# mailund/stralg

Measured on AMD Instinct MI355X. Metric: Msuffixes/s (SA-IS + BWT C/O tables, 1 GiB DNA), higher is better.
Workload: dtype u8 text / u32 indices; 1 GPU; sa_is_construction + init_bwt_table (C, O) on 1073741824 symbols (dna), alphabet_size=5, one independent record per GPU; n=1073741824, alphabet_size=5, records_per_gpu=1, parallelism=batch x1, no collectives, seed=42, generator=dna, numa_node_rank0=1

## Files before the change

### include/stralg_amd.h

```cpp
#ifndef STRALG_AMD_H
#define STRALG_AMD_H

#include <stddef.h>
#include <stdint.h>

#ifdef __cplusplus
extern "C" {
#endif

typedef struct sx_ctx sx_ctx;

enum {
    SX_OK = 0,
    SX_E_ARG = -1,
    SX_E_NOMEM = -2,
    SX_E_INTERNAL = -3,
    SX_E_MALFORMED = -4,
    SX_E_CAPACITY = -5
};

enum {
    SX_KC_CLASSIFY = 0,
    SX_KC_SAMPLES,
    SX_KC_KEYS,
    SX_KC_RADIX_HIST,
    SX_KC_RADIX_SCATTER,
    SX_KC_SCAN,
    SX_KC_NAMES,
    SX_KC_DOUBLING,
    SX_KC_INDUCE_GATHER,
    SX_KC_INDUCE_SCAN,
    SX_KC_INDUCE_SCATTER,
    SX_KC_INDUCE_CHAIN,
    SX_KC_BWT_GATHER,
    SX_KC_OTABLE,
    SX_KC_MISC,
    SX_KC_FASTA,
    SX_KC_REMAP,
    SX_KC_LCP,
    SX_KC_SEARCH,
    SX_KC_LOCAL_SORT,
    SX_KC_SAM,
    SX_KC_COUNT
};

typedef struct sx_kernel_stat {
    uint64_t launches;
    double ms;
    uint64_t alg_bytes;
} sx_kernel_stat;

typedef struct sx_build_stats {
    uint64_t n;
    uint64_t n_lms;
    uint64_t n_samples;
    uint64_t n_names;
    uint32_t key_bits;
    uint32_t key_slots;
    uint32_t doubling_rounds;
    uint32_t induce_rounds;
    uint32_t sort_passes;
    uint32_t lms_path;
    uint32_t sort_local;
    uint32_t refine_tiers;
    double ms_total;
    uint32_t induce_redo;
    uint32_t long_runs;
    uint32_t recursion_levels;
    uint32_t sample_tied_permille;
    uint32_t long_subbuckets;
} sx_build_stats;

int sx_device_count(void);
int sx_device_numa_node(int device);
int sx_ctx_create(int device, sx_ctx **out);
void sx_ctx_destroy(sx_ctx *ctx);
int sx_ctx_live_count(void);
const char *sx_last_error(const sx_ctx *ctx);
void sx_ctx_trim(sx_ctx *ctx);
enum {
    SX_FLAG_FORCE_GENERAL_PATH = 1,
    SX_FLAG_CHAIN_MAX_ENTRIES = 2,
    SX_FLAG_NO_DIRECT_SORT = 3,
    SX_FLAG_PREFIX_SYMBOLS = 4,
    SX_FLAG_RADIX_DIGIT_BITS = 5,
    SX_FLAG_SORT_MODE = 6,
    SX_FLAG_INDUCE_BATCH_OFF = 7,
    SX_FLAG_INDUCE_BATCH_MIN = 8,
    SX_FLAG_INDUCE_ATTENDED = 9
    ,SX_FLAG_COPY_TEXT_FIRST = 10
    ,SX_FLAG_RECURSE_MIN = 11
    ,SX_FLAG_SAMPLE_MIN = 12
    ,SX_FLAG_INDUCE_NO_HOIST = 13
    ,SX_FLAG_TEXT_KEYS_OFF = 14
    ,SX_FLAG_LONG_SUBBUCKETS_OFF = 15
    ,SX_FLAG_SMALL_DIRECT_MAX = 16
    ,SX_FLAG_LOCAL_SORT_LEAN_OFF = 17
    ,SX_FLAG_SAM_BATCH_READS = 18
    ,SX_FLAG_SAM_WINDOW_BYTES = 19
};
int sx_ctx_set_flag(sx_ctx *ctx, int flag, int value);

int sx_sa_build(sx_ctx *ctx, const uint8_t *text, uint64_t n, uint32_t alphabet_size,
                uint32_t *sa_out);
int sx_sa_build_dev(sx_ctx *ctx, const uint8_t *d_text, uint64_t n, uint32_t alphabet_size,
                    uint32_t *d_sa_out);

int sx_sa_bwt_build_dev(sx_ctx *ctx, const uint8_t *d_text, uint64_t n, uint32_t alphabet_size,
                        uint32_t *d_sa_out, uint8_t *d_bwt_out);

int sx_bwt_tables(sx_ctx *ctx, const uint8_t *text, const uint32_t *sa, uint64_t N,
                  uint32_t sigma, uint32_t *c_out, uint32_t *o_out);
int sx_bwt_tables_dev(sx_ctx *ctx, const uint8_t *d_text, const uint32_t *d_sa, uint64_t N,
                      uint32_t sigma, uint32_t *d_c_out, uint32_t *d_o_out, uint8_t *d_bwt_out);

int sx_bwt_tables_from_bwt_dev(sx_ctx *ctx, const uint8_t *d_bwt, uint64_t N, uint32_t sigma,
                               uint32_t *d_c_out, uint32_t *d_o_out);
int sx_build_tables(sx_ctx *ctx, const uint8_t *text, uint64_t n, uint32_t sigma, uint32_t *sa_out,
                    uint32_t *c_out, uint32_t *o_out);

int sx_sa_inverse_dev(sx_ctx *ctx, const uint32_t *d_sa, uint64_t N, uint32_t *d_inv_out);
int sx_sa_lcp_dev(sx_ctx *ctx, const uint8_t *d_text, const uint32_t *d_sa, uint64_t N, uint32_t *d_inv_out,
                  uint32_t *d_lcp_out);
int sx_sa_inverse_lcp(sx_ctx *ctx, const uint8_t *text, const uint32_t *sa, uint64_t N, uint32_t *inv_out,
                      uint32_t *lcp_out);
int sx_bwt_exact_search_dev(sx_ctx *ctx, const uint32_t *d_c_table, const uint32_t *d_o_table, uint64_t N,
                            uint32_t sigma, const uint8_t *d_patterns, const uint32_t *d_offsets, uint32_t count,
                            uint32_t *d_l_out, uint32_t *d_r_out);

#define SX_APPROX_MAX_EDITS 8
#define SX_APPROX_GAP_D 0x8000u
typedef struct sx_approx_hit {
    uint32_t query;
    uint32_t L, R;
    uint16_t match_length;
    uint16_t n_gaps;
    uint16_t gap[SX_APPROX_MAX_EDITS];
} sx_approx_hit;
int sx_bwt_approx_search_dev(sx_ctx *ctx, const uint32_t *d_c_table, const uint32_t *d_o_table,
                             const uint32_t *d_ro_table, uint64_t N, uint32_t sigma, const uint8_t *d_patterns,
                             const uint32_t *d_offsets, uint32_t count, int max_edits, uint64_t *d_hit_offsets,
                             sx_approx_hit *d_hits, uint64_t hit_capacity, uint64_t *total_hits_out);
int sx_bwt_approx_search(sx_ctx *ctx, const uint32_t *c_table, const uint32_t *o_table, const uint32_t *ro_table,
                         uint64_t N, uint32_t sigma, const uint8_t *patterns, const uint32_t *offsets, uint32_t count,
                         int max_edits, uint64_t *hit_offsets, sx_approx_hit **hits_out, uint64_t *total_hits_out);

typedef int (*sx_sink_fn)(void *user, int section, const void *data, size_t bytes);
enum { SX_SECTION_SA = 0, SX_SECTION_C = 1, SX_SECTION_O = 2, SX_SECTION_SAM = 3 ,
       SX_SECTION_INDEX = 4  };
int sx_build_tables_stream(sx_ctx *ctx, const uint8_t *text, uint64_t n, uint32_t sigma, int want_sa, sx_sink_fn sink,
                           void *user);

typedef struct sx_sam_batch {
    const sx_approx_hit *d_hits;
    uint64_t n_hits;
    const uint32_t *d_sa;
    uint64_t sa_len;
    const uint32_t *const *d_sa_list;
    const uint64_t *d_sa_len_list;
    const uint8_t *d_names, *d_seqs, *d_quals;
    const uint32_t *d_name_off, *d_seq_off, *d_qual_off;
    uint32_t n_reads;
    const uint8_t *d_rnames;
    const uint32_t *d_rname_off;
    uint32_t n_records;
} sx_sam_batch;
int sx_sam_layout_dev(sx_ctx *ctx, const sx_sam_batch *batch, uint64_t *d_byte_offsets, uint64_t *total_bytes_out);
int sx_sam_emit_dev(sx_ctx *ctx, const sx_sam_batch *batch, const uint64_t *d_byte_offsets, uint64_t total_bytes, uint64_t byte_lo,
                    uint64_t byte_hi, uint8_t *d_out);

typedef struct sx_fastq {
    uint32_t count;
    uint8_t *names, *seqs, *quals;
    uint32_t *name_off, *seq_off, *qual_off;
} sx_fastq;
int sx_fastq_index(const uint8_t *file, size_t len, sx_fastq *out);
void sx_fastq_free(sx_fastq *fq);

typedef struct sx_map_record {
    const char *name;
    const uint32_t *sa;
    const uint32_t *c_table;
// ... 77 lines not shown
```

### stralg_amd/_lib.py

```python
import ctypes as C
import os

_HERE = os.path.dirname(os.path.abspath(__file__))
PRODUCT_LIB = os.path.join(_HERE, "libstralg_amd.so")

KC_NAMES = ["classify", "samples", "keys", "radix_hist", "radix_scatter", "scan", "names", "doubling",
            "induce_gather", "induce_scan", "induce_scatter", "induce_chain", "bwt_gather", "otable", "misc",
            "fasta", "remap", "lcp", "search", "local_sort", "sam"]


class KernelStat(C.Structure):
    _fields_ = [("launches", C.c_uint64), ("ms", C.c_double), ("alg_bytes", C.c_uint64)]


class BuildStats(C.Structure):
    _fields_ = [("n", C.c_uint64), ("n_lms", C.c_uint64), ("n_samples", C.c_uint64),
                ("n_names", C.c_uint64), ("key_bits", C.c_uint32), ("key_slots", C.c_uint32),
                ("doubling_rounds", C.c_uint32), ("induce_rounds", C.c_uint32),
                ("sort_passes", C.c_uint32), ("lms_path", C.c_uint32), ("sort_local", C.c_uint32), ("refine_tiers", C.c_uint32),
                ("ms_total", C.c_double), ("induce_redo", C.c_uint32), ("long_runs", C.c_uint32),
                ("recursion_levels", C.c_uint32), ("sample_tied_permille", C.c_uint32), ("long_subbuckets", C.c_uint32)]

    def as_dict(self):
        return {k: getattr(self, k) for k, _ in self._fields_}


APPROX_MAX_EDITS = 8
APPROX_GAP_D = 0x8000
APPROX_HIT_DTYPE = [("query", "<u4"), ("L", "<u4"), ("R", "<u4"), ("match_length", "<u2"), ("n_gaps", "<u2"),
                    ("gap", "<u2", (APPROX_MAX_EDITS,))]
SX_E_ARG, SX_E_MALFORMED, SX_E_CAPACITY = -1, -4, -5
SX_SECTION_SAM = 3
SX_FLAG_SAM_BATCH_READS, SX_FLAG_SAM_WINDOW_BYTES = 18, 19


class SamBatch(C.Structure):
    _fields_ = [("d_hits", C.c_void_p), ("n_hits", C.c_uint64), ("d_sa", C.c_void_p), ("sa_len", C.c_uint64),
                ("d_sa_list", C.c_void_p), ("d_sa_len_list", C.c_void_p),
                ("d_names", C.c_void_p), ("d_seqs", C.c_void_p), ("d_quals", C.c_void_p),
                ("d_name_off", C.c_void_p), ("d_seq_off", C.c_void_p), ("d_qual_off", C.c_void_p), ("n_reads", C.c_uint32),
                ("d_rnames", C.c_void_p), ("d_rname_off", C.c_void_p), ("n_records", C.c_uint32)]


class Fastq(C.Structure):
    _fields_ = [("count", C.c_uint32), ("names", C.c_void_p), ("seqs", C.c_void_p), ("quals", C.c_void_p),
                ("name_off", C.c_void_p), ("seq_off", C.c_void_p), ("qual_off", C.c_void_p)]


class MapRecord(C.Structure):
    _fields_ = [("name", C.c_char_p), ("sa", C.c_void_p), ("c_table", C.c_void_p), ("o_table", C.c_void_p),
                ("ro_table", C.c_void_p), ("N", C.c_uint64), ("sigma", C.c_uint32), ("remap", C.c_void_p)]


class FastqDev(C.Structure):
    _fields_ = [("count", C.c_uint32), ("d_names", C.c_void_p), ("d_seqs", C.c_void_p), ("d_quals", C.c_void_p),
                ("d_name_off", C.c_void_p), ("d_seq_off", C.c_void_p), ("d_qual_off", C.c_void_p),
                ("name_bytes", C.c_uint64), ("seq_bytes", C.c_uint64), ("qual_bytes", C.c_uint64)]


class IndexSource(C.Structure):
    _fields_ = [("record", MapRecord), ("string", C.c_void_p)]


class IndexRecord(C.Structure):
    _fields_ = [("name", C.c_char_p), ("N", C.c_uint64), ("sigma", C.c_uint32), ("has_ro", C.c_int), ("has_string", C.c_int),
                ("remap", C.c_void_p), ("d_string", C.c_void_p), ("d_sa", C.c_void_p), ("d_c", C.c_void_p), ("d_o", C.c_void_p),
                ("d_ro", C.c_void_p)]


SX_SECTION_INDEX = 4
SINK_FN = C.CFUNCTYPE(C.c_int, C.c_void_p, C.c_int, C.c_void_p, C.c_size_t)


def load(path=None):
    path = path or PRODUCT_LIB
    try:
        import torch
    except ImportError:
        pass
    if not os.path.exists(path):
        raise RuntimeError(
            f"{path} is missing: build it with `make -C stralg_amd/csrc` "
            "(or python -c 'import __graft_entry__ as g; g.build()'); there is no CPU fallback")
    lib = C.CDLL(path)
    vp, u8p, u32p, u64p = C.c_void_p, C.c_void_p, C.c_void_p, C.c_void_p
    sig = {
        "sx_device_count": (C.c_int, []),
        "sx_device_numa_node": (C.c_int, [C.c_int]),
        "sx_ctx_create": (C.c_int, [C.c_int, C.POINTER(vp)]),
        "sx_ctx_destroy": (None, [vp]),
        "sx_ctx_live_count": (C.c_int, []),
        "sx_last_error": (C.c_char_p, [vp]),
        "sx_ctx_trim": (None, [vp]),
        "sx_ctx_set_flag": (C.c_int, [vp, C.c_int, C.c_int]),
        "sx_sa_build": (C.c_int, [vp, u8p, C.c_uint64, C.c_uint32, u32p]),
        "sx_sa_build_dev": (C.c_int, [vp, u8p, C.c_uint64, C.c_uint32, u32p]),
        "sx_sa_bwt_build_dev": (C.c_int, [vp, u8p, C.c_uint64, C.c_uint32, u32p, u8p]),
        "sx_bwt_tables_from_bwt_dev": (C.c_int, [vp, u8p, C.c_uint64, C.c_uint32, u32p, u32p]),
        "sx_build_tables": (C.c_int, [vp, u8p, C.c_uint64, C.c_uint32, u32p, u32p, u32p]),
        "sx_bwt_tables": (C.c_int, [vp, u8p, u32p, C.c_uint64, C.c_uint32, u32p, u32p]),
        "sx_bwt_tables_dev": (C.c_int, [vp, u8p, u32p, C.c_uint64, C.c_uint32, u32p, u32p, u8p]),
        "sx_sa_inverse_dev": (C.c_int, [vp, u32p, C.c_uint64, u32p]),
        "sx_sa_lcp_dev": (C.c_int, [vp, u8p, u32p, C.c_uint64, u32p, u32p]),
        "sx_sa_inverse_lcp": (C.c_int, [vp, u8p, u32p, C.c_uint64, u32p, u32p]),
# ... 78 lines not shown
```

### stralg_amd/api.py

```python
import ctypes as C
import threading
import time

import numpy as np

from . import _lib


class StralgAmdError(RuntimeError):
    pass


def _ptr(x):
    if x is None:
        return None
    if isinstance(x, int):
        return x
    if isinstance(x, np.ndarray):
        return x.ctypes.data
    if hasattr(x, "data_ptr"):
        return x.data_ptr()
    raise TypeError(f"cannot take the address of {type(x)!r}")


# ... 217 lines not shown
        self._check(self.lib.sx_fasta_pack_dev(self.h, _ptr(d_file), file_len, _ptr(d_packed), C.byref(plen), _ptr(d_term),
                                               term_cap, C.byref(nrec)), "sx_fasta_pack_dev")
        return int(plen.value), int(nrec.value)

    def remap_dev(self, d_in, n, d_out):
        table = np.zeros(256, dtype=np.int16)
        sigma = C.c_uint32(0)
        self._check(self.lib.sx_remap_dev(self.h, _ptr(d_in), n, _ptr(d_out), table.ctypes.data_as(C.POINTER(C.c_int16)),
                                          C.byref(sigma)), "sx_remap_dev")
        return int(sigma.value), table

    def reverse_dev(self, d_in, n, d_out):
        self._check(self.lib.sx_reverse_dev(self.h, _ptr(d_in), n, _ptr(d_out)), "sx_reverse_dev")

    def fasta_records(self, data):
        buf = np.frombuffer(bytes(data), dtype=np.uint8)
        packed = np.zeros(buf.size + 1, dtype=np.uint8)
        term = np.zeros(buf.size + 2, dtype=np.uint32)
        plen, nrec = C.c_uint64(0), C.c_uint32(0)
        self._check(self.lib.sx_fasta_pack(self.h, _ptr(buf) if buf.size else None, buf.size, _ptr(packed), C.byref(plen),
                                           _ptr(term), term.size, C.byref(nrec)), "sx_fasta_pack")
        out = []
        for r in range(nrec.value):
            n0 = 0 if r == 0 else int(term[2 * r - 1]) + 1
            s0 = int(term[2 * r]) + 1
            out.append((packed[n0:int(term[2 * r])].tobytes(), packed[s0:int(term[2 * r + 1])].tobytes()))
        return out

    def prim_sort_pairs_dev(self, ka, va, kb, vb, n, begin_bit, end_bit):
        flag = C.c_int(0)
        self._check(self.lib.sx_prim_sort_pairs_dev(self.h, _ptr(ka), _ptr(va), _ptr(kb), _ptr(vb), n, begin_bit,
                                                    end_bit, C.byref(flag)), "sx_prim_sort_pairs_dev")
        return bool(flag.value)

    def prim_exclusive_sum_dev(self, d_in, d_out, n, d_total=None):
        self._check(self.lib.sx_prim_exclusive_sum_dev(self.h, _ptr(d_in), _ptr(d_out), n, _ptr(d_total)),
                    "sx_prim_exclusive_sum_dev")

    def prim_classify_dev(self, d_text, n, d_flags, d_hist_all, d_hist_l, d_hist_lms):
        self._check(self.lib.sx_prim_classify_dev(self.h, _ptr(d_text), n, _ptr(d_flags), _ptr(d_hist_all),
                                                  _ptr(d_hist_l), _ptr(d_hist_lms)), "sx_prim_classify_dev")

    def profile_only(self, kclass_name=None):
        k = -1 if kclass_name is None else _lib.KC_NAMES.index(kclass_name)
        self._check(self.lib.sx_profile_only(self.h, k), "sx_profile_only")

    def profile_enable(self, on=True):
        self._check(self.lib.sx_profile_enable(self.h, 1 if on else 0), "sx_profile_enable")

    def profile_reset(self):
        self._check(self.lib.sx_profile_reset(self.h), "sx_profile_reset")

    def profile_read(self):
        arr = (_lib.KernelStat * len(_lib.KC_NAMES))()
        self._check(self.lib.sx_profile_read(self.h, arr), "sx_profile_read")
        return {name: {"launches": int(arr[i].launches), "ms": float(arr[i].ms), "alg_bytes": int(arr[i].alg_bytes)}
                for i, name in enumerate(_lib.KC_NAMES)}

    def last_stats(self):
        st = _lib.BuildStats()
        self._check(self.lib.sx_last_stats(self.h, C.byref(st)), "sx_last_stats")
        return st.as_dict()

    def force_general_path(self, on=True):
        self._check(self.lib.sx_ctx_set_flag(self.h, 1, 1 if on else 0), "sx_ctx_set_flag")

    def set_chain_max_entries(self, entries):
        self._check(self.lib.sx_ctx_set_flag(self.h, 2, int(entries)), "sx_ctx_set_flag")

    def set_no_direct_sort(self, on=True):
        self._check(self.lib.sx_ctx_set_flag(self.h, 3, 1 if on else 0), "sx_ctx_set_flag")

    def set_prefix_symbols(self, symbols):
        self._check(self.lib.sx_ctx_set_flag(self.h, 4, int(symbols)), "sx_ctx_set_flag")

    def set_radix_digit_bits(self, bits):
        self._check(self.lib.sx_ctx_set_flag(self.h, 5, int(bits)), "sx_ctx_set_flag")

    def set_sort_mode(self, mode):
        self._check(self.lib.sx_ctx_set_flag(self.h, 6, int(mode)), "sx_ctx_set_flag")

    def set_induce_batch(self, on=True):
        self._check(self.lib.sx_ctx_set_flag(self.h, 7, 0 if on else 1), "sx_ctx_set_flag")

    def set_induce_batch_min(self, entries):
        self._check(self.lib.sx_ctx_set_flag(self.h, 8, int(entries)), "sx_ctx_set_flag")

    def set_induce_attended(self, mode=1):
        self._check(self.lib.sx_ctx_set_flag(self.h, 9, int(mode)), "sx_ctx_set_flag")

    def set_induce_hoist(self, on=True):
        self._check(self.lib.sx_ctx_set_flag(self.h, 13, 0 if on else 1), "sx_ctx_set_flag")

    def set_text_keys(self, on=True):
        self._check(self.lib.sx_ctx_set_flag(self.h, 14, 0 if on else 1), "sx_ctx_set_flag")

    def set_long_subbuckets(self, on=True):
        self._check(self.lib.sx_ctx_set_flag(self.h, 15, 0 if on else 1), "sx_ctx_set_flag")

    def set_local_sort_lean(self, on=True):
        self._check(self.lib.sx_ctx_set_flag(self.h, 17, 0 if on else 1), "sx_ctx_set_flag")

    def set_small_direct_max(self, suffixes):
        self._check(self.lib.sx_ctx_set_flag(self.h, 16, int(suffixes)), "sx_ctx_set_flag")

    def set_recurse_min(self, symbols):
        self._check(self.lib.sx_ctx_set_flag(self.h, 11, int(symbols)), "sx_ctx_set_flag")

    def set_sample_min(self, suffixes):
        self._check(self.lib.sx_ctx_set_flag(self.h, 12, int(suffixes)), "sx_ctx_set_flag")

    def set_copy_text_first(self, on=True):
        self._check(self.lib.sx_ctx_set_flag(self.h, 10, 1 if on else 0), "sx_ctx_set_flag")

    def trim(self):
        self.lib.sx_ctx_trim(self.h)

    def bind_to_numa_node(self):
        self.lib.stralg_amd_bind_thread_to_device.argtypes = [C.c_int]
        self.lib.stralg_amd_bind_thread_to_device.restype = C.c_int
        return int(self.lib.stralg_amd_bind_thread_to_device(self.device))


def _map_record(name, t, keep):
    sa = np.ascontiguousarray(t.sa.array, dtype=np.uint32)
    c = np.ascontiguousarray(t.c_table, dtype=np.uint32)
    o = np.ascontiguousarray(t.o_table, dtype=np.uint32)
    ro = None if t.ro_table is None else np.ascontiguousarray(t.ro_table, dtype=np.uint32)
    tab = np.ascontiguousarray(np.clip(t.remap_table.table, -1, 127), dtype=np.int8)
    keep.append((sa, c, o, ro, tab))
    return _lib.MapRecord(bytes(name), _ptr(sa), _ptr(c), _ptr(o), _ptr(ro), sa.size, t.remap_table.alphabet_size, _ptr(tab))


class Index:

    def __init__(self, ctx, handle):
        self.ctx = ctx
        self.h = handle

    @classmethod
    def from_fasta(cls, fasta_bytes, include_reverse=True, ctx=None):
        ctx = ctx or default_context()
        buf = np.frombuffer(bytes(fasta_bytes), dtype=np.uint8)
        h = C.c_void_p()
        ctx._check(ctx.lib.sx_index_build_fasta(ctx.h, _ptr(buf) if buf.size else None, buf.size, 1 if include_reverse else 0,
                                                C.byref(h)), "sx_index_build_fasta")
        return cls(ctx, h)

    @classmethod
    def from_tables(cls, records, ctx=None):
        ctx = ctx or default_context()
        src = (_lib.IndexSource * max(1, len(records)))()
        keep = []
        for r, (name, t) in enumerate(records):
            src[r].record = _map_record(name, t, keep)
            string = getattr(t.sa, "string", None)
            if string is not None:
                string = np.ascontiguousarray(string, dtype=np.uint8)
                keep.append(string)
                src[r].string = _ptr(string)
        h = C.c_void_p()
        ctx._check(ctx.lib.sx_index_from_sources(ctx.h, src, len(records), C.byref(h)), "sx_index_from_sources")
        return cls(ctx, h)

    @classmethod
    def load(cls, path_or_bytes, ctx=None):
# ... 329 lines not shown
```

### stralg_amd/csrc/sx_common.hpp

```cpp
#pragma once
#include <hip/hip_runtime.h>
#include <hip/hip_ext.h>

#include <stdint.h>
#include <stdio.h>
#include <string.h>

#include <vector>

#include "../../include/stralg_amd.h"

#define SX_CHECK(expr)                                                         \
    do {                                                                       \
        hipError_t e_ = (expr);                                                \
        if (e_ != hipSuccess) return sx_fail(ctx, (int)e_, #expr, __FILE__, __LINE__); \
    } while (0)

#define SX_TRY(expr)                                                           \
    do {                                                                       \
        int rc_ = (expr);                                                      \
        if (rc_ != 0) return rc_;                                              \
    } while (0)

struct sx_slab {
    void *p = nullptr;
    size_t cap = 0;
};

struct sx_arena {
    char *base = nullptr;
    size_t cap = 0, off = 0;
    template <class T> T *take(size_t count)
    {
        size_t bytes = (count * sizeof(T) + 255) & ~(size_t)255;
        if (off + bytes > cap) return nullptr;
        T *r = reinterpret_cast<T *>(base + off);
        off += bytes;
        return r;
    }
};

struct sx_event_pair {
    hipEvent_t a, b;
    int kclass;
};

enum {
    SX_SLAB_N = 0,
    SX_SLAB_M = 1,
    SX_SLAB_BWT = 2,
    SX_SLAB_SCAN = 3,
    SX_SLAB_SORT = 4,
    SX_SLAB_IO = 5,
    SX_SLAB_CHAIN = 6,
    SX_NSLABS = 7
};

struct sx_ctx {
    int device = 0;
    hipStream_t stream = nullptr;
    char err[512] = {0};
    sx_slab slab[SX_NSLABS];
    uint32_t *h_pin = nullptr;
    uint32_t readback_seq = 0;
    char *h_stage[2] = {nullptr, nullptr};
    uint32_t chain_epoch = 0;
    int64_t chain_max_override = -1;
    int prefix_symbols = 0;
    int force_general = 0;
    int no_direct = 0;
    int radix_digit_bits = 0;
    int sort_mode = 0;
    int induce_batch_off = 0;
    int induce_attended = 0;
    int induce_no_hoist = 0;
    int text_keys_off = 0;
    int long_subbuckets_off = 0;
    int local_sort_lean_off = 0;
    int64_t small_direct_max = -1;
    int copy_text_first = 0;
    int64_t sam_batch_reads = 0;
    int64_t sam_window_bytes = 0;
    int64_t sample_min = -1;
    int64_t recurse_min = -1;
    sx_ctx *child = nullptr;
    int depth = 0;
    int64_t induce_batch_min = -1;
    int prof_on = 0;
    int prof_only = -1;
    hipError_t launch_err = hipSuccess;
    int launch_err_class = 0;
    std::vector<sx_event_pair> ev_used;
    std::vector<sx_event_pair> ev_free;
    sx_kernel_stat kstat[SX_KC_COUNT];
    sx_build_stats stats;
};

int sx_fail(sx_ctx *ctx, int code, const char *what, const char *file, int line);
int sx_fail_msg(sx_ctx *ctx, int code, const char *msg);
int sx_slab_ensure(sx_ctx *ctx, int which, size_t bytes);
int sx_sync(sx_ctx *ctx);
int sx_readback(sx_ctx *ctx, const uint32_t *d_src, size_t count, uint32_t *h_dst);
int sx_readback_ranges(sx_ctx *ctx, const uint32_t *const *d_src, const uint32_t *counts, int ranges, uint32_t *h_dst);
int sx_chain_slab(sx_ctx *ctx, int which, size_t bytes);
uint32_t sx_chain_next_epoch(sx_ctx *ctx);

int sx_child_begin(sx_ctx *ctx, sx_ctx **child);
void sx_child_end(sx_ctx *ctx, sx_ctx *child);

sx_event_pair *sx_prof_pair(sx_ctx *ctx, int kclass);
void sx_prof_count(sx_ctx *ctx, int kclass, uint64_t alg_bytes);

template <class... P, class... A>
static inline void sx_launch(sx_ctx *ctx, int kclass, uint64_t alg_bytes, void (*kernel)(P...),
                             dim3 grid, dim3 block, A... args)
{
    const bool timed = ctx->prof_on && (ctx->prof_only < 0 || ctx->prof_only == kclass);
    sx_event_pair *ep = timed ? sx_prof_pair(ctx, kclass) : nullptr;
    if (ep) hipExtLaunchKernelGGL(kernel, grid, block, 0, ctx->stream, ep->a, ep->b, 0u, static_cast<P>(args)...);
    else hipLaunchKernelGGL(kernel, grid, block, 0, ctx->stream, args...);
    const hipError_t e = hipGetLastError();
    if (e != hipSuccess && ctx->launch_err == hipSuccess) ctx->launch_err = e, ctx->launch_err_class = kclass;
    if (ep) sx_prof_count(ctx, kclass, alg_bytes);
}

static inline uint32_t sx_div_up(uint64_t a, uint64_t b) { return (uint32_t)((a + b - 1) / b); }
static inline int sx_bitlen(uint64_t v)
{
    int b = 0;
    while (v) {
        ++b;
        v >>= 1;
    }
    return b;
}
```

### stralg_amd/csrc/sx_ctx.hip

```cpp
#include <atomic>
#include <chrono>
#include "sx_common.hpp"
#include "sx_scan.hpp"

#include <new>

static const char *kClassNames[SX_KC_COUNT] = {
    "classify", "samples", "keys", "radix_hist", "radix_scatter", "scan", "names",
    "doubling", "induce_gather", "induce_scan", "induce_scatter", "induce_chain", "bwt_gather", "otable", "misc",
    "fasta", "remap", "lcp", "search", "local_sort", "sam",
};

int sx_fail(sx_ctx *ctx, int code, const char *what, const char *file, int line)
{
    if (ctx) snprintf(ctx->err, sizeof ctx->err, "%s failed: %s (%d) at %s:%d", what,
                      hipGetErrorString((hipError_t)code), code, file, line);
    return code ? code : SX_E_INTERNAL;
}

int sx_fail_msg(sx_ctx *ctx, int code, const char *msg)
{
    if (ctx) snprintf(ctx->err, sizeof ctx->err, "%s", msg);
    return code;
}
// ... 93 lines not shown
int sx_readback(sx_ctx *ctx, const uint32_t *d_src, size_t count, uint32_t *h_dst)
{
    if (count > 1024) return sx_fail_msg(ctx, SX_E_INTERNAL, "readback too large");
    const uint32_t seq = ++ctx->readback_seq ? ctx->readback_seq : ++ctx->readback_seq;
    hipLaunchKernelGGL(sx::readback_kernel, dim3(1), dim3(256), 0, ctx->stream, d_src, (uint32_t)count, ctx->h_pin, seq);
    if (hipGetLastError() != hipSuccess) return sx_fail_msg(ctx, SX_E_INTERNAL, "readback launch refused");
    return readback_wait(ctx, seq, count, h_dst);
}

int sx_readback_ranges(sx_ctx *ctx, const uint32_t *const *d_src, const uint32_t *counts, int ranges, uint32_t *h_dst)
{
    sx::readback_ranges r = {{nullptr, nullptr, nullptr, nullptr}, {0, 0, 0, 0}};
    size_t total = 0;
    if (ranges < 1 || ranges > 4) return sx_fail_msg(ctx, SX_E_INTERNAL, "readback: one to four arrays");
    for (int k = 0; k < ranges; ++k) r.src[k] = d_src[k], r.count[k] = counts[k], total += counts[k];
    if (total > 1024) return sx_fail_msg(ctx, SX_E_INTERNAL, "readback too large");
    const uint32_t seq = ++ctx->readback_seq ? ctx->readback_seq : ++ctx->readback_seq;
    hipLaunchKernelGGL(sx::readback_ranges_kernel, dim3(1), dim3(256), 0, ctx->stream, r, ctx->h_pin, seq);
    if (hipGetLastError() != hipSuccess) return sx_fail_msg(ctx, SX_E_INTERNAL, "readback launch refused");
    return readback_wait(ctx, seq, total, h_dst);
}

static int readback_wait(sx_ctx *ctx, uint32_t seq, size_t count, uint32_t *h_dst)
{
    volatile uint32_t *flag = ctx->h_pin + 1024;
    const auto t0 = std::chrono::steady_clock::now();
    uint32_t spins = 0;
    while (*flag != seq) {
        __builtin_ia32_pause();
        if ((++spins & 0xFFu) == 0 && std::chrono::steady_clock::now() - t0 > std::chrono::microseconds(kReadbackSpinUs)) break;
    }
    if (*flag != seq) SX_CHECK(hipStreamSynchronize(ctx->stream));
    std::atomic_thread_fence(std::memory_order_acquire);
    if (*flag != seq) return sx_fail_msg(ctx, SX_E_INTERNAL, "readback: the sequence word did not arrive");
    if (ctx->launch_err != hipSuccess) return launch_error(ctx);
    memcpy(h_dst, ctx->h_pin, count * sizeof(uint32_t));
    return 0;
}

sx_event_pair *sx_prof_pair(sx_ctx *ctx, int kclass)
{
    sx_event_pair ep;
    if (!ctx->ev_free.empty()) {
        ep = ctx->ev_free.back();
        ctx->ev_free.pop_back();
    } else {
        if (hipEventCreate(&ep.a) != hipSuccess || hipEventCreate(&ep.b) != hipSuccess) return nullptr;
    }
    ep.kclass = kclass;
    ctx->ev_used.push_back(ep);
    return &ctx->ev_used.back();
}

void sx_prof_count(sx_ctx *ctx, int kclass, uint64_t alg_bytes)
{
    ctx->kstat[kclass].launches += 1;
    ctx->kstat[kclass].alg_bytes += alg_bytes;
}

static void prof_drain(sx_ctx *ctx)
{
    if (ctx->ev_used.empty()) return;
    (void)hipStreamSynchronize(ctx->stream);
    for (sx_event_pair &ep : ctx->ev_used) {
        float ms = 0.f;
        if (hipEventElapsedTime(&ms, ep.a, ep.b) == hipSuccess) ctx->kstat[ep.kclass].ms += ms;
        ctx->ev_free.push_back(ep);
    }
    ctx->ev_used.clear();
}

int sx_child_begin(sx_ctx *ctx, sx_ctx **out)
{
    if (!ctx->child) {
        int rc = sx_ctx_create(ctx->device, &ctx->child);
        if (rc != 0) return sx_fail_msg(ctx, rc, "cannot create the context of the reduced string");
        ctx->child->depth = ctx->depth + 1;
    }
    sx_ctx *c = ctx->child;
    c->chain_max_override = ctx->chain_max_override;
    c->radix_digit_bits = ctx->radix_digit_bits;
    c->sort_mode = ctx->sort_mode;
    c->induce_batch_off = ctx->induce_batch_off;
    c->induce_batch_min = ctx->induce_batch_min;
    c->induce_attended = ctx->induce_attended;
    c->induce_no_hoist = ctx->induce_no_hoist;
    c->text_keys_off = ctx->text_keys_off;
    c->long_subbuckets_off = ctx->long_subbuckets_off;
    c->local_sort_lean_off = ctx->local_sort_lean_off;
    c->small_direct_max = ctx->small_direct_max;
    c->copy_text_first = ctx->copy_text_first;
    c->recurse_min = ctx->recurse_min;
    c->sample_min = ctx->sample_min;
    c->no_direct = 1;
    c->force_general = 1;
    c->prefix_symbols = 0;
    c->prof_on = ctx->prof_on;
    c->prof_only = ctx->prof_only;
    *out = c;
    return 0;
}

void sx_child_end(sx_ctx *ctx, sx_ctx *c)
{
    prof_drain(c);
    for (int k = 0; k < SX_KC_COUNT; ++k) {
        ctx->kstat[k].launches += c->kstat[k].launches;
        ctx->kstat[k].ms += c->kstat[k].ms;
        ctx->kstat[k].alg_bytes += c->kstat[k].alg_bytes;
    }
    memset(c->kstat, 0, sizeof c->kstat);
    c->prof_on = 0;
}

extern "C" {

int sx_device_count(void)
{
    int n = 0;
    if (hipGetDeviceCount(&n) != hipSuccess) return 0;
    return n;
}

int sx_device_numa_node(int device)
{
    char bus[64] = {0};
    if (hipDeviceGetPCIBusId(bus, (int)sizeof bus, device) != hipSuccess) return -1;
    for (char *p = bus; *p; ++p)
        if (*p >= 'A' && *p <= 'F') *p = (char)(*p - 'A' + 'a');
    char path[160];
    snprintf(path, sizeof path, "/sys/bus/pci/devices/%s/numa_node", bus);
    FILE *f = fopen(path, "r");
    if (!f) return -1;
    int node = -1;
    if (fscanf(f, "%d", &node) != 1) node = -1;
    fclose(f);
    return node;
}

static std::atomic<int> g_live_contexts{0};
extern "C" int sx_ctx_live_count(void) { return g_live_contexts.load(); }

int sx_ctx_create(int device, sx_ctx **out)
{
    if (!out) return SX_E_ARG;
    *out = nullptr;
    int ndev = 0;
    hipError_t e = hipGetDeviceCount(&ndev);
    if (e != hipSuccess || ndev <= 0) {
        fprintf(stderr, "stralg_amd: no usable HIP device (%s); this library has no CPU fallback\n",
                e != hipSuccess ? hipGetErrorString(e) : "device count 0");
        return e != hipSuccess ? (int)e : SX_E_INTERNAL;
    }
    if (device < 0 || device >= ndev) return SX_E_ARG;
    sx_ctx *ctx = new (std::nothrow) sx_ctx();
    if (!ctx) return SX_E_NOMEM;
    ctx->device = device;
    memset(ctx->kstat, 0, sizeof ctx->kstat);
    memset(&ctx->stats, 0, sizeof ctx->stats);
    if (hipSetDevice(device) != hipSuccess || hipStreamCreateWithFlags(&ctx->stream, hipStreamNonBlocking) != hipSuccess ||
        hipHostMalloc((void **)&ctx->h_pin, 8192, hipHostMallocDefault) != hipSuccess) {
        fprintf(stderr, "stralg_amd: cannot initialise device %d\n", device);
        delete ctx;
        return SX_E_INTERNAL;
    }
    memset(ctx->h_pin, 0, 8192);
// ... 28 lines not shown
    }
    if (ctx->h_pin) (void)hipHostFree(ctx->h_pin);
    for (char *b : ctx->h_stage)
        if (b) (void)hipHostFree(b);
    if (ctx->stream) (void)hipStreamDestroy(ctx->stream);
    g_live_contexts.fetch_sub(1);
    delete ctx;
}

int sx_ctx_set_flag(sx_ctx *ctx, int flag, int value)
{
    if (!ctx) return SX_E_ARG;
    if (flag == SX_FLAG_FORCE_GENERAL_PATH) {
        ctx->force_general = value ? 1 : 0;
        return 0;
    }
    if (flag == SX_FLAG_NO_DIRECT_SORT) {
        ctx->no_direct = value ? 1 : 0;
        return 0;
    }
    if (flag == SX_FLAG_PREFIX_SYMBOLS) {
        ctx->prefix_symbols = value > 0 ? value : 0;
        return 0;
    }
    if (flag == SX_FLAG_SORT_MODE) {
        if (value < 0 || value > 3) return SX_E_ARG;
        ctx->sort_mode = value;
        return 0;
    }
    if (flag == SX_FLAG_RADIX_DIGIT_BITS) {
        if (value != 0 && (value < 8 || value > 10)) return SX_E_ARG;
        ctx->radix_digit_bits = value;
        return 0;
    }
    if (flag == SX_FLAG_INDUCE_BATCH_OFF) {
        ctx->induce_batch_off = value ? 1 : 0;
        return 0;
    }
    if (flag == SX_FLAG_SAMPLE_MIN) {
        ctx->sample_min = value < 0 ? -1 : (int64_t)value;
        return 0;
    }
    if (flag == SX_FLAG_RECURSE_MIN) {
        ctx->recurse_min = value < 0 ? -1 : (int64_t)value;
        return 0;
    }
    if (flag == SX_FLAG_COPY_TEXT_FIRST) {
        ctx->copy_text_first = value ? 1 : 0;
        return 0;
    }
    if (flag == SX_FLAG_INDUCE_ATTENDED) {
        if (value < 0 || value > 2) return SX_E_ARG;
        ctx->induce_attended = value == 1 ? 1 : 0;
        return 0;
    }
    if (flag == SX_FLAG_TEXT_KEYS_OFF) {
        ctx->text_keys_off = value ? 1 : 0;
        return 0;
    }
    if (flag == SX_FLAG_SMALL_DIRECT_MAX) {
        ctx->small_direct_max = value < 0 ? -1 : (int64_t)value;
        return 0;
    }
    if (flag == SX_FLAG_LONG_SUBBUCKETS_OFF) {
        ctx->long_subbuckets_off = value ? 1 : 0;
        return 0;
    }
    if (flag == SX_FLAG_LOCAL_SORT_LEAN_OFF) {
        ctx->local_sort_lean_off = value ? 1 : 0;
        return 0;
    }
    if (flag == SX_FLAG_SAM_BATCH_READS) {
        ctx->sam_batch_reads = value > 0 ? value : 0;
        return 0;
    }
    if (flag == SX_FLAG_SAM_WINDOW_BYTES) {
        ctx->sam_window_bytes = value > 0 ? value : 0;
        return 0;
    }
    if (flag == SX_FLAG_INDUCE_NO_HOIST) {
        ctx->induce_no_hoist = value ? 1 : 0;
        return 0;
    }
    if (flag == SX_FLAG_INDUCE_BATCH_MIN) {
        ctx->induce_batch_min = value < 0 ? -1 : (int64_t)value;
        return 0;
    }
    if (flag == SX_FLAG_CHAIN_MAX_ENTRIES) {
        ctx->chain_max_override = value < 0 ? -1 : (int64_t)value;
        return 0;
    }
    return SX_E_ARG;
}

const char *sx_last_error(const sx_ctx *ctx) { return ctx ? ctx->err : "no context"; }

int sx_profile_enable(sx_ctx *ctx, int on)
{
    if (!ctx) return SX_E_ARG;
    if (!on) prof_drain(ctx);
    ctx->prof_on = on ? 1 : 0;
    return 0;
}

int sx_profile_only(sx_ctx *ctx, int kclass)
{
    if (!ctx || kclass >= SX_KC_COUNT) return SX_E_ARG;
    ctx->prof_only = kclass < 0 ? -1 : kclass;
    return 0;
}

int sx_profile_reset(sx_ctx *ctx)
{
    if (!ctx) return SX_E_ARG;
    prof_drain(ctx);
    memset(ctx->kstat, 0, sizeof ctx->kstat);
    return 0;
}

int sx_profile_read(sx_ctx *ctx, sx_kernel_stat *out)
{
    if (!ctx || !out) return SX_E_ARG;
    prof_drain(ctx);
    memcpy(out, ctx->kstat, sizeof ctx->kstat);
    return 0;
}

const char *sx_kernel_class_name(int kclass)
{
    return kclass >= 0 && kclass < SX_KC_COUNT ? kClassNames[kclass] : "?";
}

int sx_last_stats(const sx_ctx *ctx, sx_build_stats *out)
{
    if (!ctx || !out) return SX_E_ARG;
    *out = ctx->stats;
    return 0;
}

}
```

### stralg_amd/csrc/sx_induce.hip

```cpp
#include "sx_induce_common.hpp"
#include "sx_induce_small.hpp"
#include "sx_induce_wide.hpp"
#include "sx_induce_chain.hpp"

using namespace sx;

size_t sx_induce_scratch_bytes(uint64_t N, uint32_t sigma)
{
    const uint64_t ntiles = (N + kIndTile - 1) / kIndTile + 1;
    const uint64_t wtiles = N / 4096 + 4;
    return (size_t)N * 8 + 256 + (size_t)(N / 2 + 2) * 8 + 256 + (size_t)N + 256 + (size_t)sigma * ntiles * 4 + 256 +
           (size_t)kBatchRows * (ntiles + 1) * 4 + 1024 +
           (sigma > 8 ? (size_t)(wtiles + wtiles / 256 + 4) * 1024 + 512 : 0) + 16384 +
           (sigma > 8 ? ((size_t)N / kWideTile + 520) * 1024 + 5 * 65536 * 4 + 16384 : 0);
}

namespace {
#ifndef SX_INDUCE_GRID_CAP
#define SX_INDUCE_GRID_CAP 16384
#endif
constexpr uint32_t kInduceGridCap = SX_INDUCE_GRID_CAP;
constexpr int kMaxSpec = 16;

template <class WT> struct induce_state {
    sx_ctx *ctx;
    const uint8_t *T;
    uint32_t *SA;
    WT *WN;
    uint64_t N, m;
    uint8_t *BW;
    uint32_t *cursor[2];
    uint32_t *ranges;
    uint32_t *tickets;
    uint32_t *run_len;
    uint64_t *status;
    uint32_t chain_max;
    uint32_t *hist;
    uint32_t *bhist;
    uint32_t *btotals;
    int batch_on;
    int unattended;
    uint32_t *poison;
    uint32_t *host_poison;
    uint32_t *whist;
    uint32_t *wsums;
    uint32_t stride;
    uint32_t nk;
    int small_alphabet;
    int par;
    wnd_cfg cfg;
    int hoist;
    uint32_t *d_begin;
    uint32_t *hoist_E;
    uint32_t *hoist_tot;
    uint32_t *hoist_err;
    uint32_t hoist_from;
    int next_c;
    int begun_c;
};

template <class WT>
void launch_round(induce_state<WT> &st, const uint32_t *srcP, const WT *srcW, int range_slot, int out_slot,
                  uint32_t tiles_bound, uint32_t tiles_likely, int rev, int mode, uint32_t c, int dir, int tail_follows,
                  int chained_only_up_to_chain_max = 0, int three_launch_only = 0)
{
    sx_ctx *ctx = st.ctx;
    uint32_t grid = tiles_bound < 1 ? 1 : tiles_bound;
    if (grid > kInduceGridCap) grid = kInduceGridCap;
    const uint32_t epoch = sx_chain_next_epoch(ctx);
    uint32_t *rin = st.ranges + 2 * range_slot;
    uint32_t *rout = out_slot >= 0 ? st.ranges + 2 * out_slot : nullptr;
    const uint32_t *cur = st.cursor[st.par];
    uint32_t *nxt = st.cursor[st.par ^ 1];
    const bool only3 = three_launch_only != 0;
    const bool both = only3 || (!chained_only_up_to_chain_max && (uint64_t)tiles_likely * kIndTile > st.chain_max);
    const uint32_t chain_max = only3 ? 0u : ((both || chained_only_up_to_chain_max) ? st.chain_max : ~0u);
    const int pass_large = chained_only_up_to_chain_max;
    if (both && st.small_alphabet) {
        const uint8_t *srcB = srcP == st.SA ? (const uint8_t *)st.BW : nullptr;
        const uint64_t src_len = srcP == st.SA ? st.N : st.m;
        if (srcB)
            sx_launch(ctx, SX_KC_INDUCE_GATHER, 0, induce_count_bytes_kernel, dim3(grid), dim3(kBlock), srcB, (const uint32_t *)rin, rev,
                      mode, c, st.hist, st.stride, st.nk, chain_max, src_len);
        else
            sx_launch(ctx, SX_KC_INDUCE_GATHER, 0, induce_count_kernel<WT, 3>, dim3(grid), dim3(kBlock), srcW, srcB,
                      (const uint32_t *)rin, rev, mode, c, st.cfg, st.hist, st.stride, st.nk, chain_max, src_len);
        sx_launch(ctx, SX_KC_INDUCE_SCAN, (uint64_t)tiles_bound * st.nk * 8, induce_offsets_kernel, dim3(st.nk),
                  dim3(kRowThreads), st.hist, st.stride, (const uint32_t *)rin, rout, cur, nxt, dir, c, chain_max, only3 ? 1 : 0);
        {
#define SX_SCATTER_SMALL(M)                                                                                            \
    sx_launch(ctx, SX_KC_INDUCE_SCATTER, 0, induce_scatter_small_kernel<WT, M>, dim3(grid), dim3(kBlock), srcP, srcW, \
              (const uint32_t *)rin, c, st.cfg, st.T, (const uint32_t *)st.hist, st.stride, cur, st.SA, st.WN, st.BW, st.nk, \
              chain_max)
            switch (mode) {
            case MODE_L_FROM_L: SX_SCATTER_SMALL(MODE_L_FROM_L); break;
            case MODE_L_FROM_LMS: SX_SCATTER_SMALL(MODE_L_FROM_LMS); break;
            case MODE_S_FROM_S: SX_SCATTER_SMALL(MODE_S_FROM_S); break;
            default: SX_SCATTER_SMALL(MODE_S_FROM_L); break;
            }
#undef SX_SCATTER_SMALL
        }
    }
    if (both && !st.small_alphabet) {
        const uint8_t *srcB = srcP == st.SA ? (const uint8_t *)st.BW : nullptr;
        const uint32_t wtiles = sx_div_up((uint64_t)(tiles_bound < 1 ? 1 : tiles_bound) * kIndTile, kWideTile);
        const uint32_t wgrid = wtiles > 2048 ? 2048 : wtiles;
        const int only = only3 ? 1 : 0;
        sx_launch(ctx, SX_KC_INDUCE_GATHER, 0, induce_wide_count_kernel<WT>, dim3(wgrid), dim3(kWideThreads), srcW, srcB,
                  (const uint32_t *)rin, rev, mode, c, st.cfg, st.whist, chain_max);
        if (wtiles <= kWideOffMaxTiles) {
            sx_launch(ctx, SX_KC_INDUCE_SCAN, (uint64_t)wtiles * 2048, induce_wide_offsets_kernel, dim3(256 / kWideOffCols), dim3(kWideOffThreads),
                      st.whist, (const uint32_t *)rin, rout, cur, nxt, dir, c, chain_max, only);
        } else {
            const uint32_t nchunks = sx_div_up(wtiles, kWideChunk);
            sx_launch(ctx, SX_KC_INDUCE_SCAN, (uint64_t)wtiles * 1024, induce_wide_colsum_kernel, dim3(nchunks), dim3(kBlock),
                      (const uint32_t *)st.whist, (const uint32_t *)rin, st.wsums, chain_max);
            sx_launch(ctx, SX_KC_INDUCE_SCAN, (uint64_t)nchunks * 2048, induce_wide_bases_kernel, dim3(1), dim3(kBlock), st.wsums,
                      (const uint32_t *)rin, rout, cur, nxt, dir, c, chain_max, only);
            sx_launch(ctx, SX_KC_INDUCE_SCAN, (uint64_t)wtiles * 2048, induce_wide_apply_kernel, dim3(nchunks), dim3(kBlock), st.whist,
                      (const uint32_t *)rin, (const uint32_t *)st.wsums, chain_max);
        }
        sx_launch(ctx, SX_KC_INDUCE_SCATTER, 0, induce_wide_scatter_kernel<WT, 8>, dim3(wgrid), dim3(kWideThreads),
                  srcP, srcW, (const uint32_t *)rin, rev, mode, c, st.cfg, st.T, (const uint32_t *)st.whist, cur, dir, st.SA, st.WN,
                  st.BW, chain_max);
    }
    uint32_t cgrid = grid > 1024 ? 1024 : grid;
    if (only3) {
    } else if (st.small_alphabet)
        sx_launch(ctx, SX_KC_INDUCE_CHAIN, 0, induce_round_kernel<WT, 3>, dim3(cgrid), dim3(kBlock), srcP, srcW,
                  (const uint32_t *)rin, rout, rev, mode, c, st.cfg, st.T, cur, nxt, dir, st.SA, st.WN, st.BW, st.nk, st.status,
                  epoch, st.tickets + range_slot, chain_max, tail_follows, pass_large);
    else if (st.nk <= 32)
        sx_launch(ctx, SX_KC_INDUCE_CHAIN, 0, induce_round_kernel<WT, 5>, dim3(cgrid), dim3(kBlock), srcP, srcW,
                  (const uint32_t *)rin, rout, rev, mode, c, st.cfg, st.T, cur, nxt, dir, st.SA, st.WN, st.BW, st.nk, st.status,
                  epoch, st.tickets + range_slot, chain_max, tail_follows, pass_large);
    else
        sx_launch(ctx, SX_KC_INDUCE_CHAIN, 0, induce_round_kernel<WT, 8>, dim3(cgrid), dim3(kBlock), srcP, srcW,
                  (const uint32_t *)rin, rout, rev, mode, c, st.cfg, st.T, cur, nxt, dir, st.SA, st.WN, st.BW, st.nk, st.status,
                  epoch, st.tickets + range_slot, chain_max, tail_follows, pass_large);
    st.par ^= 1;
    ctx->stats.induce_rounds++;
}

#ifndef SX_TAIL_ITERS_UNATTENDED
#define SX_TAIL_ITERS_UNATTENDED 1024u
#endif
constexpr uint32_t kTailIters = 64, kTailItersUnattended = SX_TAIL_ITERS_UNATTENDED;
template <class WT>
void launch_tail(induce_state<WT> &st, int range_slot, int out_slot, int rev, int mode, uint32_t c, int dir)
{
    sx_ctx *ctx = st.ctx;
    const uint32_t *cur = st.cursor[st.par];
    uint32_t *nxt = st.cursor[st.par ^ 1];
    if (st.small_alphabet)
        sx_launch(ctx, SX_KC_INDUCE_CHAIN, 0, induce_tail_small_kernel<WT>, dim3(1), dim3(kTailBlock), st.SA, st.WN, st.BW,
                  (const uint32_t *)(st.ranges + 2 * range_slot), st.ranges + 2 * out_slot, rev, mode, c, st.cfg, st.T,
                  cur, nxt, dir, st.unattended ? kTailItersUnattended : kTailIters, st.unattended ? st.poison : (uint32_t *)nullptr,
                  st.host_poison);
    else {
        tail_next nb = {-1, st.nk, nullptr, nullptr, nullptr, nullptr, nullptr, 0u, nullptr};
        if (st.hoist && st.unattended && st.next_c >= 0)
            nb = {st.next_c, st.nk, (const uint32_t *)st.d_begin, (const uint32_t *)st.hoist_E, (const uint32_t *)st.hoist_tot, st.ranges,
                  st.tickets, (uint32_t)(kMaxSpec + 2), st.hoist_err};
        sx_launch(ctx, SX_KC_INDUCE_CHAIN, 0, induce_tail_kernel<WT, 8>, dim3(1), dim3(kTailBlock), st.SA, st.WN, st.BW,
                  (const uint32_t *)(st.ranges + 2 * range_slot), st.ranges + 2 * out_slot, rev, mode, c, st.cfg, st.T,
                  cur, nxt, dir, st.unattended ? kTailItersUnattended : kTailIters, st.unattended ? st.poison : (uint32_t *)nullptr,
                  st.host_poison, nb);
        st.begun_c = nb.c;
    }
    st.par ^= 1;
}

template <class WT>
void launch_batch(induce_state<WT> &st, int range_slot, int out_slot, uint32_t tiles_bound, int mode, uint32_t c)
{
    sx_ctx *ctx = st.ctx;
    uint32_t grid = tiles_bound < 1 ? 1 : tiles_bound;
    if (grid > kInduceGridCap) grid = kInduceGridCap;
    const uint32_t *rin = st.ranges + 2 * range_slot;
    uint32_t *rout = st.ranges + 2 * out_slot;
    const uint32_t *cur = st.cursor[st.par];
    uint32_t *nxt = st.cursor[st.par ^ 1];
    const uint32_t min_len = ctx->induce_batch_min >= 0 ? (uint32_t)ctx->induce_batch_min : kTailEntries;
    if (mode == MODE_L_FROM_L) {
        sx_launch(ctx, SX_KC_INDUCE_GATHER, 0, induce_batch_count_kernel<WT, MODE_L_FROM_L>, dim3(grid), dim3(kBlock),
                  (const uint32_t *)st.SA, (const WT *)st.WN, rin, c, st.cfg, st.T, st.bhist, st.stride, min_len);
    } else {
        sx_launch(ctx, SX_KC_INDUCE_GATHER, 0, induce_batch_count_kernel<WT, MODE_S_FROM_S>, dim3(grid), dim3(kBlock),
                  (const uint32_t *)st.SA, (const WT *)st.WN, rin, c, st.cfg, st.T, st.bhist, st.stride, min_len);
    }
    sx_launch(ctx, SX_KC_INDUCE_SCAN, (uint64_t)tiles_bound * st.nk * kBatchRounds * 8, induce_batch_offsets_kernel,
              dim3(kBatchRounds * st.nk), dim3(kRowThreads), st.bhist, st.stride, rin, st.btotals, st.nk, min_len);
    if (mode == MODE_L_FROM_L) {
        sx_launch(ctx, SX_KC_INDUCE_SCATTER, 0, induce_batch_scatter_kernel<WT, MODE_L_FROM_L>, dim3(grid), dim3(kBlock),
                  (const uint32_t *)st.SA, (const WT *)st.WN, rin, rout, c, st.cfg, st.T, (const uint32_t *)st.bhist, st.stride,
                  (const uint32_t *)st.btotals, cur, nxt, st.SA, st.WN, st.BW, st.nk, min_len);
    } else {
        sx_launch(ctx, SX_KC_INDUCE_SCATTER, 0, induce_batch_scatter_kernel<WT, MODE_S_FROM_S>, dim3(grid), dim3(kBlock),
                  (const uint32_t *)st.SA, (const WT *)st.WN, rin, rout, c, st.cfg, st.T, (const uint32_t *)st.bhist, st.stride,
                  (const uint32_t *)st.btotals, cur, nxt, st.SA, st.WN, st.BW, st.nk, min_len);
    }
    st.par ^= 1;
    ctx->stats.induce_rounds++;
}

template <class WT>
int run_self_rounds(induce_state<WT> &st, uint32_t fixed_bound, uint32_t region_entries, int rev, int mode, uint32_t c,
                    int dir, int which, uint32_t *total_in_region, double share ,
                    const uint32_t *resume = nullptr )
{
    sx_ctx *ctx = st.ctx;
    bool first = true;
    uint32_t bound_tiles = sx_div_up(region_entries ? region_entries : 1, kIndTile);
    int spec = 1;
    {
        const int sh = st.small_alphabet ? 2 : 6;
        while (spec < kMaxSpec && (bound_tiles >> (sh * spec)) >= 1) ++spec;
    }
    if (!st.small_alphabet) {
        double expect = (double)region_entries * share;
        int by_share = 1;
        const double tail_takes = (double)(kTailMulti * kTailEntries) / ((st.unattended && !resume) ? 2.0 : 8.0);
        while (by_share < kMaxSpec && expect > tail_takes) ++by_share, expect *= share;
        if (st.unattended && !resume) spec = by_share;
        else if (by_share > spec) spec = by_share;
    }
    const uint64_t max_batches = 2 * (st.N / kTailIters) + 64;
    uint32_t r[2] = {0, 0};
    bool resuming = resume != nullptr;
    if (resuming) r[0] = resume[0], r[1] = resume[1];
    for (uint64_t batch = 0;; ++batch) {
        if (batch > max_batches) return sx_fail_msg(ctx, SX_E_INTERNAL, "induce: the rounds of a bucket did not come to an end");
        if (!resuming) {
        if (first && st.hoist) {
            if (st.begun_c != (int)c)
                sx_launch(ctx, SX_KC_INDUCE_SCAN, 0, bucket_begin_kernel, dim3(1), dim3(256), st.ranges, st.cursor[st.par],
                          (const uint32_t *)st.d_begin, (const uint32_t *)st.hoist_E, (const uint32_t *)st.hoist_tot, st.nk, c, st.hoist_from,
                          dir, st.tickets, (uint32_t)(kMaxSpec + 2), (const uint32_t *)(st.unattended ? st.poison : nullptr), st.hoist_err);
            st.begun_c = -1;
            st.hoist_from = c;
        } else if (first)
            sx_launch(ctx, SX_KC_INDUCE_SCAN, 0, set_range_kernel, dim3(1), dim3(1), st.ranges, fixed_bound, fixed_bound,
                      (const uint32_t *)st.cursor[st.par], (int)c, which, st.tickets, (uint32_t)(kMaxSpec + 2),
                      (const uint32_t *)(st.unattended ? st.poison : nullptr));
        else
            SX_CHECK(hipMemsetAsync(st.tickets, 0, (kMaxSpec + 2) * sizeof(uint32_t), ctx->stream));
        const bool batched = st.small_alphabet && st.batch_on && (mode == MODE_L_FROM_L || mode == MODE_S_FROM_S);
        if (batched) {
            int slot = 0;
            if (first) {
                double expect = (double)region_entries;
                const double batch_from = ctx->induce_batch_min >= 0 ? (double)ctx->induce_batch_min : (double)kBatchFrom;
                for (int k = 0; k < 6 && expect > batch_from; ++k, expect *= share) {
                    uint32_t tb = sx_div_up((uint64_t)(expect * 2.0 < (double)region_entries ? expect * 2.0 : (double)region_entries), kIndTile);
                    if (tb < 256) tb = bound_tiles < 256 ? bound_tiles : 256;
                    const bool sure = ctx->induce_batch_min >= 0 || expect > 4.0 * (double)st.chain_max;
                    launch_round<WT>(st, st.SA, st.WN, slot, slot + 1, tb, tb, rev, mode, c, dir, 1, 0, sure ? 1 : 0);
                    ++slot;
                }
            }
            launch_batch<WT>(st, slot, slot + 1, bound_tiles, mode, c);
            ++slot;
            if (!first) {
                for (int k = 0; k < 3; ++k, ++slot)
                    launch_round<WT>(st, st.SA, st.WN, slot, slot + 1, bound_tiles < 256 ? bound_tiles : 256, 0, rev, mode, c, dir, 1, 1);
            }
            spec = slot;
        }
        for (int k = 0; k < spec && !batched; ++k) {
            uint32_t tb = bound_tiles >> k;
            const uint32_t floor_tiles = bound_tiles < 256 ? bound_tiles : 256;
            if (tb < floor_tiles) tb = floor_tiles;
            double expect = 2.0 * (double)bound_tiles;
            for (int i = 0; i < k; ++i) expect *= share;
            const uint32_t likely = expect < (double)bound_tiles ? (uint32_t)expect : bound_tiles;
            const bool sure = first && k == 0 && (uint64_t)region_entries > 16ull * st.chain_max;
            launch_round<WT>(st, st.SA, st.WN, k, k + 1, tb, first && k == 0 ? bound_tiles : likely, rev, mode, c, dir, 1, 0, sure ? 1 : 0);
        }
        launch_tail<WT>(st, spec, spec + 1, rev, mode, c, dir);
        if (st.unattended) {
            if (total_in_region) *total_in_region = 0xFFFFFFFFu;
            return 0;
        }
        SX_TRY(sx_readback(ctx, st.ranges + 2 * (spec + 1), 2, r));
        if (r[1] == r[0]) {
            if (total_in_region) *total_in_region = dir > 0 ? r[1] : r[0];
            return 0;
        }
        }
        resuming = false;
        sx_launch(ctx, SX_KC_INDUCE_SCAN, 0, set_range_kernel, dim3(1), dim3(1), st.ranges, r[0], r[1],
                  (const uint32_t *)st.cursor[st.par], (int)c, 0, (uint32_t *)nullptr, 0u, (const uint32_t *)nullptr);
        if (r[1] - r[0] <= kRunEntries) {
            for (int rep = 0; rep < 2; ++rep) {
                SX_CHECK(hipMemsetAsync(st.run_len, 0xFF, sizeof(uint32_t), ctx->stream));
                const uint64_t look = st.N < (uint64_t)kRunProbe ? st.N : (uint64_t)kRunProbe;
                sx_launch(ctx, SX_KC_INDUCE_CHAIN, 0, run_probe_kernel, dim3(1, r[1] - r[0]), dim3(kBlock), st.T,
                          (const uint32_t *)st.SA, (const uint32_t *)st.ranges, c, 0u,
                          (uint32_t)(look < kRunProbeChunk ? look : kRunProbeChunk), st.run_len);
                if (look > kRunProbeChunk) {
                    const uint32_t far_chunks = sx_div_up(look - kRunProbeChunk, kRunProbeChunk);
                    sx_launch(ctx, SX_KC_INDUCE_CHAIN, 0, run_probe_kernel,
                              dim3(far_chunks < kRunProbeGrid ? far_chunks : kRunProbeGrid, r[1] - r[0]), dim3(kBlock), st.T,
                              (const uint32_t *)st.SA, (const uint32_t *)st.ranges, c, kRunProbeChunk, (uint32_t)look, st.run_len);
                }
                sx_launch(ctx, SX_KC_INDUCE_CHAIN, 0, run_fill_kernel<WT>, dim3(4096), dim3(kBlock), st.T, st.SA, st.WN, st.BW,
                          (const uint32_t *)st.ranges, (const uint32_t *)st.cursor[st.par], c, rev, dir, st.cfg,
                          (const uint32_t *)st.run_len);
                sx_launch(ctx, SX_KC_INDUCE_CHAIN, 0, run_commit_kernel, dim3(1), dim3(1), st.ranges, st.cursor[st.par], c, dir,
                          (const uint32_t *)st.run_len);
            }
        }
        first = false;
    }
}

template <class WT>
int induce_typed(sx_ctx *ctx, const sx_text_info &ti, uint32_t sigma, const uint32_t *sorted_lms,
                 const void *seed_windows, bool seed_windows_u32, uint32_t *SA, uint8_t *bwt_out, sx_arena &arena, wnd_cfg cfg)
{
    const uint64_t N = ti.N;
    const uint32_t nk = ti.maxc + 1 < sigma ? ti.maxc + 1 : sigma;
    induce_state<WT> st;
    st.ctx = ctx;
    st.T = ti.T;
    st.SA = SA;
    st.nk = nk;
    st.small_alphabet = nk <= 8;
    st.cfg = cfg;
    st.par = 0;
    st.WN = arena.take<WT>(N);
    st.BW = bwt_out ? bwt_out : arena.take<uint8_t>(N);
    st.N = N;
    st.m = ti.m;
    const bool widen = seed_windows && seed_windows_u32 && sizeof(WT) == 8;
    WT *seedW = seed_windows && !widen ? (WT *)seed_windows : arena.take<WT>(ti.m ? ti.m : 1);
    st.cursor[0] = arena.take<uint32_t>(256);
    st.cursor[1] = arena.take<uint32_t>(256);
    st.ranges = arena.take<uint32_t>(2 * (kMaxSpec + 3));
    st.tickets = arena.take<uint32_t>(kMaxSpec + 3);
    st.run_len = arena.take<uint32_t>(4);
    if (!st.WN || !st.BW || !seedW || !st.cursor[0] || !st.cursor[1] || !st.ranges || !st.tickets || !st.run_len)
        return sx_fail_msg(ctx, SX_E_INTERNAL, "induce: arena too small");

    uint32_t begin[257], lms_off[257];
    begin[0] = 0;
    lms_off[0] = 0;
    uint32_t largest = 1;
    for (uint32_t c = 0; c < 256; ++c) {
        begin[c + 1] = begin[c] + ti.h_all[c];
        lms_off[c + 1] = lms_off[c] + ti.h_lms[c];
        if (ti.h_all[c] > largest) largest = ti.h_all[c];
    }
    st.chain_max = ctx->chain_max_override >= 0 ? (uint32_t)ctx->chain_max_override
                                                : (st.small_alphabet ? 256u * (uint32_t)kIndTile : 4u * kTailEntries);
    const size_t status_words = ((size_t)sx_div_up(largest, kIndTile) + 2) * nk + kChainHeader;
    st.stride = sx_div_up(largest, kIndTile) + 1;
    st.hist = st.whist = st.wsums = st.bhist = st.btotals = nullptr;
    st.batch_on = ctx->induce_batch_off ? 0 : 1;
    if (st.small_alphabet) {
        st.hist = arena.take<uint32_t>((size_t)nk * st.stride);
        st.bhist = arena.take<uint32_t>((size_t)kBatchRows * st.stride);
        st.btotals = arena.take<uint32_t>(kBatchRows);
        if (!st.hist || !st.bhist || !st.btotals) return sx_fail_msg(ctx, SX_E_INTERNAL, "induce: arena too small (tile counts)");
    } else {
        const size_t wt = (size_t)sx_div_up(largest, kWideTile) + 2;
        st.whist = arena.take<uint32_t>(wt * 256);
        st.wsums = arena.take<uint32_t>((wt / kWideChunk + 2) * 256);
        if (!st.whist || !st.wsums) return sx_fail_msg(ctx, SX_E_INTERNAL, "induce: arena too small (tile counts)");
    }
    SX_TRY(sx_chain_slab(ctx, SX_SLAB_CHAIN, status_words * 8));
    st.status = (uint64_t *)ctx->slab[SX_SLAB_CHAIN].p;
    SX_CHECK(hipMemsetAsync(st.status, 0, sizeof(uint64_t), ctx->stream));

    if (widen)
        sx_launch(ctx, SX_KC_INDUCE_GATHER, ti.m * 12, widen_windows_kernel, dim3(sx_div_up(ti.m, kBlock * 4)), dim3(kBlock),
                  (const uint32_t *)seed_windows, (uint64_t)ti.m, (uint64_t *)seedW);
    else if (!seed_windows)
        sx_launch(ctx, SX_KC_INDUCE_GATHER, ti.m * (4 + sizeof(WT) + 16), fill_windows_kernel<WT>,
                  dim3(sx_div_up(ti.m, kBlock)), dim3(kBlock), ti.T, sorted_lms, ti.m, cfg, seedW);
    sx_launch(ctx, SX_KC_MISC, 0, set_entry_kernel<WT>, dim3(1), dim3(1), SA, st.WN, st.BW, (uint32_t)ti.n, ti.T, cfg);

    st.poison = arena.take<uint32_t>(4);
    if (!st.poison) return sx_fail_msg(ctx, SX_E_INTERNAL, "induce: arena too small");
    st.host_poison = ctx->h_pin + 1040;
    st.hoist = (!st.small_alphabet && !ctx->induce_no_hoist) ? 1 : 0;
    st.d_begin = st.hoist_E = st.hoist_tot = st.hoist_err = nullptr;
    st.hoist_from = 0;
    st.next_c = st.begun_c = -1;
    uint32_t *hz_BG = nullptr, *hz_EL = nullptr, *hz_ES = nullptr, *hz_tot = nullptr, *hz_dbase = nullptr, *hz_hist = nullptr,
             *hz_desc = nullptr;
    uint32_t h_desc[2][768];
    uint32_t hz_rows[2] = {0, 0}, hz_most[2] = {1, 1};
    if (st.hoist) {
        for (int pass = 0; pass < 2; ++pass) {
            uint32_t row = 0;
            for (uint32_t c = 0; c < 256; ++c) {
                const uint32_t len = c < nk ? (pass == 0 ? ti.h_lms[c] : ti.h_l[c]) : 0u;
                h_desc[pass][c] = pass == 0 ? lms_off[c] : begin[c];
                h_desc[pass][256 + c] = len;
                h_desc[pass][512 + c] = row;
                const uint32_t tiles = sx_div_up(len, kWideTile);
                row += tiles;
                if (tiles > hz_most[pass]) hz_most[pass] = tiles;
            }
            hz_rows[pass] = row;
        }
        st.d_begin = arena.take<uint32_t>(260);
        hz_BG = arena.take<uint32_t>(65536);
        hz_EL = arena.take<uint32_t>(65536);
        hz_ES = arena.take<uint32_t>(65536);
        hz_tot = arena.take<uint32_t>(65536);
        hz_dbase = arena.take<uint32_t>(65536);
        hz_desc = arena.take<uint32_t>(2 * 768);
        st.hoist_err = arena.take<uint32_t>(4);
        hz_hist = arena.take<uint32_t>(((size_t)(hz_rows[0] > hz_rows[1] ? hz_rows[0] : hz_rows[1]) + 2) * 256);
        if (!st.d_begin || !hz_BG || !hz_EL || !hz_ES || !hz_tot || !hz_dbase || !hz_desc || !st.hoist_err || !hz_hist)
            return sx_fail_msg(ctx, SX_E_INTERNAL, "induce: arena too small (up-front rounds)");
        SX_CHECK(hipMemcpyAsync(st.d_begin, begin, 257 * sizeof(uint32_t), hipMemcpyHostToDevice, ctx->stream));
        SX_CHECK(hipMemcpyAsync(hz_desc, h_desc, sizeof h_desc, hipMemcpyHostToDevice, ctx->stream));
        SX_CHECK(hipMemsetAsync(hz_BG, 0, 65536 * sizeof(uint32_t), ctx->stream));
        SX_CHECK(hipMemsetAsync(st.hoist_err, 0, 4 * sizeof(uint32_t), ctx->stream));
        uint32_t bg_grid = (uint32_t)sx_div_up(sx_div_up(ti.n ? ti.n : 1, 16), (uint64_t)kBigramThreads * 16);
        if (bg_grid > kBigramGrid) bg_grid = kBigramGrid;
        sx_launch(ctx, SX_KC_INDUCE_GATHER, ti.n * (uint64_t)sx_div_up(nk, kBigramWords / nk), bigram_kernel, dim3(bg_grid),
                  dim3(kBigramThreads), ti.T, (uint64_t)ti.n, nk, hz_BG);
        sx_launch(ctx, SX_KC_INDUCE_SCAN, 0, hoist_tables_kernel, dim3(1), dim3(256), (const uint32_t *)hz_BG, (const uint32_t *)st.d_begin, nk,
                  hz_EL, hz_ES);
    }
    auto hoisted_rounds = [&](int pass) -> int {
        const uint32_t *desc = hz_desc + pass * 768;
        const int rev = pass, mode = pass == 0 ? MODE_L_FROM_LMS : MODE_S_FROM_L, dir = pass == 0 ? +1 : -1;
        const uint32_t *srcP = pass == 0 ? sorted_lms : (const uint32_t *)SA;
        const WT *srcW = pass == 0 ? (const WT *)seedW : (const WT *)st.WN;
        const uint8_t *srcB = pass == 0 ? (const uint8_t *)nullptr : (const uint8_t *)st.BW;
        st.hoist_E = pass == 0 ? hz_EL : hz_ES;
        st.hoist_tot = hz_tot;
        st.hoist_from = pass == 0 ? 0u : nk - 1u;
        uint32_t gx = hz_most[pass];
        if (gx > kHoistGridX) gx = kHoistGridX;
        sx_launch(ctx, SX_KC_INDUCE_GATHER, 0, hoist_count_kernel<WT>, dim3(gx, nk), dim3(kWideThreads), srcW, srcB, desc, rev, mode, st.cfg,
                  hz_hist);
        sx_launch(ctx, SX_KC_INDUCE_SCAN, (uint64_t)hz_rows[pass] * 2048, hoist_offsets_kernel, dim3(nk), dim3(kBlock * kHoistOffGroups),
                  hz_hist, desc, (const uint32_t *)st.hoist_E, dir, hz_tot, hz_dbase);
        sx_launch(ctx, SX_KC_INDUCE_SCATTER, 0, hoist_scatter_kernel<WT, 8>, dim3(gx, nk), dim3(kWideThreads), srcP, srcW, desc, rev,
                  mode, st.cfg, st.T, (const uint32_t *)hz_hist, (const uint32_t *)hz_dbase, dir, st.SA, st.WN, st.BW,
                  (uint32_t)(pass == 0 ? 1 : 0));
        ctx->stats.induce_rounds++;
        return 0;
    };
    auto pass_end = [&](int pass, bool with_stop, uint32_t (&rec)[4], uint32_t (&cur)[256], uint32_t (&tail)[3]) -> int {
        const uint32_t *src[4];
        uint32_t cnt[4], page[4 + 256 + 3];
        int k = 0;
        if (with_stop) src[k] = (const uint32_t *)st.poison, cnt[k++] = 4;
        src[k] = (const uint32_t *)st.cursor[st.par], cnt[k++] = nk;
        if (pass == 1) {
            src[k] = (const uint32_t *)st.status, cnt[k++] = 2;
            if (st.hoist) src[k] = (const uint32_t *)st.hoist_err, cnt[k++] = 1;
        }
        SX_TRY(sx_readback_ranges(ctx, src, cnt, k, page));
        const uint32_t *q = page;
        if (with_stop) memcpy(rec, q, sizeof rec), q += 4;
        memcpy(cur, q, nk * sizeof(uint32_t)), q += nk;
        tail[0] = tail[1] = tail[2] = 0;
        if (pass == 1) {
            tail[0] = q[0], tail[1] = q[1];
            if (st.hoist) tail[2] = q[2];
        }
        return 0;
    };
    auto cursors_as_counted = [&](const uint32_t (&cur)[256]) -> bool {
        bool ok = true;
        for (uint32_t c = 1; c < nk; ++c)
            if (ti.h_all[c] && cur[c] != begin[c] + ti.h_l[c]) ok = false;
        return ok;
    };
    const bool unattended_ok = ctx->induce_attended != 1 && ti.open_tiles == 0;
    auto stopped = [&]() -> bool { return st.unattended && *(volatile uint32_t *)st.host_poison != 0; };
    auto pass_L = [&](uint32_t from, const uint32_t *resume) -> int {
        for (uint32_t c = from; c < nk; ++c) {
            if (ti.h_all[c] == 0) continue;
            if (stopped()) return 0;
            const bool carry_on = resume && c == from;
            if (carry_on) st.hoist_from = c;
            if (ti.h_l[c]) {
                uint32_t head_end = 0;
                st.unattended = (unattended_ok && !carry_on) ? 1 : 0;
                st.next_c = -1;
                for (uint32_t c2 = c + 1; c2 < nk && st.next_c < 0; ++c2)
                    if (ti.h_all[c2] && ti.h_l[c2]) st.next_c = (int)c2;
                SX_TRY(run_self_rounds<WT>(st, begin[c], ti.h_l[c], 0, MODE_L_FROM_L, c, +1, 1, &head_end, (double)ti.h_all[c] / (double)N,
                                           carry_on ? resume : nullptr));
                if (!st.unattended && head_end - begin[c] != ti.h_l[c])
                    return sx_fail_msg(ctx, SX_E_INTERNAL, "induce L: bucket did not receive its L-type count");
                st.unattended = unattended_ok ? 1 : 0;
            }
            if (ti.h_lms[c] && !st.hoist) {
                sx_launch(ctx, SX_KC_INDUCE_SCAN, 0, set_range_kernel, dim3(1), dim3(1), st.ranges, lms_off[c], lms_off[c + 1],
                          (const uint32_t *)st.cursor[st.par], (int)c, 0, st.tickets, 1u, (const uint32_t *)(st.unattended ? st.poison : nullptr));
                launch_round<WT>(st, sorted_lms, seedW, 0, -1, sx_div_up(ti.h_lms[c], kIndTile), sx_div_up(ti.h_lms[c], kIndTile), 0,
                                 MODE_L_FROM_LMS, c, +1, 0, 0, ti.h_lms[c] > st.chain_max ? 1 : 0);
            }
        }
        return 0;
    };
    auto pass_S = [&](uint32_t from, const uint32_t *resume) -> int {
        for (uint32_t cc = from + 1; cc-- > 0;) {
            const uint32_t c = cc;
            if (ti.h_all[c] == 0) continue;
            if (stopped()) return 0;
            const bool carry_on = resume && c == from;
            if (carry_on) st.hoist_from = c;
            const uint32_t n_s = ti.h_all[c] - ti.h_l[c];
            if (c > 0 && n_s) {
                uint32_t tail_end = 0;
                st.unattended = (unattended_ok && !carry_on) ? 1 : 0;
                st.next_c = -1;
                for (uint32_t c2 = c; c2-- > 1 && st.next_c < 0;)
                    if (ti.h_all[c2] && ti.h_all[c2] - ti.h_l[c2]) st.next_c = (int)c2;
                SX_TRY(run_self_rounds<WT>(st, begin[c + 1], n_s, 1, MODE_S_FROM_S, c, -1, 2, &tail_end, (double)ti.h_all[c] / (double)N,
                                           carry_on ? resume : nullptr));
                if (!st.unattended && begin[c + 1] - tail_end != n_s)
                    return sx_fail_msg(ctx, SX_E_INTERNAL, "induce S: bucket did not receive its S-type count");
                st.unattended = unattended_ok ? 1 : 0;
            }
            if (ti.h_l[c] && !st.hoist) {
                sx_launch(ctx, SX_KC_INDUCE_SCAN, 0, set_range_kernel, dim3(1), dim3(1), st.ranges, begin[c],
                          begin[c] + ti.h_l[c], (const uint32_t *)st.cursor[st.par], (int)c, 0, st.tickets, 1u,
                          (const uint32_t *)(st.unattended ? st.poison : nullptr));
                launch_round<WT>(st, SA, st.WN, 0, -1, sx_div_up(ti.h_l[c], kIndTile), sx_div_up(ti.h_l[c], kIndTile), 1,
                                 MODE_S_FROM_L, c, -1, 0, 0, ti.h_l[c] > st.chain_max ? 1 : 0);
            }
        }
        return 0;
    };
    ctx->stats.long_runs = ti.open_tiles ? 1u : 0u;
    for (int pass = 0; pass < 2; ++pass) {
        st.unattended = unattended_ok ? 1 : 0;
        if (pass == 1) SX_CHECK(hipStreamSynchronize(ctx->stream));
        SX_CHECK(hipMemcpyAsync(st.cursor[st.par], pass == 0 ? begin : begin + 1, 256 * sizeof(uint32_t), hipMemcpyHostToDevice, ctx->stream));
        if (st.hoist) SX_TRY(hoisted_rounds(pass));
        uint32_t from = pass == 0 ? 0u : nk - 1u, rec[4] = {0, 0, 0, 0}, cur[256], tail[3];
        const uint32_t *resume = nullptr;
        for (uint32_t attempt = 0;; ++attempt) {
            if (attempt > 2 * nk + 4) return sx_fail_msg(ctx, SX_E_INTERNAL, "induce: a pass did not come to its end");
            if (unattended_ok) {
                *(volatile uint32_t *)st.host_poison = 0;
                SX_CHECK(hipMemsetAsync(st.poison, 0, 4 * sizeof(uint32_t), ctx->stream));
            }
            st.next_c = st.begun_c = -1;
            SX_TRY(pass == 0 ? pass_L(from, resume) : pass_S(from, resume));
            SX_TRY(pass_end(pass, unattended_ok, rec, cur, tail));
            if (!unattended_ok || !rec[0]) break;
            ctx->stats.induce_redo++;
            from = rec[1];
            resume = rec + 2;
        }
        if (!cursors_as_counted(cur))
            return sx_fail_msg(ctx, SX_E_INTERNAL, pass == 0 ? "induce L: a bucket did not receive its L-type count"
                                                             : "induce S: a bucket did not receive its S-type count");
        if (pass == 1 && tail[0]) return sx_fail_msg(ctx, SX_E_INTERNAL, "induce: a look-back wait timed out");
        if (pass == 1 && tail[2]) return sx_fail_msg(ctx, SX_E_INTERNAL, "induce: a bucket's cursor is not where the text's bigram counts put it");
    }

    if (ctx->prof_on) {
        uint64_t n_l = 0;
        for (uint32_t c = 0; c < nk; ++c) n_l += ti.h_l[c];
        const uint64_t scanned = n_l + ti.m + (N - 1);
        if (ctx->prof_only < 0 || ctx->prof_only == SX_KC_INDUCE_GATHER)
            ctx->kstat[SX_KC_INDUCE_GATHER].alg_bytes += (scanned - ti.m) + ti.m * sizeof(WT);
        if (ctx->prof_only < 0 || ctx->prof_only == SX_KC_INDUCE_SCATTER)
            ctx->kstat[SX_KC_INDUCE_SCATTER].alg_bytes += (scanned + N) * (4 + sizeof(WT)) + N;
    }
    return 0;
}
}

int sx_bwt_from_seed_windows(sx_ctx *ctx, const uint32_t *seedw, uint64_t N, uint32_t maxc, uint8_t *bwt_out)
{
    wnd_cfg cfg;
    (void)sx_window_cfg(maxc, cfg);
    cfg.CW = 1;
    sx_launch(ctx, SX_KC_BWT_GATHER, N * 5, bwt_from_windows_kernel<uint32_t>, dim3(sx_div_up(N, kBlock * 16)), dim3(kBlock),
              seedw, N, cfg, bwt_out);
    return 0;
}

int sx_induce(sx_ctx *ctx, const sx_text_info &ti, uint32_t sigma, const uint32_t *sorted_lms,
              const void *seed_windows, bool seed_windows_u32, uint32_t *SA, uint8_t *bwt_out, sx_arena &arena)
{
    if (ti.N > 0xFFFFFFFFull) return sx_fail_msg(ctx, SX_E_ARG, "induce: n exceeds 32-bit positions");
    wnd_cfg cfg;
    const bool wide = sx_window_cfg(ti.maxc, cfg);
    if (!wide) return induce_typed<uint32_t>(ctx, ti, sigma, sorted_lms, seed_windows, false, SA, bwt_out, arena, cfg);
    return induce_typed<uint64_t>(ctx, ti, sigma, sorted_lms, seed_windows, seed_windows_u32, SA, bwt_out, arena, cfg);
}
```

### stralg_amd/csrc/sx_induce_chain.hpp

```cpp
#pragma once
#include "sx_induce_common.hpp"

namespace sx {

template <class WT, int BITS>
__global__ __launch_bounds__(kBlock) void induce_round_kernel(
    const uint32_t *__restrict__ srcP, const WT *__restrict__ srcW, const uint32_t *__restrict__ range_in,
    uint32_t *__restrict__ range_out, int rev, int mode, uint32_t c, wnd_cfg cfg, const uint8_t *__restrict__ T,
    const uint32_t *__restrict__ cursor_cur, uint32_t *__restrict__ cursor_nxt, int dir, uint32_t *__restrict__ SA,
    WT *__restrict__ WN, uint8_t *__restrict__ BW, uint32_t nkeys, uint64_t *__restrict__ status, uint32_t epoch,
    uint32_t *__restrict__ ticket,
    uint32_t chain_max ,
    int tail_follows ,
    int pass_large )
{
    __shared__ uint32_t wcount[kWavesPerBlock][256];
    __shared__ uint32_t gpos[256];
    __shared__ uint32_t gbase[256];
    __shared__ uint32_t tcount[256];
    __shared__ uint32_t s_tile;
    const int t = (int)threadIdx.x, lane = lane_id(), w = wave_id();
    const uint32_t lo = range_in[0], hi = range_in[1];
    const uint32_t len = hi - lo;
    if (len > chain_max && !pass_large) return;
    if (len == 0 || (range_out && tail_follows && len <= (BITS > 3 ? kTailMulti * kTailEntries : kTailEntries)) || len > chain_max) {
        if (blockIdx.x == 0) {
            cursor_nxt[t] = cursor_cur[t];
            if (t == 0 && range_out) {
                range_out[0] = len ? lo : hi;
                range_out[1] = hi;
            }
        }
        return;
    }
    const uint32_t ntiles = (len + kIndTile - 1) / kIndTile;
    gbase[t] = cursor_cur[t];
    for (;;) {
        if (t == 0) s_tile = atomicAdd(ticket, 1u);
        for (int i = t; i < kWavesPerBlock * 256; i += kBlock) (&wcount[0][0])[i] = 0;
        __syncthreads();
        const uint32_t tile = s_tile;
        if (tile >= ntiles) break;
        const uint32_t wave0 = tile * (uint32_t)kIndTile + (uint32_t)w * (kWave * kIndItems);
        uint32_t val[kIndItems], dig[kIndItems], rnk[kIndItems];
        WT wnd[kIndItems];
        bool ok[kIndItems];
#pragma unroll
        for (int k = 0; k < kIndItems; ++k) {
            const uint32_t i = wave0 + (uint32_t)k * kWave + lane;
            const uint32_t idx = lo + (i < len ? (rev ? len - 1u - i : i) : 0u);
            val[k] = srcP[idx];
            wnd[k] = srcW[idx];
        }
#pragma unroll
        for (int k = 0; k < kIndItems; ++k) {
            const uint32_t i = wave0 + (uint32_t)k * kWave + lane;
            const uint32_t p = i < len ? val[k] : 0u;
            const WT ww = wnd[k];
            ok[k] = false;
            dig[k] = 0;
            val[k] = 0;
            wnd[k] = 0;
            if (p != 0) {
                const uint32_t ch = wnd_first<WT>(ww, cfg);
                ok[k] = induce_accept(ch, c, mode);
                dig[k] = ch;
                val[k] = p - 1u;
                wnd[k] = wnd_pop<WT>(ww, cfg);
            }
        }
#pragma unroll
        for (int k = 0; k < kIndItems; ++k) rnk[k] = wave_rank_step<BITS>(dig[k], ok[k], wcount[w]);
        __syncthreads();
        {
            const uint32_t d = (uint32_t)t;
            uint32_t cnt = 0;
#pragma unroll
            for (int ww = 0; ww < kWavesPerBlock; ++ww) {
                const uint32_t x = wcount[ww][d];
                wcount[ww][d] = cnt;
                cnt += x;
            }
            uint32_t excl = 0;
            if (BITS > 3) {
                if (d < nkeys) excl = chain_exclusive_prefix(status, nkeys, tile, d, cnt, epoch);
                gpos[d] = excl;
                tcount[d] = cnt;
            } else {
                tcount[d] = cnt;
            }
        }
        if (BITS <= 3) {
            __syncthreads();
            for (uint32_t d = (uint32_t)w; d < nkeys; d += kWavesPerBlock) {
                const uint32_t excl = chain_exclusive_prefix_wave(status, nkeys, tile, d, tcount[d], epoch);
                if (lane == 0) gpos[d] = excl;
            }
        }
        __syncthreads();
        if (tile == ntiles - 1) {
            const uint32_t d = (uint32_t)t;
            const uint32_t total = (d < nkeys ? gpos[d] : 0u) + tcount[d], cur = gbase[d];
            cursor_nxt[d] = dir > 0 ? cur + total : cur - total;
            if (d == c && range_out) {
                range_out[0] = dir > 0 ? cur : cur - total;
                range_out[1] = dir > 0 ? cur + total : cur;
            }
        }
        __syncthreads();
        {
            bool need[kIndItems];
#pragma unroll
            for (int k = 0; k < kIndItems; ++k) need[k] = ok[k] && val[k] != 0 && wnd_count<WT>(wnd[k]) == 0;
            refill_windows<WT, kIndItems>(T, val, need, cfg, wnd);
        }
#pragma unroll
        for (int k = 0; k < kIndItems; ++k) {
            if (ok[k]) {
                const uint32_t d = dig[k];
                const uint32_t r = gpos[d] + wcount[w][d] + rnk[k];
                const uint32_t dst = dir > 0 ? gbase[d] + r : gbase[d] - 1u - r;
                const WT nw = wnd[k];
                SA[dst] = val[k];
                WN[dst] = nw;
                BW[dst] = wnd_symbol<WT>(nw, cfg);
            }
        }
        __syncthreads();
    }
}

struct tail_next {
    int c;
    uint32_t nk;
    const uint32_t *begin;
    const uint32_t *E;
    const uint32_t *tot;
    uint32_t *range;
    uint32_t *tickets;
    uint32_t ntickets;
    uint32_t *err;
};
template <class WT, int BITS>
__global__ __launch_bounds__(kTailBlock) void induce_tail_kernel(uint32_t *SA, WT *WN, uint8_t *BW, const uint32_t *__restrict__ range_in,
                                                             uint32_t *__restrict__ range_out, int rev, int mode,
                                                             uint32_t c, wnd_cfg cfg, const uint8_t *__restrict__ T,
                                                             const uint32_t *__restrict__ cursor_cur,
                                                             uint32_t *__restrict__ cursor_nxt, int dir,
                                                             uint32_t max_iters, uint32_t *poison, uint32_t *host_poison,
                                                             tail_next nb)
{
    constexpr int kDigits = BITS == 3 ? 8 : 256;
    __shared__ uint32_t wcount[kTailWaves][kDigits];
    __shared__ uint32_t gbase[256];
    __shared__ uint32_t s_range[2];
    __shared__ uint32_t s_flag;
    constexpr int kStageCap = BITS > 3 ? kTailTile : 1;
#ifndef SX_TAIL_STAGE_FROM
#define SX_TAIL_STAGE_FROM 512u
#endif
    constexpr uint32_t kStageFrom = SX_TAIL_STAGE_FROM;
    __shared__ WT st_w[kStageCap];
    __shared__ uint32_t st_v[kStageCap];
    __shared__ uint8_t st_d[kStageCap];
    __shared__ uint32_t st_off[BITS > 3 ? 256 : 1], st_ex[BITS > 3 ? 256 : 1], st_scan[kTailWaves];
    const int t = (int)threadIdx.x, lane = lane_id(), w = wave_id();
    if (t < 256) gbase[t] = cursor_cur[t];
    if (t == 0) {
        s_range[0] = range_in[0];
        s_range[1] = range_in[1];
    }
    for (int i = t; i < kTailWaves * kDigits; i += kTailBlock) (&wcount[0][0])[i] = 0;
    __syncthreads();
    uint32_t val[kIndItems];
    WT wnd[kIndItems];
    bool live[kIndItems];
    bool held = false;
    uint32_t prev_len = 0;
    const uint32_t wave0 = (uint32_t)w * (kWave * kIndItems);
    for (uint32_t it = 0; it < max_iters; ++it) {
        const uint32_t lo = s_range[0], len = s_range[1] - lo;
        if (len == 0 || len > (BITS == 3 ? kTailEntries : kTailMulti * kTailEntries)) break;
        const bool multi = len > kTailEntries;
        if ((mode == MODE_L_FROM_L || mode == MODE_S_FROM_S) && len == prev_len && !multi) {
            const uint32_t G = len <= (uint32_t)kTailBlock ? (uint32_t)kTailBlock / len : 1u;
            const uint64_t cpat = 0x0101010101010101ull * (uint64_t)c;
            uint32_t first_other = G;
            for (uint32_t e = (uint32_t)t; e < len * G; e += kTailBlock) {
                const uint32_t i = e / G, q = e % G;
                const uint32_t p = SA[lo + (rev ? len - 1u - i : i)];
                bool all_c = false;
                if (p >= 16u * (q + 1u)) {
                    uint64_t o0, o1;
                    load_bytes16(T, (uint64_t)(p - 16u * (q + 1u)), o0, o1);
                    all_c = o0 == cpat && o1 == cpat;
                }
                if (!all_c && q < first_other) first_other = q;
            }
            if (t == 0) s_flag = G;
            __syncthreads();
            if (first_other < G) atomicMin(&s_flag, first_other);
            __syncthreads();
            const uint32_t L = 16u * s_flag;
            __syncthreads();
            if (L) {
                const uint32_t cur = gbase[c], total = L * len;
                for (uint32_t o = (uint32_t)t; o < total; o += kTailBlock) {
// ... 132 lines not shown
        __syncthreads();
        }
        if ((uint32_t)t == c) {
            const uint32_t now = gbase[c];
            s_range[0] = dir > 0 ? c_first : now;
            s_range[1] = dir > 0 ? now : c_first;
        }
        __syncthreads();
    }
    uint32_t mine = t < 256 ? gbase[t] : 0u;
    if (nb.c >= 0) {
        if (t == 0) {
            s_flag = (s_range[0] != s_range[1] || (poison && poison[0])) ? 1u : 0u;
            for (uint32_t i = 0; i < nb.ntickets; ++i) nb.tickets[i] = 0;
        }
        __syncthreads();
        const uint32_t d = (uint32_t)t, cn = (uint32_t)nb.c;
        if (s_flag) {
            if (t == 0) nb.range[0] = nb.range[1] = 0;
        } else if (d < nb.nk && (dir > 0 ? d >= cn : d <= cn)) {
            uint32_t want, have = mine;
            if (dir > 0) {
                want = cn == 0 ? nb.begin[d] : nb.E[(uint64_t)(cn - 1) * 256 + d];
                for (uint32_t k = c; k < cn; ++k) have += nb.tot[(uint64_t)k * 256 + d];
            } else {
                want = cn + 1 >= nb.nk ? nb.begin[d + 1] : nb.E[(uint64_t)(cn + 1) * 256 + d];
                for (uint32_t k = c; k > cn; --k) have -= nb.tot[(uint64_t)k * 256 + d];
            }
            if (have != want) atomicOr(nb.err, dir > 0 ? 1u : 2u);
            mine = want;
            if (d == cn) {
                nb.range[0] = dir > 0 ? nb.begin[cn] : want;
                nb.range[1] = dir > 0 ? want : nb.begin[cn + 1];
            }
        }
    }
    if (t < 256) cursor_nxt[t] = mine;
    if (t == 0) {
        range_out[0] = s_range[0];
        range_out[1] = s_range[1];
        tail_report(s_range[0], s_range[1], c, poison, host_poison);
    }
}

constexpr uint32_t kRunProbe = 1u << 26;
constexpr uint32_t kRunEntries = 64;
constexpr uint32_t kRunProbeChunk = (uint32_t)kBlock * 16u;
constexpr uint32_t kRunProbeGrid = 256;
__global__ __launch_bounds__(kBlock) void run_probe_kernel(const uint8_t *__restrict__ T, const uint32_t *__restrict__ SA,
                                                          const uint32_t *__restrict__ range, uint32_t c, uint32_t from,
                                                          uint32_t look, uint32_t *__restrict__ run_len )
{
    const uint32_t lo = range[0], len = range[1] - lo;
    if (len == 0 || len > kRunEntries || blockIdx.y >= len) {
        if (blockIdx.x == 0 && blockIdx.y == 0 && threadIdx.x == 0 && (len == 0 || len > kRunEntries)) atomicMin(run_len, 0u);
        return;
    }
    const uint32_t p = SA[lo + blockIdx.y];
    for (uint32_t chunk0 = from + blockIdx.x * kRunProbeChunk; chunk0 < look; chunk0 += gridDim.x * kRunProbeChunk) {
        if (__hip_atomic_load(run_len, __ATOMIC_RELAXED, __HIP_MEMORY_SCOPE_AGENT) <= chunk0) return;
        const uint32_t d0 = chunk0 + threadIdx.x * 16u;
        if (d0 >= p) {
            if (d0 < p + 16u) atomicMin(run_len, p);
            continue;
        }
        const uint32_t cnt = p - d0 < 16u ? p - d0 : 16u;
        uint32_t first_other = cnt;
        for (uint32_t e = 0; e < cnt; ++e)
            if (T[p - d0 - 1u - e] != (uint8_t)c) {
                first_other = e;
                break;
            }
        if (first_other < 16u) atomicMin(run_len, d0 + first_other);
    }
}

__device__ __forceinline__ uint32_t run_length(const uint32_t *run_len, uint32_t len)
{
    if (len == 0 || len > kRunEntries) return 0;
    const uint32_t L = *run_len, most = kRunProbe / len;
    return L > most ? most : L;
}

template <class WT>
__global__ __launch_bounds__(kBlock) void run_fill_kernel(const uint8_t *__restrict__ T, uint32_t *SA, WT *__restrict__ WN,
                                                         uint8_t *__restrict__ BW, const uint32_t *__restrict__ range,
                                                         const uint32_t *__restrict__ cursor, uint32_t c, int rev, int dir,
                                                         wnd_cfg cfg, const uint32_t *__restrict__ run_len)
{
    const uint32_t lo = range[0], len = range[1] - lo;
    const uint64_t total = (uint64_t)run_length(run_len, len) * len;
    const uint32_t cur = cursor[c];
    for (uint64_t o = (uint64_t)blockIdx.x * kBlock + threadIdx.x; o < total; o += (uint64_t)gridDim.x * kBlock) {
        const uint32_t j = (uint32_t)(o / len) + 1u, i = (uint32_t)(o % len);
        const uint32_t v = SA[lo + (rev ? len - 1u - i : i)] - j;
        const uint32_t dst = dir > 0 ? cur + (uint32_t)o : cur - 1u - (uint32_t)o;
        const WT nw = v ? wnd_fill<WT>(T, v, cfg) : (WT)0;
        SA[dst] = v;
        WN[dst] = nw;
        BW[dst] = wnd_symbol<WT>(nw, cfg);
    }
}

__global__ void run_commit_kernel(uint32_t *__restrict__ range, uint32_t *__restrict__ cursor, uint32_t c, int dir,
                                  const uint32_t *__restrict__ run_len)
{
    if (threadIdx.x != 0 || blockIdx.x != 0) return;
    const uint32_t lo = range[0], len = range[1] - lo;
    const uint32_t total = run_length(run_len, len) * len;
    if (total == 0) return;
    const uint32_t cur = cursor[c];
    cursor[c] = dir > 0 ? cur + total : cur - total;
    range[0] = dir > 0 ? cur + total - len : cur - total;
    range[1] = range[0] + len;
}

__global__ void set_range_kernel(uint32_t *range, uint32_t lo, uint32_t hi, const uint32_t *cursor, int c, int which,
                                 uint32_t *tickets, uint32_t ntickets, const uint32_t *poison)
{
    if (threadIdx.x == 0 && blockIdx.x == 0) {
        for (uint32_t i = 0; i < ntickets; ++i) tickets[i] = 0;
        if (which == 1) hi = cursor[c];
        else if (which == 2) lo = cursor[c];
        if (poison && poison[0]) lo = hi = 0;
        range[0] = lo;
        range[1] = hi;
    }
}

__device__ __forceinline__ void tail_report(uint32_t lo, uint32_t hi, uint32_t c, uint32_t *poison, uint32_t *host_poison)
{
    if (!poison || lo == hi || poison[0]) return;
    poison[1] = c, poison[2] = lo, poison[3] = hi;
    poison[0] = 1;
    __hip_atomic_store(host_poison, 1u, __ATOMIC_RELAXED, __HIP_MEMORY_SCOPE_SYSTEM);
}

template <class WT>
__global__ __launch_bounds__(kBlock) void bwt_from_windows_kernel(const WT *__restrict__ WN, uint64_t N, wnd_cfg cfg,
                                                                  uint8_t *__restrict__ bwt)
{
    const uint64_t i0 = ((uint64_t)blockIdx.x * kBlock + threadIdx.x) * 16u;
    if (i0 >= N) return;
    if (i0 + 16u <= N && (((uintptr_t)WN | (uintptr_t)bwt) & 15u) == 0) {
        uint32_t out[4] = {0, 0, 0, 0};
#pragma unroll
        for (int q = 0; q < 4; ++q) {
            WT w[4];
            load_quad(WN + i0 + 4 * q, w);
#pragma unroll
            for (int e = 0; e < 4; ++e) {
                const uint32_t b = wnd_count<WT>(w[e]) == 0 ? 0u : wnd_first<WT>(w[e], cfg);
                out[q] |= (b & 0xFFu) << (8 * e);
            }
        }
        uint4 v;
        v.x = out[0], v.y = out[1], v.z = out[2], v.w = out[3];
        *reinterpret_cast<uint4 *>(bwt + i0) = v;
    } else {
        for (uint64_t i = i0; i < N && i < i0 + 16u; ++i) {
            const WT w = WN[i];
            bwt[i] = wnd_count<WT>(w) == 0 ? (uint8_t)0 : (uint8_t)wnd_first<WT>(w, cfg);
        }
    }
}

__global__ __launch_bounds__(kBlock) void widen_windows_kernel(const uint32_t *__restrict__ in, uint64_t count, uint64_t *__restrict__ out)
{
    const uint64_t i0 = ((uint64_t)blockIdx.x * kBlock + threadIdx.x) * 4u;
    if (i0 >= count) return;
    if (i0 + 4u <= count && (((uintptr_t)in | (uintptr_t)out) & 15u) == 0) {
        const uint4 v = *reinterpret_cast<const uint4 *>(in + i0);
        uint4 a, b;
        a.x = v.x, a.y = 0, a.z = v.y, a.w = 0;
        b.x = v.z, b.y = 0, b.z = v.w, b.w = 0;
        *reinterpret_cast<uint4 *>(out + i0) = a;
        *reinterpret_cast<uint4 *>(out + i0 + 2) = b;
    } else {
        for (uint64_t i = i0; i < count && i < i0 + 4u; ++i) out[i] = in[i];
    }
}

template <class WT>
__global__ void set_entry_kernel(uint32_t *SA, WT *WN, uint8_t *BW, uint32_t p, const uint8_t *T, wnd_cfg cfg)
{
    const WT w = p ? wnd_fill<WT>(T, p, cfg) : (WT)0;
    SA[0] = p;
    WN[0] = w;
    BW[0] = wnd_symbol<WT>(w, cfg);
}

}
```

### stralg_amd/csrc/sx_induce_common.hpp

```cpp
#pragma once
#include "sx_common.hpp"
#include "sx_device.hpp"
#include "sx_scan.hpp"
#include "sx_internal.hpp"
#include "sx_window.hpp"

namespace sx {

constexpr int kIndItems = 8;
constexpr int kIndTile = kBlock * kIndItems;
constexpr int kTailBlock = 1024, kTailWaves = kTailBlock / kWave;
constexpr int kTailTile = kTailBlock * kIndItems;
constexpr uint32_t kTailEntries = (uint32_t)kTailTile;
constexpr uint32_t kTailMulti = 4;

enum { MODE_L_FROM_L = 0, MODE_L_FROM_LMS = 1, MODE_S_FROM_S = 2, MODE_S_FROM_L = 3 };
__device__ __forceinline__ void tail_report(uint32_t lo, uint32_t hi, uint32_t c, uint32_t *poison, uint32_t *host_poison);

__device__ __forceinline__ bool induce_accept(uint32_t ch, uint32_t c, int mode)
{
    switch (mode) {
    case MODE_L_FROM_L: return ch >= c;
    case MODE_L_FROM_LMS: return true;
    case MODE_S_FROM_S: return ch <= c;
    default: return ch < c;
    }
}

template <class WT>
__global__ __launch_bounds__(kBlock) void fill_windows_kernel(const uint8_t *__restrict__ T,
                                                              const uint32_t *__restrict__ pos, uint64_t count,
                                                              wnd_cfg cfg, WT *__restrict__ out)
{
    const uint64_t k = (uint64_t)blockIdx.x * kBlock + threadIdx.x;
    if (k >= count) return;
    const uint32_t p = pos[k];
    out[k] = p ? wnd_fill<WT>(T, p, cfg) : (WT)0;
}

__device__ __forceinline__ void load_quad(const uint32_t *__restrict__ p, uint32_t (&o)[4])
{
    const uint4 v = *reinterpret_cast<const uint4 *>(p);
    o[0] = v.x, o[1] = v.y, o[2] = v.z, o[3] = v.w;
}
__device__ __forceinline__ void load_quad(const uint64_t *__restrict__ p, uint64_t (&o)[4])
{
    const uint4 v0 = *reinterpret_cast<const uint4 *>(p), v1 = *reinterpret_cast<const uint4 *>(p + 2);
    o[0] = pack64(v0.x, v0.y), o[1] = pack64(v0.z, v0.w), o[2] = pack64(v1.x, v1.y), o[3] = pack64(v1.z, v1.w);
}

}
```

### stralg_amd/csrc/sx_induce_small.hpp

```cpp
#pragma once
#include "sx_induce_common.hpp"

namespace sx {


__global__ __launch_bounds__(kBlock) void induce_count_bytes_kernel(const uint8_t *__restrict__ srcB,
                                                                    const uint32_t *__restrict__ range_in, int rev, int mode,
                                                                    uint32_t c, uint32_t *__restrict__ hist, uint32_t stride,
                                                                    uint32_t nkeys, uint32_t chain_max, uint64_t src_len)
{
    const uint32_t lo = range_in[0], len = range_in[1] - lo;
    if (len <= chain_max) return;
    const uint32_t ntiles = (len + kIndTile - 1) / kIndTile;
    const bool aligned = ((uintptr_t)srcB & 15u) == 0;
    {
        constexpr int kPieces = kIndTile / 16 / kWave + 1;
        const int lane = lane_id();
        for (uint32_t tile = blockIdx.x * kWavesPerBlock + wave_id(); tile < ntiles; tile += gridDim.x * kWavesPerBlock) {
            const uint32_t tile0 = tile * (uint32_t)kIndTile;
            const uint32_t cnt = len - tile0 < (uint32_t)kIndTile ? len - tile0 : (uint32_t)kIndTile;
            const uint32_t a = rev ? lo + len - tile0 - cnt : lo + tile0, b = a + cnt;
            uint32_t S[kPieces][4], inside[kPieces];
#pragma unroll
            for (int k = 0; k < kPieces; ++k) {
// ... 46 lines not shown
    if (len <= chain_max) return;
    const uint32_t ntiles = (len + kIndTile - 1) / kIndTile;
    const bool aligned = ((uintptr_t)srcW & 15u) == 0;
    (void)srcB;
    {
        constexpr int kQuads = kIndTile / 4 / kWave + 1;
        const int lane = lane_id();
        for (uint32_t tile = blockIdx.x * kWavesPerBlock + wave_id(); tile < ntiles; tile += gridDim.x * kWavesPerBlock) {
            const uint32_t tile0 = tile * (uint32_t)kIndTile;
            const uint32_t cnt = len - tile0 < (uint32_t)kIndTile ? len - tile0 : (uint32_t)kIndTile;
            const uint32_t a = rev ? lo + len - tile0 - cnt : lo + tile0, b = a + cnt;
            const bool whole = aligned && ((uint64_t)(a >> 2) + (uint64_t)kQuads * kWave) * 4u <= src_len;
            uint64_t packed = 0;
            constexpr int kHalf = (kQuads + 1) / 2;
#pragma unroll 1
            for (int h = 0; h < 2; ++h) {
                WT W[kHalf][4];
                uint32_t inside[kHalf];
#pragma unroll
                for (int kk = 0; kk < kHalf; ++kk) {
                    const int k = h * kHalf + kk;
                    const uint64_t e0 = ((uint64_t)(a >> 2) + (uint64_t)lane + (uint64_t)k * kWave) * 4u;
                    const uint32_t from = e0 < a ? (uint32_t)(a - e0) : 0u, to = e0 >= b ? 0u : (b - e0 < 4u ? (uint32_t)(b - e0) : 4u);
                    inside[kk] = (k < kQuads && from < to) ? ((1u << to) - 1u) & ~((1u << from) - 1u) : 0u;
                    W[kk][0] = W[kk][1] = W[kk][2] = W[kk][3] = 0;
                    if (whole) {
                        if (k < kQuads) load_quad(srcW + e0, W[kk]);
                    } else {
#pragma unroll
                        for (int e = 0; e < 4; ++e)
                            if ((inside[kk] >> e) & 1u) W[kk][e] = srcW[e0 + e];
                    }
                }
#pragma unroll
                for (int kk = 0; kk < kHalf; ++kk) {
#pragma unroll
                    for (int e = 0; e < 4; ++e) {
                        const uint32_t ch = wnd_first<WT>(W[kk][e], cfg) & 7u;
                        const bool ok = ((inside[kk] >> e) & 1u) && wnd_count<WT>(W[kk][e]) != 0 && induce_accept(ch, c, mode);
                        packed += (uint64_t)(ok ? 1u : 0u) << (8u * ch);
                    }
                }
            }
            uint64_t even = packed & 0x00FF00FF00FF00FFull, odd = (packed >> 8) & 0x00FF00FF00FF00FFull;
            even = wave_total_packed(even);
            odd = wave_total_packed(odd);
            if ((uint32_t)lane < nkeys && lane < 8)
                hist[(uint64_t)lane * stride + tile] = (uint32_t)(((lane & 1) ? odd : even) >> (16 * (lane >> 1))) & 0xFFFFu;
        }
        return;
    }
}

__global__ __launch_bounds__(kRowThreads) void induce_offsets_kernel(uint32_t *__restrict__ hist, uint32_t stride,
                                                                const uint32_t *__restrict__ range_in,
                                                                uint32_t *__restrict__ range_out,
                                                                const uint32_t *__restrict__ cursor_cur,
                                                                uint32_t *__restrict__ cursor_nxt, int dir, uint32_t c,
                                                                uint32_t chain_max,
                                                                int only_form )
{
    __shared__ uint32_t lds[kRowPieces * kRowWaves];
    const uint32_t len = range_in[1] - range_in[0];
    if (len <= chain_max) {
        if (only_form && threadIdx.x == 0) {
            cursor_nxt[blockIdx.x] = cursor_cur[blockIdx.x];
            if (blockIdx.x == c && range_out) range_out[0] = range_out[1] = range_in[1];
        }
        return;
    }
    const uint32_t ntiles = (len + kIndTile - 1) / kIndTile;
    const uint32_t key = blockIdx.x;
    const uint32_t total = wide_scan_row_inplace(hist + (uint64_t)key * stride, ntiles, lds);
    if (threadIdx.x == 0) {
        const uint32_t cur = cursor_cur[key];
        cursor_nxt[key] = dir > 0 ? cur + total : cur - total;
        if (key == c && range_out) {
            range_out[0] = dir > 0 ? cur : cur - total;
            range_out[1] = dir > 0 ? cur + total : cur;
        }
    }
}

template <class WT, int MODE>
__global__ __launch_bounds__(kBlock) void induce_scatter_small_kernel(
    const uint32_t *__restrict__ srcP, const WT *__restrict__ srcW, const uint32_t *__restrict__ range_in, uint32_t c,
    wnd_cfg cfg, const uint8_t *__restrict__ T, const uint32_t *__restrict__ offs, uint32_t stride,
    const uint32_t *__restrict__ cursor_cur, uint32_t *__restrict__ SA, WT *__restrict__ WN, uint8_t *__restrict__ BW,
    uint32_t nkeys, uint32_t chain_max)
{
    constexpr bool kRev = MODE == MODE_S_FROM_S || MODE == MODE_S_FROM_L;
    constexpr uint64_t kField16 = 0x00FF00FF00FF00FFull;
    __shared__ uint64_t wsum[2][kWavesPerBlock];
    __shared__ uint64_t sbase[2];
    __shared__ uint32_t gadj[8];
    __shared__ uint32_t sP[kIndTile];
    __shared__ WT sW[kIndTile];
    __shared__ uint8_t sD[kIndTile];
    __shared__ uint16_t refill[kIndTile];
    __shared__ uint32_t nrefill;
    const int t = (int)threadIdx.x, lane = lane_id(), w = wave_id();
    const uint32_t lo = range_in[0], len = range_in[1] - lo;
    if (len <= chain_max) return;
    const uint32_t ntiles = (len + kIndTile - 1) / kIndTile;
    const uint32_t base_d = t < (int)nkeys ? cursor_cur[t] : 0u;
    for (uint32_t tile = blockIdx.x; tile < ntiles; tile += gridDim.x) {
        const uint32_t pre = t < (int)nkeys ? offs[(uint64_t)t * stride + tile] : 0u;
        if (t == 0) nrefill = 0;
        const uint32_t i0 = tile * (uint32_t)kIndTile + (uint32_t)t * kIndItems;
        uint32_t P[kIndItems];
        WT W[kIndItems];
        if (i0 + kIndItems <= len) {
            const uint32_t first = kRev ? lo + len - i0 - kIndItems : lo + i0;
            uint32_t Pm[kIndItems];
            WT Wm[kIndItems];
            __builtin_memcpy(Pm, srcP + first, sizeof(Pm));
            __builtin_memcpy(Wm, srcW + first, sizeof(Wm));
#pragma unroll
            for (int k = 0; k < kIndItems; ++k) {
                P[k] = Pm[kRev ? kIndItems - 1 - k : k];
                W[k] = Wm[kRev ? kIndItems - 1 - k : k];
            }
        } else {
#pragma unroll
            for (int k = 0; k < kIndItems; ++k) {
                const uint32_t i = i0 + (uint32_t)k;
                const uint32_t idx = i < len ? (kRev ? lo + len - 1u - i : lo + i) : lo;
                P[k] = i < len ? srcP[idx] : 0u;
                W[k] = i < len ? srcW[idx] : (WT)0;
            }
        }
        uint32_t rnk[kIndItems], dig[kIndItems];
        bool ok[kIndItems];
        uint64_t cnt = 0;
#pragma unroll
        for (int k = 0; k < kIndItems; ++k) {
            const uint32_t ch = wnd_first<WT>(W[k], cfg) & 7u;
            ok[k] = P[k] != 0 && induce_accept(ch, c, MODE);
            dig[k] = ch;
            rnk[k] = (uint32_t)(cnt >> (8u * ch)) & 0xFFu;
            cnt += (uint64_t)(ok[k] ? 1u : 0u) << (8u * ch);
        }
        const uint64_t own0 = cnt & kField16, own1 = (cnt >> 8) & kField16;
        const uint64_t inc0 = wave_inclusive_sum_packed(own0), inc1 = wave_inclusive_sum_packed(own1);
        if (lane == kWave - 1) wsum[0][w] = inc0, wsum[1][w] = inc1;
        __syncthreads();
        uint64_t ex0 = inc0 - own0, ex1 = inc1 - own1, tot0 = 0, tot1 = 0;
#pragma unroll
        for (int i = 0; i < kWavesPerBlock; ++i) {
            const uint64_t x0 = wsum[0][i], x1 = wsum[1][i];
            if (i < w) ex0 += x0, ex1 += x1;
            tot0 += x0, tot1 += x1;
        }
        if (t < 8) {
            uint32_t first_slot = 0;
            for (int d = 0; d < t; ++d) first_slot += (uint32_t)(((d & 1) ? tot1 : tot0) >> (16 * (d >> 1))) & 0xFFFFu;
            const uint32_t g = kRev ? base_d - 1u - pre : base_d + pre;
            gadj[t] = kRev ? g + first_slot : g - first_slot;
        }
        if (t == 0) {
            uint64_t even = 0, odd = 0;
            uint32_t run = 0;
#pragma unroll
            for (int d = 0; d < 8; ++d) {
                if (d & 1) odd |= (uint64_t)run << (16 * (d >> 1));
                else even |= (uint64_t)run << (16 * (d >> 1));
                run += (uint32_t)(((d & 1) ? tot1 : tot0) >> (16 * (d >> 1))) & 0xFFFFu;
            }
            sbase[0] = even, sbase[1] = odd;
        }
        __syncthreads();
        ex0 += sbase[0];
        ex1 += sbase[1];
        const uint32_t produced = (uint32_t)((tot0 & 0xFFFFu) + ((tot0 >> 16) & 0xFFFFu) + ((tot0 >> 32) & 0xFFFFu) + (tot0 >> 48) +
                                             (tot1 & 0xFFFFu) + ((tot1 >> 16) & 0xFFFFu) + ((tot1 >> 32) & 0xFFFFu) + (tot1 >> 48));
#pragma unroll
        for (int k = 0; k < kIndItems; ++k) {
            if (ok[k]) {
                const uint32_t d = dig[k];
                const uint32_t slot = ((uint32_t)(((d & 1u) ? ex1 : ex0) >> (16u * (d >> 1))) & 0xFFFFu) + rnk[k];
                const uint32_t j = P[k] - 1u;
                const WT nw = wnd_pop<WT>(W[k], cfg);
                sP[slot] = j;
                sW[slot] = nw;
                sD[slot] = (uint8_t)d;
                if (j != 0 && wnd_count<WT>(nw) == 0) refill[atomicAdd(&nrefill, 1u)] = (uint16_t)slot;
            }
        }
        __syncthreads();
        const uint32_t nre = nrefill;
        if (nre) {
            for (uint32_t r = (uint32_t)t; r < nre; r += kBlock) {
                const uint32_t slot = refill[r];
                sW[slot] = wnd_fill<WT>(T, sP[slot], cfg);
            }
            __syncthreads();
        }
#pragma unroll
        for (int k = 0; k < kIndItems; ++k) {
            const uint32_t i = (uint32_t)t + (uint32_t)k * kBlock;
            if (i < produced) {
                const uint32_t g = gadj[sD[i]];
                const uint32_t dst = kRev ? g - i : g + i;
                const WT nw = sW[i];
                SA[dst] = sP[i];
                WN[dst] = nw;
                BW[dst] = wnd_symbol<WT>(nw, cfg);
            }
        }
        __syncthreads();
    }
}

constexpr int kTailBatch = 8;
constexpr uint32_t kRunCap = 255;
#ifndef SX_TAIL_CLOSED_FROM
#define SX_TAIL_CLOSED_FROM 256u
#endif
constexpr uint32_t kClosedFrom = SX_TAIL_CLOSED_FROM;
constexpr uint32_t kClosedEntries = 5120;
template <class WT>
__global__ __launch_bounds__(kTailBlock) void induce_tail_small_kernel(uint32_t *SA, WT *WN, uint8_t *BW,
                                                                       const uint32_t *__restrict__ range_in,
                                                                       uint32_t *__restrict__ range_out, int rev, int mode,
                                                                       uint32_t c, wnd_cfg cfg, const uint8_t *__restrict__ T,
                                                                       const uint32_t *__restrict__ cursor_cur,
                                                                       uint32_t *__restrict__ cursor_nxt, int dir,
                                                                       uint32_t max_iters, uint32_t *poison, uint32_t *host_poison)
{
    constexpr uint64_t kField16 = 0x00FF00FF00FF00FFull;
    __shared__ uint64_t wsum[kTailBatch][2][kTailWaves];
    __shared__ uint32_t s_tot[kTailBatch][8], s_base[kTailBatch][8];
    __shared__ uint32_t gbase[8];
    __shared__ uint32_t s_range[2];
    __shared__ uint32_t s_flag;
    constexpr uint32_t kCfEntries = sizeof(WT) == 4 ? kClosedEntries : 64u;
    __shared__ uint32_t cf_p[kCfEntries];
    __shared__ WT cf_w[kCfEntries];
    __shared__ uint8_t cf_r[kCfEntries];
    __shared__ uint32_t cf_hr[kRunCap + 1], cf_he[8][kRunCap + 1], cf_scan[kTailWaves], cf_rmax;
    const int t = (int)threadIdx.x, lane = lane_id(), w = wave_id();
    if (t < 8) gbase[t] = cursor_cur[t];
    if (t == 0) {
        s_range[0] = range_in[0];
        s_range[1] = range_in[1];
    }
    __syncthreads();
    const uint32_t B = cfg.B, cmask = cfg.mask;
    bool last_batch = false;
    uint32_t val[kIndItems];
    WT wnd[kIndItems];
    uint32_t live = 0;
    uint32_t per = kIndItems;
    bool held = false;
    uint32_t prev_len = 0, last_in = ~0u;
    for (uint32_t it = 0; it < max_iters;) {
        const uint32_t lo = s_range[0], len = s_range[1] - lo;
        if (len == 0 || len > kTailEntries) break;
        if (len == prev_len) {
            const uint32_t G = len <= (uint32_t)kTailBlock ? (uint32_t)kTailBlock / len : 1u;
            const uint64_t cpat = 0x0101010101010101ull * (uint64_t)c;
            uint32_t first_other = G;
            for (uint32_t e = (uint32_t)t; e < len * G; e += kTailBlock) {
                const uint32_t i = e / G, q = e % G;
                const uint32_t p = SA[lo + (rev ? len - 1u - i : i)];
                bool all_c = false;
                if (p >= 16u * (q + 1u)) {
                    uint64_t o0, o1;
                    load_bytes16(T, (uint64_t)(p - 16u * (q + 1u)), o0, o1);
                    all_c = o0 == cpat && o1 == cpat;
                }
                if (!all_c && q < first_other) first_other = q;
            }
            if (t == 0) s_flag = G;
            __syncthreads();
            if (first_other < G) atomicMin(&s_flag, first_other);
            __syncthreads();
            const uint32_t L = 16u * s_flag;
            __syncthreads();
            if (L) {
                const uint32_t cur = gbase[c], total = L * len;
                for (uint32_t o = (uint32_t)t; o < total; o += kTailBlock) {
                    const uint32_t j = o / len + 1u, i = o % len;
                    const uint32_t v = SA[lo + (rev ? len - 1u - i : i)] - j;
                    const uint32_t dst = dir > 0 ? cur + o : cur - 1u - o;
                    const WT nw = v ? wnd_fill<WT>(T, v, cfg) : (WT)0;
                    SA[dst] = v;
                    WN[dst] = nw;
                    BW[dst] = wnd_symbol<WT>(nw, cfg);
                }
                __syncthreads();
                if ((uint32_t)t == c) {
                    gbase[c] = dir > 0 ? cur + total : cur - total;
                    s_range[0] = dir > 0 ? cur + total - len : cur - total;
                    s_range[1] = dir > 0 ? cur + total : cur - total + len;
                }
                held = false;
                last_batch = false;
                ++it;
                __syncthreads();
                continue;
            }
        }
        prev_len = len;
        if ((mode == MODE_L_FROM_L || mode == MODE_S_FROM_S) && c >= 1u && last_batch && (uint64_t)len * 2 >= last_in &&
            len >= kClosedFrom && len <= kCfEntries) {
            if (t <= (int)kRunCap) cf_hr[t] = 0;
            for (uint32_t i = (uint32_t)t; i < (kRunCap + 1) * 8; i += kTailBlock) (&cf_he[0][0])[i] = 0;
            __syncthreads();
            const uint64_t cpat = 0x0101010101010101ull * (uint64_t)c;
            const uint32_t per2 = (len + (uint32_t)kTailBlock - 1u) / (uint32_t)kTailBlock;
#pragma unroll 1
            for (uint32_t k = 0; k < per2; ++k) {
                const uint32_t i = (uint32_t)t * per2 + k;
                if (i < len) {
                    const uint32_t p = SA[lo + (rev ? len - 1u - i : i)];
                    uint32_t r = 0;
                    bool open = p != 0;
                    for (uint32_t g = 0; g < (kRunCap + 1) / 64 && open; ++g) {
                        uint64_t o[4][2];
#pragma unroll
                        for (uint32_t u = 0; u < 4; ++u) {
                            const uint32_t done = 64u * g + 16u * u;
                            o[u][0] = o[u][1] = ~cpat;
                            if (p >= done + 16u) load_bytes16(T, (uint64_t)(p - done - 16u), o[u][0], o[u][1]);
                        }
#pragma unroll
                        for (uint32_t u = 0; u < 4; ++u) {
                            const uint32_t done = 64u * g + 16u * u;
                            if (!open) {
                            } else if (p >= done + 16u) {
                                const uint64_t x1 = o[u][1] ^ cpat, x0 = o[u][0] ^ cpat;
                                if (x1) r += (uint32_t)__clzll((unsigned long long)x1) >> 3, open = false;
                                else if (x0) r += 8u + ((uint32_t)__clzll((unsigned long long)x0) >> 3), open = false;
                                else r += 16u;
                            } else {
                                uint32_t a = p - done;
                                while (a > 0 && T[a - 1u] == (uint8_t)c) --a, ++r;
                                open = false;
                            }
                        }
                    }
                    if (r > kRunCap) r = kRunCap;
                    const WT wend = p > r ? wnd_fill<WT>(T, p - r, cfg) : (WT)0;
                    cf_p[i] = p;
                    cf_r[i] = (uint8_t)r;
                    cf_w[i] = wend;
                    atomicAdd(&cf_hr[r], 1u);
                    if (r < kRunCap && p > r) {
                        const uint32_t d = wnd_first<WT>(wend, cfg);
                        if (induce_accept(d, c, mode)) atomicAdd(&cf_he[d & 7u][r], 1u);
                    }
                }
            }
            __syncthreads();
            if (w <= 8) {
                uint32_t *row = w == 0 ? cf_hr : cf_he[w - 1];
                uint32_t v[4], sum = 0, top = 0;
#pragma unroll
                for (int q = 0; q < 4; ++q) {
                    v[q] = row[4 * lane + q];
                    if (v[q]) top = (uint32_t)(4 * lane + q);
                    sum += v[q];
                }
                uint32_t inc = wave_inclusive_scan<OpAdd>(sum);
                if (w == 0) {
                    const uint32_t rmax = wave_reduce_max(top);
                    if (lane == 0) cf_rmax = rmax;
                    uint32_t run = inc - sum, s4[4], ssum = 0;
#pragma unroll
                    for (int q = 0; q < 4; ++q) {
// ... 7 lines not shown
                    for (int q = 0; q < 4; ++q) {
                        row[4 * lane + q] = run2;
                        run2 += s4[q];
                    }
                } else {
                    uint32_t run = inc - sum;
#pragma unroll
                    for (int q = 0; q < 4; ++q) {
                        row[4 * lane + q] = run;
                        run += v[q];
                    }
                }
            }
            __syncthreads();
            const uint32_t rmax = cf_rmax;
            const uint32_t J = rmax < kRunCap ? rmax + 1u : kRunCap;
            const uint32_t curC = gbase[c];
            uint32_t curD[8];
#pragma unroll
            for (int d = 0; d < 8; ++d) curD[d] = gbase[d];
            WT crun = 0;
            for (uint32_t i = 0; i < cfg.CW; ++i) crun = (crun << B) | (WT)(c - 1u);
            const WT field_mask = cfg.CW * B >= 8 * sizeof(WT) ? ~(WT)0 : (((WT)1 << (cfg.CW * B)) - 1u);
            uint32_t cur_len = len;
            for (uint32_t e0 = 0; e0 < J; e0 += (uint32_t)kTailWaves) {
            if (e0 > 0) {
                const uint32_t alive = cf_hr[e0] - cf_hr[e0 - 1u];
                if ((uint64_t)alive * 8 <= (uint64_t)cur_len * 7) {
                    constexpr uint32_t kPerC = (kCfEntries + (uint32_t)kTailBlock - 1u) / (uint32_t)kTailBlock;
                    const uint32_t perc = (cur_len + (uint32_t)kTailBlock - 1u) / (uint32_t)kTailBlock;
                    uint32_t kp[kPerC], kr[kPerC], keep = 0, cnt = 0;
                    WT kw[kPerC];
#pragma unroll
                    for (uint32_t k = 0; k < kPerC; ++k) {
                        const uint32_t i = (uint32_t)t * perc + k;
                        kp[k] = 0, kr[k] = 0, kw[k] = 0;
                        if (k < perc && i < cur_len) {
                            kp[k] = cf_p[i], kr[k] = cf_r[i], kw[k] = cf_w[i];
                            if (kr[k] >= e0) keep |= 1u << k, ++cnt;
                        }
                    }
                    const uint32_t inc = wave_inclusive_scan<OpAdd>(cnt);
                    if (lane == kWave - 1) cf_scan[w] = inc;
                    __syncthreads();
                    uint32_t at = inc - cnt;
                    for (int ww = 0; ww < w; ++ww) at += cf_scan[ww];
#pragma unroll
                    for (uint32_t k = 0; k < kPerC; ++k) {
                        if ((keep >> k) & 1u) {
                            cf_p[at] = kp[k], cf_r[at] = (uint8_t)kr[k], cf_w[at] = kw[k];
                            ++at;
                        }
                    }
                    cur_len = alive;
                    __syncthreads();
                }
            }
            const uint32_t nchunks = (cur_len + (uint32_t)kWave - 1u) / (uint32_t)kWave;
            const uint32_t j = e0 + 1u + (uint32_t)w;
            if (j <= J) {
                uint32_t cc = cf_hr[j - 1u], cd[8];
#pragma unroll
                for (int d = 0; d < 8; ++d) cd[d] = cf_he[d][j - 1u];
                for (uint32_t ch = 0; ch < nchunks; ++ch) {
                    const uint32_t i = ch * (uint32_t)kWave + (uint32_t)lane;
                    const bool valid = i < cur_len;
                    const uint32_t r = valid ? cf_r[i] : 0u, p = valid ? cf_p[i] : 0u;
                    const WT wend = valid ? cf_w[i] : (WT)0;
                    const uint32_t dd = wnd_first<WT>(wend, cfg);
                    const bool cont = valid && r >= j;
                    const bool endf = valid && r + 1u == j && r < kRunCap && p > r && induce_accept(dd, c, mode);
                    const uint64_t bc = __ballot(cont ? 1 : 0);
                    if (bc) {
                        if (cont) {
                            const uint32_t o = cc + (uint32_t)__popcll(bc & lanemask_lt());
                            const uint32_t dst = dir > 0 ? curC + o : curC - 1u - o, pos = p - j;
                            const uint32_t k = r - j, have = k + wnd_count<WT>(wend);
                            WT nw = 0;
                            if (pos != 0) {
                                const WT codes = k >= cfg.CW ? crun : ((crun & (((WT)1 << (k * B)) - 1u)) | ((wend >> kCntBits) << (k * B))) & field_mask;
                                nw = (codes << kCntBits) | (WT)(have < cfg.CW ? have : cfg.CW);
                            }
                            SA[dst] = pos;
                            WN[dst] = nw;
                            BW[dst] = wnd_symbol<WT>(nw, cfg);
                        }
                        cc += (uint32_t)__popcll(bc);
                    }
                    const uint64_t be = __ballot(endf ? 1 : 0);
                    if (be) {
#pragma unroll
                        for (int d = 1; d < 8; ++d) {
                            const bool mine = endf && dd == (uint32_t)d;
                            const uint64_t bd = __ballot(mine ? 1 : 0);
                            if (bd) {
                                if (mine) {
                                    const uint32_t o = cd[d] + (uint32_t)__popcll(bd & lanemask_lt());
                                    const uint32_t dst = dir > 0 ? curD[d] + o : curD[d] - 1u - o, pos = p - j;
                                    const WT nw = pos == 0 ? (WT)0 : wnd_pop<WT>(wend, cfg);
                                    SA[dst] = pos;
                                    WN[dst] = nw;
                                    BW[dst] = wnd_symbol<WT>(nw, cfg);
                                }
                                cd[d] += (uint32_t)__popcll(bd);
                            }
                        }
                    }
                }
            }
            __syncthreads();
            }
            if (t < 8) {
                const uint32_t tot = (uint32_t)t == c ? cf_hr[kRunCap] : cf_he[t][kRunCap];
                const uint32_t before = gbase[t];
                gbase[t] = dir > 0 ? before + tot : before - tot;
                if ((uint32_t)t == c) {
                    const uint32_t from = rmax < kRunCap ? tot : cf_hr[kRunCap - 1u];
                    s_range[0] = dir > 0 ? before + from : before - tot;
                    s_range[1] = dir > 0 ? before + tot : before - from;
                }
            }
            held = false;
            last_batch = true;
            last_in = len;
            it += J;
            __syncthreads();
            continue;
        }
        if (!held) {
            live = 0;
            per = (len + (uint32_t)kTailBlock - 1u) / (uint32_t)kTailBlock;
#pragma unroll
            for (int k = 0; k < kIndItems; ++k) {
                const uint32_t i = (uint32_t)t * per + (uint32_t)k;
                val[k] = 0;
                wnd[k] = 0;
                if ((uint32_t)k < per && i < len) {
                    const uint32_t idx = lo + (rev ? len - 1u - i : i);
                    val[k] = SA[idx];
                    wnd[k] = WN[idx];
                    live |= 1u << k;
                }
            }
            held = true;
        }
        const uint32_t nr = (uint64_t)len * 8 >= last_in ? (uint32_t)kTailBatch : 1u;
        last_in = len;
        last_batch = nr > 1;
        if (nr > 1) {
            WT fresh[kIndItems];
            uint32_t dry = 0;
#pragma unroll
            for (int k = 0; k < kIndItems; ++k) {
                fresh[k] = 0;
                if ((uint32_t)k < per && ((live >> k) & 1u) && val[k] != 0) {
                    const uint32_t need = val[k] < (uint32_t)(kTailBatch + 1) ? val[k] : (uint32_t)(kTailBatch + 1);
                    if (wnd_count<WT>(wnd[k]) < need) {
                        dry |= 1u << k;
                        fresh[k] = wnd_fill<WT>(T, val[k], cfg);
                    }
                }
            }
#pragma unroll
            for (int k = 0; k < kIndItems; ++k)
                if ((dry >> k) & 1u) wnd[k] = fresh[k];
        }
        const bool wave_live = __any(live != 0u ? 1 : 0);
        uint64_t cnt[kTailBatch];
        uint32_t emask[kIndItems];
        uint32_t alive_after = 0;
        uint64_t ex0[kTailBatch], ex1[kTailBatch];
#pragma unroll
        for (int j = 0; j < kTailBatch; ++j) cnt[j] = 0, ex0[j] = 0, ex1[j] = 0;
#pragma unroll
        for (int k = 0; k < kIndItems; ++k) emask[k] = 0;
        if (wave_live) {
#pragma unroll
            for (int k = 0; k < kIndItems; ++k) {
                if ((uint32_t)k >= per) break;
                bool alive = (live >> k) & 1u;
                const WT codes = wnd[k] >> kCntBits;
#pragma unroll
                for (int j = 0; j < kTailBatch; ++j) {
                    if ((uint32_t)j < nr) {
                        const uint32_t sym = ((uint32_t)(codes >> (j * B)) & cmask) + 1u;
                        const bool ok = alive && val[k] > (uint32_t)j && induce_accept(sym, c, mode);
                        if (ok) {
                            const uint32_t sh = 8u * (sym & 7u);
                            emask[k] |= (1u << j) | (((uint32_t)(cnt[j] >> sh) & 7u) << (8 + 3 * j));
                            cnt[j] += 1ull << sh;
                        }
                        alive = ok && sym == c;
                    }
                }
                if (alive) alive_after |= 1u << k;
            }
#pragma unroll
            for (int j = 0; j < kTailBatch; ++j) {
                if ((uint32_t)j < nr) {
                    const uint64_t own0 = cnt[j] & kField16, own1 = (cnt[j] >> 8) & kField16;
                    const uint64_t inc0 = wave_inclusive_sum_packed(own0), inc1 = wave_inclusive_sum_packed(own1);
                    if (lane == kWave - 1) wsum[j][0][w] = inc0, wsum[j][1][w] = inc1;
                    ex0[j] = inc0 - own0, ex1[j] = inc1 - own1;
                }
            }
        } else if (lane < kTailBatch * 2) {
            wsum[lane >> 1][lane & 1][w] = 0;
        }
        __syncthreads();
        if (t < kTailBatch * 2 * kTailWaves) {
            const int j = t / (2 * kTailWaves), h = (t / kTailWaves) & 1, ww = t % kTailWaves;
            static_assert(kTailWaves == 16, "a (round, half) is scanned by a 16-lane segment");
            const uint64_t own = (uint32_t)j < nr ? wsum[j][h][ww] : 0ull;
            const uint64_t inc = row_inclusive_sum_packed(own);
            if ((uint32_t)j < nr) {
                wsum[j][h][ww] = inc - own;
                if (ww == kTailWaves - 1) {
#pragma unroll
                    for (int f = 0; f < 4; ++f) s_tot[j][2 * f + h] = (uint32_t)(inc >> (16 * f)) & 0xFFFFu;
                }
            }
        }
        __syncthreads();
        if (t < 8) {
            uint32_t b = gbase[t];
#pragma unroll
            for (int j = 0; j < kTailBatch; ++j) {
                if ((uint32_t)j < nr) {
                    s_base[j][t] = b;
                    b = dir > 0 ? b + s_tot[j][t] : b - s_tot[j][t];
                }
            }
            gbase[t] = b;
            if ((uint32_t)t == c) {
                const uint32_t sb = s_base[nr - 1u][t], n_last = s_tot[nr - 1u][t];
                s_range[0] = dir > 0 ? sb : sb - n_last;
                s_range[1] = dir > 0 ? sb + n_last : sb;
            }
        }
        __syncthreads();
        uint32_t live_next = 0;
        if (wave_live) {
#pragma unroll
        for (int j = 0; j < kTailBatch; ++j)
            if ((uint32_t)j < nr) ex0[j] += wsum[j][0][w], ex1[j] += wsum[j][1][w];
#pragma unroll
        for (int k = 0; k < kIndItems; ++k) {
            if ((uint32_t)k >= per) break;
            const WT codes = wnd[k] >> kCntBits;
            const uint32_t wcnt = wnd_count<WT>(wnd[k]);
#pragma unroll
            for (int j = 0; j < kTailBatch; ++j) {
                if ((uint32_t)j < nr && ((emask[k] >> j) & 1u)) {
                    const uint32_t d = (((uint32_t)(codes >> (j * B)) & cmask) + 1u) & 7u;
                    const uint64_t exw = (d & 1u) ? ex1[j] : ex0[j];
                    const uint32_t r = ((uint32_t)(exw >> (16u * (d >> 1))) & 0xFFFFu) + ((emask[k] >> (8 + 3 * j)) & 7u);
                    const uint32_t sb = s_base[j][d];
                    const uint32_t dst = dir > 0 ? sb + r : sb - 1u - r;
                    const uint32_t pos = val[k] - (uint32_t)(j + 1);
                    WT nw = (((codes >> (j * B)) >> B) << kCntBits) | (WT)(wcnt - (uint32_t)(j + 1));
                    if (pos != 0 && wcnt == (uint32_t)(j + 1)) nw = wnd_fill<WT>(T, pos, cfg);
                    SA[dst] = pos;
                    WN[dst] = nw;
                    BW[dst] = wnd_symbol<WT>(nw, cfg);
                    if ((uint32_t)j == nr - 1u && ((alive_after >> k) & 1u)) {
                        live_next |= 1u << k;
                        val[k] = pos;
                        wnd[k] = nw;
                    }
                }
            }
        }
        }
        live = live_next;
        it += nr;
        __syncthreads();
    }
    if (t < 8) cursor_nxt[t] = gbase[t];
    if (t == 0) {
        range_out[0] = s_range[0];
        range_out[1] = s_range[1];
        tail_report(s_range[0], s_range[1], c, poison, host_poison);
    }
}

constexpr int kBatchRounds = 8;
constexpr int kBatchRows = kBatchRounds * 8;
#ifndef SX_BATCH_FROM
#define SX_BATCH_FROM (1u << 21)
#endif
constexpr uint32_t kBatchFrom = SX_BATCH_FROM;

template <class WT> struct batch_plan {
    uint32_t a;
    uint32_t tsym;
    bool term;
};

__device__ __forceinline__ uint32_t batch_field_of(uint32_t bit, uint32_t B)
{
    return B == 2 ? bit >> 1 : (B == 1 ? bit : (B == 3 ? (bit * 171u) >> 9 : bit >> 2));
}

template <class WT, int MODE>
__device__ __forceinline__ batch_plan<WT> batch_chain(WT &w, uint32_t p, uint32_t c, const wnd_cfg &cfg, WT cpat,
                                                        const uint8_t *__restrict__ T)
{
    batch_plan<WT> pl;
    uint32_t cntw = wnd_count<WT>(w);
    WT x = (w >> kCntBits) ^ cpat;
    uint32_t r = x ? batch_field_of((uint32_t)(sizeof(WT) == 8 ? __builtin_ctzll((unsigned long long)x) : __builtin_ctz((uint32_t)x)), cfg.B)
                   : cfg.CW;
    if (r >= cntw && cntw <= (uint32_t)kBatchRounds && p > cntw) {
        w = wnd_fill<WT>(T, p, cfg);
        cntw = wnd_count<WT>(w);
        x = (w >> kCntBits) ^ cpat;
        r = x ? batch_field_of((uint32_t)(sizeof(WT) == 8 ? __builtin_ctzll((unsigned long long)x) : __builtin_ctz((uint32_t)x)), cfg.B)
              : cfg.CW;
    }
    uint32_t a = r < cntw ? r : cntw;
    pl.term = a < (uint32_t)kBatchRounds && a < cntw;
    if (a > (uint32_t)kBatchRounds) a = (uint32_t)kBatchRounds;
    pl.a = a;
    pl.tsym = ((uint32_t)((w >> kCntBits) >> (a * cfg.B)) & cfg.mask) + 1u;
    pl.term = pl.term && induce_accept(pl.tsym, c, MODE) && pl.tsym < 8u;
    return pl;
}

template <class WT>
__device__ __forceinline__ WT batch_window(WT w, uint32_t depth, uint32_t pos, const wnd_cfg &cfg, const uint8_t *__restrict__ T)
{
    const uint32_t cntw = wnd_count<WT>(w);
    WT nw = ((((w >> kCntBits) >> (depth * cfg.B)) >> cfg.B) << kCntBits) | (WT)(cntw - (depth + 1u));
    if (pos != 0 && cntw == depth + 1u) nw = wnd_fill<WT>(T, pos, cfg);
    return nw;
}

template <class WT> __device__ __forceinline__ WT batch_cpat(uint32_t c, const wnd_cfg &cfg)
{
    WT pat = 0;
    for (uint32_t i = 0; i < cfg.CW; ++i) pat |= (WT)(c - 1u) << (i * cfg.B);
    return pat;
}

template <class WT, bool kRev, bool kWantP>
__device__ __forceinline__ void batch_load(const uint32_t *__restrict__ srcP, const WT *__restrict__ srcW, uint32_t lo, uint32_t len,
                                           uint32_t i0, uint32_t (&P)[kIndItems], WT (&W)[kIndItems])
{
    if (i0 + kIndItems <= len) {
        const uint32_t first = kRev ? lo + len - i0 - kIndItems : lo + i0;
        uint32_t Pm[kIndItems];
        WT Wm[kIndItems];
        if (kWantP) __builtin_memcpy(Pm, srcP + first, sizeof(Pm));
        __builtin_memcpy(Wm, srcW + first, sizeof(Wm));
#pragma unroll
        for (int k = 0; k < kIndItems; ++k) {
            P[k] = kWantP ? Pm[kRev ? kIndItems - 1 - k : k] : 0u;
            W[k] = Wm[kRev ? kIndItems - 1 - k : k];
        }
    } else {
#pragma unroll
        for (int k = 0; k < kIndItems; ++k) {
            const uint32_t i = i0 + (uint32_t)k;
            const uint32_t idx = i < len ? (kRev ? lo + len - 1u - i : lo + i) : lo;
            P[k] = (kWantP && i < len) ? srcP[idx] : 0u;
            W[k] = i < len ? srcW[idx] : (WT)0;
        }
    }
}

template <class WT, int MODE>
__device__ __forceinline__ void batch_tally(const batch_plan<WT> &pl, uint32_t c, uint64_t (&cnt)[kBatchRounds])
{
#pragma unroll
    for (int j = 0; j < kBatchRounds; ++j) {
        const uint64_t self = (uint32_t)j < pl.a ? 1ull << (8u * c) : 0ull;
        const uint64_t term = (pl.term && pl.a == (uint32_t)j) ? 1ull << (8u * pl.tsym) : 0ull;
        cnt[j] += self + term;
    }
}

template <class WT, int MODE>
__global__ __launch_bounds__(kBlock) void induce_batch_count_kernel(const uint32_t *__restrict__ srcP, const WT *__restrict__ srcW,
                                                                    const uint32_t *__restrict__ range_in, uint32_t c, wnd_cfg cfg,
                                                                    const uint8_t *__restrict__ T, uint32_t *__restrict__ hist ,
                                                                    uint32_t stride, uint32_t min_len)
{
    constexpr bool kRev = MODE == MODE_S_FROM_S;
    constexpr uint64_t kField16 = 0x00FF00FF00FF00FFull;
    __shared__ uint64_t wtot[kBatchRounds][2][kWavesPerBlock];
    const int t = (int)threadIdx.x, lane = lane_id(), w = wave_id();
    const uint32_t lo = range_in[0], len = range_in[1] - lo;
    if (len <= min_len) return;
    const uint32_t ntiles = (len + kIndTile - 1) / kIndTile;
    const WT cpat = batch_cpat<WT>(c, cfg);
    for (uint32_t tile = blockIdx.x; tile < ntiles; tile += gridDim.x) {
        const uint32_t i0 = tile * (uint32_t)kIndTile + (uint32_t)t * kIndItems;
        uint32_t P[kIndItems];
        WT W[kIndItems];
        batch_load<WT, kRev, false>(srcP, srcW, lo, len, i0, P, W);
        uint64_t cnt[kBatchRounds];
#pragma unroll
        for (int j = 0; j < kBatchRounds; ++j) cnt[j] = 0;
#pragma unroll
        for (int k = 0; k < kIndItems; ++k) {
            const uint32_t cntw = wnd_count<WT>(W[k]);
            uint32_t p = cntw;
            if (cntw != 0 && cntw <= (uint32_t)kBatchRounds) {
                const WT x = (W[k] >> kCntBits) ^ cpat;
                const WT low = cntw * cfg.B >= sizeof(WT) * 8 ? ~(WT)0 : (((WT)1 << (cntw * cfg.B)) - 1);
                if ((x & low) == 0) {
                    const uint32_t i = i0 + (uint32_t)k;
                    p = srcP[kRev ? lo + len - 1u - i : lo + i];
                }
            }
            const batch_plan<WT> pl = batch_chain<WT, MODE>(W[k], p, c, cfg, cpat, T);
            batch_tally<WT, MODE>(pl, c, cnt);
        }
#pragma unroll
        for (int j = 0; j < kBatchRounds; ++j) {
            const uint64_t e = wave_total_packed(cnt[j] & kField16), o = wave_total_packed((cnt[j] >> 8) & kField16);
            if (lane == 0) wtot[j][0][w] = e, wtot[j][1][w] = o;
        }
        __syncthreads();
        if (t < kBatchRows) {
            const int j = t >> 3, d = t & 7;
            uint64_t sum = 0;
#pragma unroll
            for (int ww = 0; ww < kWavesPerBlock; ++ww) sum += wtot[j][d & 1][ww];
            hist[(uint64_t)t * stride + tile] = (uint32_t)(sum >> (16 * (d >> 1))) & 0xFFFFu;
        }
        __syncthreads();
    }
}

__global__ __launch_bounds__(kRowThreads) void induce_batch_offsets_kernel(uint32_t *__restrict__ hist, uint32_t stride,
                                                                      const uint32_t *__restrict__ range_in,
                                                                      uint32_t *__restrict__ totals, uint32_t nk, uint32_t min_len)
{
    __shared__ uint32_t lds[kRowPieces * kRowWaves];
    const uint32_t len = range_in[1] - range_in[0];
    if (len <= min_len) return;
    const uint32_t ntiles = (len + kIndTile - 1) / kIndTile;
    const uint32_t row = (blockIdx.x / nk) * 8u + blockIdx.x % nk;
    const uint32_t total = wide_scan_row_inplace(hist + (uint64_t)row * stride, ntiles, lds);
    if (threadIdx.x == 0) totals[row] = total;
}

template <class WT, int MODE>
__global__ __launch_bounds__(kBlock, 2) void induce_batch_scatter_kernel(
    const uint32_t *__restrict__ srcP, const WT *__restrict__ srcW, const uint32_t *__restrict__ range_in,
    uint32_t *__restrict__ range_out, uint32_t c, wnd_cfg cfg, const uint8_t *__restrict__ T, const uint32_t *__restrict__ offs,
    uint32_t stride, const uint32_t *__restrict__ totals, const uint32_t *__restrict__ cursor_cur, uint32_t *__restrict__ cursor_nxt,
    uint32_t *__restrict__ SA, WT *__restrict__ WN, uint8_t *__restrict__ BW, uint32_t nk, uint32_t min_len)
{
    constexpr bool kRev = MODE == MODE_S_FROM_S;
    constexpr uint64_t kField16 = 0x00FF00FF00FF00FFull;
    __shared__ uint64_t wsum[kBatchRounds][2][kWavesPerBlock];
    __shared__ uint32_t s_round0[kBatchRows];
    __shared__ uint32_t s_base[kBatchRows];
    const int t = (int)threadIdx.x, lane = lane_id(), w = wave_id();
    const uint32_t lo = range_in[0], hi = range_in[1], len = hi - lo;
    if (len <= min_len) {
        if (blockIdx.x == 0) {
            if (t < 256) cursor_nxt[t] = cursor_cur[t];
            if (t == 0 && range_out) range_out[0] = lo, range_out[1] = hi;
        }
        return;
    }
    const uint32_t ntiles = (len + kIndTile - 1) / kIndTile;
    __shared__ uint32_t s_tot[kBatchRows];
    if (t < kBatchRows) s_tot[t] = (uint32_t)(t & 7) < nk ? totals[t] : 0u;
    __syncthreads();
    if (t < kBatchRows) {
        const int j = t >> 3, d = t & 7;
        uint32_t before = 0;
        for (int jj = 0; jj < j; ++jj) before += s_tot[jj * 8 + d];
        s_round0[t] = before;
    }
    __syncthreads();
    if (blockIdx.x == 0 && t < 256) {
        uint32_t all = 0;
        if ((uint32_t)t < nk) all = s_round0[(kBatchRounds - 1) * 8 + t] + s_tot[(kBatchRounds - 1) * 8 + t];
        const uint32_t cur = cursor_cur[t];
        cursor_nxt[t] = kRev ? cur - all : cur + all;
        if ((uint32_t)t == c && range_out) {
            const uint32_t last = s_tot[(kBatchRounds - 1) * 8 + t];
            range_out[0] = kRev ? cur - all : cur + all - last;
            range_out[1] = kRev ? cur - all + last : cur + all;
        }
    }
    const uint32_t base_d = (uint32_t)(t & 7) < nk && t < kBatchRows ? cursor_cur[t & 7] : 0u;
    const WT cpat = batch_cpat<WT>(c, cfg);
    for (uint32_t tile = blockIdx.x; tile < ntiles; tile += gridDim.x) {
        if (t < kBatchRows) {
            const uint32_t rel = s_round0[t] + (((uint32_t)(t & 7) < nk) ? offs[(uint64_t)t * stride + tile] : 0u);
            s_base[t] = kRev ? base_d - 1u - rel : base_d + rel;
        }
        const uint32_t i0 = tile * (uint32_t)kIndTile + (uint32_t)t * kIndItems;
        uint32_t P[kIndItems];
        WT W[kIndItems];
        batch_load<WT, kRev, true>(srcP, srcW, lo, len, i0, P, W);
        batch_plan<WT> pl[kIndItems];
        uint64_t cnt[kBatchRounds];
#pragma unroll
        for (int j = 0; j < kBatchRounds; ++j) cnt[j] = 0;
#pragma unroll
        for (int k = 0; k < kIndItems; ++k) {
            pl[k] = batch_chain<WT, MODE>(W[k], P[k], c, cfg, cpat, T);
            batch_tally<WT, MODE>(pl[k], c, cnt);
        }
        uint64_t ex0[kBatchRounds], ex1[kBatchRounds];
#pragma unroll
        for (int j = 0; j < kBatchRounds; ++j) {
            const uint64_t own0 = cnt[j] & kField16, own1 = (cnt[j] >> 8) & kField16;
            const uint64_t inc0 = wave_inclusive_sum_packed(own0), inc1 = wave_inclusive_sum_packed(own1);
            if (lane == kWave - 1) wsum[j][0][w] = inc0, wsum[j][1][w] = inc1;
            ex0[j] = inc0 - own0, ex1[j] = inc1 - own1;
        }
        __syncthreads();
#pragma unroll
        for (int j = 0; j < kBatchRounds; ++j) {
#pragma unroll
            for (int ww = 0; ww < kWavesPerBlock; ++ww)
                if (ww < w) ex0[j] += wsum[j][0][ww], ex1[j] += wsum[j][1][ww];
        }
        uint64_t run[kBatchRounds];
#pragma unroll
        for (int j = 0; j < kBatchRounds; ++j) run[j] = 0;
#pragma unroll
        for (int k = 0; k < kIndItems; ++k) {
#pragma unroll
            for (int j = 0; j < kBatchRounds; ++j) {
                const bool self = (uint32_t)j < pl[k].a, term = pl[k].term && pl[k].a == (uint32_t)j;
                if (self || term) {
                    const uint32_t d = self ? c : pl[k].tsym;
                    const uint64_t exw = (d & 1u) ? ex1[j] : ex0[j];
                    const uint32_t r = ((uint32_t)(exw >> (16u * (d >> 1))) & 0xFFFFu) + ((uint32_t)(run[j] >> (8u * d)) & 0xFFu);
                    const uint32_t sb = s_base[j * 8 + (int)d];
                    const uint32_t dst = kRev ? sb - r : sb + r;
                    const uint32_t pos = P[k] - (uint32_t)(j + 1);
                    const WT nw = batch_window<WT>(W[k], (uint32_t)j, pos, cfg, T);
                    SA[dst] = pos;
                    WN[dst] = nw;
                    BW[dst] = wnd_symbol<WT>(nw, cfg);
                    run[j] += 1ull << (8u * d);
                }
            }
        }
        __syncthreads();
    }
}

}
```

### stralg_amd/csrc/sx_window.hpp

```cpp
#pragma once
#include "sx_common.hpp"
#include "sx_device.hpp"

namespace sx {

constexpr int kCntBits = 4;
struct wnd_cfg {
    uint32_t B;
    uint32_t CW;
    uint32_t mask;
};

template <class WT> __device__ __forceinline__ uint32_t wnd_count(WT w) { return (uint32_t)(w & (WT)15); }
template <class WT> __device__ __forceinline__ uint32_t wnd_first(WT w, const wnd_cfg &c)
{
    return (uint32_t)((w >> kCntBits) & (WT)c.mask) + 1u;
}
template <class WT> __device__ __forceinline__ uint8_t wnd_symbol(WT w, const wnd_cfg &c)
{
    return (uint8_t)(wnd_count<WT>(w) ? wnd_first<WT>(w, c) : 0u);
}
template <class WT> __device__ __forceinline__ WT wnd_pop(WT w, const wnd_cfg &c)
{
    const WT cnt = w & (WT)15;
    return (((w >> kCntBits) >> c.B) << kCntBits) | (cnt - 1);
}
template <class WT>
__device__ __forceinline__ WT wnd_from_bytes(uint64_t lo, uint64_t hi, uint32_t cnt, const wnd_cfg &c)
{
    WT acc = 0;
    if (cnt == c.CW && c.B <= 2) {
        const uint32_t w[4] = {(uint32_t)lo, (uint32_t)(lo >> 32), (uint32_t)hi, (uint32_t)(hi >> 32)};
        const uint32_t nw = c.CW >> 2, r = c.CW & 3u;
        const uint32_t coef4 = (1u << 24) | (1u << (16 + c.B)) | (1u << (8 + 2 * c.B)) | (1u << (3 * c.B));
        uint32_t a = 0, bias = 0;
#pragma unroll
        for (uint32_t j = 0; j < 4; ++j) {
            if (j < nw) a = __builtin_amdgcn_udot4(w[j], coef4, a << (4 * c.B), false);
            else if (j == nw && r) a = __builtin_amdgcn_udot4(w[j], coef4 >> (8 * (4 - r)), a << (r * c.B), false);
        }
        for (uint32_t i = 0; i < c.CW; ++i) bias |= 1u << (c.B * i);
        return (WT)(((a - bias) << kCntBits) | cnt);
    }
    if (cnt == c.CW) {
#pragma unroll
        for (uint32_t i = 0; i < 15; ++i) {
            if (i < c.CW) {
                const uint64_t byte = ((i < 8 ? lo : hi) >> (8u * (i & 7u))) & 0xFFull;
                acc = (acc << c.B) | (WT)(byte - 1u);
            }
        }
    } else {
#pragma unroll
        for (uint32_t i = 0; i < 15; ++i) {
            if (i < cnt) {
                const uint64_t byte = ((i < 8 ? lo : hi) >> (8u * (i & 7u))) & 0xFFull;
                acc = (acc << c.B) | (WT)(byte - 1u);
            }
        }
    }
    return (acc << kCntBits) | (WT)cnt;
}

template <class WT>
__device__ __forceinline__ WT wnd_fill(const uint8_t *__restrict__ T, uint32_t p, const wnd_cfg &c)
{
    const uint32_t cnt = p < c.CW ? p : c.CW;
    uint64_t lo, hi;
    load_bytes16(T, (uint64_t)(p - cnt), lo, hi);
    return wnd_from_bytes<WT>(lo, hi, cnt, c);
}

template <class WT>
__device__ __forceinline__ WT wnd_fill_lds(const uint8_t *img, uint64_t origin, uint32_t p, const wnd_cfg &c)
{
    const uint32_t cnt = p < c.CW ? p : c.CW;
    uint64_t lo, hi;
    lds_bytes16(img, (uint32_t)((uint64_t)(p - cnt) - origin), lo, hi);
    return wnd_from_bytes<WT>(lo, hi, cnt, c);
}

}

static inline bool sx_window_cfg(uint32_t maxc, sx::wnd_cfg &cfg)
{
    cfg.B = (uint32_t)sx_bitlen(maxc > 0 ? maxc - 1 : 0);
    if (cfg.B < 1) cfg.B = 1;
    cfg.mask = (1u << cfg.B) - 1u;
    const bool wide = cfg.B > 4;
    cfg.CW = ((wide ? 64u : 32u) - (uint32_t)sx::kCntBits) / cfg.B;
    if (cfg.CW > 15) cfg.CW = 15;
    return wide;
}
```

Baseline: 53310 Msuffixes/s.

## Add optional 16-bit stored induce windows to halve window-array traffic

Introduces a template storage type for the per-entry window array in induced sorting, so 32-bit working windows can be stored in 16 bits when the symbol width is small. Stores truncate the window to 12 code bits with a clamped count, and loads widen back to the working type. The small-alphabet kernels are templated on the storage type, and the paths for large alphabets are disabled in narrow mode. The mode is selected through a new flag that defaults to 0, which appears to keep 32-bit storage.

```diff
diff --git a/include/stralg_amd.h b/include/stralg_amd.h
--- a/include/stralg_amd.h
+++ b/include/stralg_amd.h
@@ -69,6 +69,7 @@
     uint32_t recursion_levels;
     uint32_t sample_tied_permille;
     uint32_t long_subbuckets;
+    uint32_t window_bits;
 } sx_build_stats;
 
 int sx_device_count(void);
@@ -98,6 +99,7 @@
     ,SX_FLAG_LOCAL_SORT_LEAN_OFF = 17
     ,SX_FLAG_SAM_BATCH_READS = 18
     ,SX_FLAG_SAM_WINDOW_BYTES = 19
+    ,SX_FLAG_INDUCE_WINDOW_BITS = 20
 };
 int sx_ctx_set_flag(sx_ctx *ctx, int flag, int value);
 
diff --git a/stralg_amd/_lib.py b/stralg_amd/_lib.py
--- a/stralg_amd/_lib.py
+++ b/stralg_amd/_lib.py
@@ -19,7 +19,8 @@
                 ("doubling_rounds", C.c_uint32), ("induce_rounds", C.c_uint32),
                 ("sort_passes", C.c_uint32), ("lms_path", C.c_uint32), ("sort_local", C.c_uint32), ("refine_tiers", C.c_uint32),
                 ("ms_total", C.c_double), ("induce_redo", C.c_uint32), ("long_runs", C.c_uint32),
-                ("recursion_levels", C.c_uint32), ("sample_tied_permille", C.c_uint32), ("long_subbuckets", C.c_uint32)]
+                ("recursion_levels", C.c_uint32), ("sample_tied_permille", C.c_uint32), ("long_subbuckets", C.c_uint32),
+                ("window_bits", C.c_uint32)]
 
     def as_dict(self):
         return {k: getattr(self, k) for k, _ in self._fields_}
diff --git a/stralg_amd/api.py b/stralg_amd/api.py
--- a/stralg_amd/api.py
+++ b/stralg_amd/api.py
@@ -323,6 +323,9 @@
 
     def set_induce_batch(self, on=True):
         self._check(self.lib.sx_ctx_set_flag(self.h, 7, 0 if on else 1), "sx_ctx_set_flag")
+
+    def set_induce_window_bits(self, bits=0):
+        self._check(self.lib.sx_ctx_set_flag(self.h, 20, int(bits)), "sx_ctx_set_flag")
 
     def set_induce_batch_min(self, entries):
         self._check(self.lib.sx_ctx_set_flag(self.h, 8, int(entries)), "sx_ctx_set_flag")
diff --git a/stralg_amd/csrc/sx_common.hpp b/stralg_amd/csrc/sx_common.hpp
--- a/stralg_amd/csrc/sx_common.hpp
+++ b/stralg_amd/csrc/sx_common.hpp
@@ -72,6 +72,7 @@
     int radix_digit_bits = 0;
     int sort_mode = 0;
     int induce_batch_off = 0;
+    int induce_window_bits = 0;
     int induce_attended = 0;
     int induce_no_hoist = 0;
     int text_keys_off = 0;
diff --git a/stralg_amd/csrc/sx_ctx.hip b/stralg_amd/csrc/sx_ctx.hip
--- a/stralg_amd/csrc/sx_ctx.hip
+++ b/stralg_amd/csrc/sx_ctx.hip
@@ -199,6 +199,7 @@
     c->radix_digit_bits = ctx->radix_digit_bits;
     c->sort_mode = ctx->sort_mode;
     c->induce_batch_off = ctx->induce_batch_off;
+    c->induce_window_bits = ctx->induce_window_bits;
     c->induce_batch_min = ctx->induce_batch_min;
     c->induce_attended = ctx->induce_attended;
     c->induce_no_hoist = ctx->induce_no_hoist;
@@ -393,6 +394,11 @@
         ctx->induce_no_hoist = value ? 1 : 0;
         return 0;
     }
+    if (flag == SX_FLAG_INDUCE_WINDOW_BITS) {
+        if (value != 0 && value != 16 && value != 32) return SX_E_ARG;
+        ctx->induce_window_bits = value;
+        return 0;
+    }
     if (flag == SX_FLAG_INDUCE_BATCH_MIN) {
         ctx->induce_batch_min = value < 0 ? -1 : (int64_t)value;
         return 0;
diff --git a/stralg_amd/csrc/sx_induce.hip b/stralg_amd/csrc/sx_induce.hip
--- a/stralg_amd/csrc/sx_induce.hip
+++ b/stralg_amd/csrc/sx_induce.hip
@@ -22,11 +22,12 @@
 constexpr uint32_t kInduceGridCap = SX_INDUCE_GRID_CAP;
 constexpr int kMaxSpec = 16;
 
-template <class WT> struct induce_state {
+template <class WT, class ST> struct induce_state {
+    static constexpr bool kNarrow = sizeof(ST) != sizeof(WT);
     sx_ctx *ctx;
     const uint8_t *T;
     uint32_t *SA;
-    WT *WN;
+    ST *WN;
     uint64_t N, m;
     uint8_t *BW;
     uint32_t *cursor[2];
@@ -59,8 +60,8 @@
     int begun_c;
 };
 
-template <class WT>
-void launch_round(induce_state<WT> &st, const uint32_t *srcP, const WT *srcW, int range_slot, int out_slot,
+template <class WT, class ST>
+void launch_round(induce_state<WT, ST> &st, const uint32_t *srcP, const WT *seedW , const ST *arrW , int range_slot, int out_slot,
                   uint32_t tiles_bound, uint32_t tiles_likely, int rev, int mode, uint32_t c, int dir, int tail_follows,
                   int chained_only_up_to_chain_max = 0, int three_launch_only = 0)
 {
@@ -83,13 +84,13 @@
             sx_launch(ctx, SX_KC_INDUCE_GATHER, 0, induce_count_bytes_kernel, dim3(grid), dim3(kBlock), srcB, (const uint32_t *)rin, rev,
                       mode, c, st.hist, st.stride, st.nk, chain_max, src_len);
         else
-            sx_launch(ctx, SX_KC_INDUCE_GATHER, 0, induce_count_kernel<WT, 3>, dim3(grid), dim3(kBlock), srcW, srcB,
+            sx_launch(ctx, SX_KC_INDUCE_GATHER, 0, induce_count_kernel<WT, 3>, dim3(grid), dim3(kBlock), seedW, srcB,
                       (const uint32_t *)rin, rev, mode, c, st.cfg, st.hist, st.stride, st.nk, chain_max, src_len);
         sx_launch(ctx, SX_KC_INDUCE_SCAN, (uint64_t)tiles_bound * st.nk * 8, induce_offsets_kernel, dim3(st.nk),
                   dim3(kRowThreads), st.hist, st.stride, (const uint32_t *)rin, rout, cur, nxt, dir, c, chain_max, only3 ? 1 : 0);
         {
 #define SX_SCATTER_SMALL(M)                                                                                            \
-    sx_launch(ctx, SX_KC_INDUCE_SCATTER, 0, induce_scatter_small_kernel<WT, M>, dim3(grid), dim3(kBlock), srcP, srcW, \
+    sx_launch(ctx, SX_KC_INDUCE_SCATTER, 0, induce_scatter_small_kernel<WT, M, ST>, dim3(grid), dim3(kBlock), srcP, seedW, arrW, \
               (const uint32_t *)rin, c, st.cfg, st.T, (const uint32_t *)st.hist, st.stride, cur, st.SA, st.WN, st.BW, st.nk, \
               chain_max)
             switch (mode) {
@@ -101,8 +102,9 @@
 #undef SX_SCATTER_SMALL
         }
     }
-    if (both && !st.small_alphabet) {
+    if constexpr (!induce_state<WT, ST>::kNarrow) if (both && !st.small_alphabet) {
         const uint8_t *srcB = srcP == st.SA ? (const uint8_t *)st.BW : nullptr;
+        const WT *srcW = seedW ? seedW : (const WT *)arrW;
         const uint32_t wtiles = sx_div_up((uint64_t)(tiles_bound < 1 ? 1 : tiles_bound) * kIndTile, kWideTile);
         const uint32_t wgrid = wtiles > 2048 ? 2048 : wtiles;
         const int only = only3 ? 1 : 0;
@@ -127,15 +129,16 @@
     uint32_t cgrid = grid > 1024 ? 1024 : grid;
     if (only3) {
     } else if (st.small_alphabet)
-        sx_launch(ctx, SX_KC_INDUCE_CHAIN, 0, induce_round_kernel<WT, 3>, dim3(cgrid), dim3(kBlock), srcP, srcW,
+        sx_launch(ctx, SX_KC_INDUCE_CHAIN, 0, induce_round_kernel<WT, 3, ST>, dim3(cgrid), dim3(kBlock), srcP, seedW, arrW,
                   (const uint32_t *)rin, rout, rev, mode, c, st.cfg, st.T, cur, nxt, dir, st.SA, st.WN, st.BW, st.nk, st.status,
                   epoch, st.tickets + range_slot, chain_max, tail_follows, pass_large);
-    else if (st.nk <= 32)
-        sx_launch(ctx, SX_KC_INDUCE_CHAIN, 0, induce_round_kernel<WT, 5>, dim3(cgrid), dim3(kBlock), srcP, srcW,
+    else if constexpr (induce_state<WT, ST>::kNarrow) {
+    } else if (st.nk <= 32)
+        sx_launch(ctx, SX_KC_INDUCE_CHAIN, 0, induce_round_kernel<WT, 5>, dim3(cgrid), dim3(kBlock), srcP, seedW, arrW,
                   (const uint32_t *)rin, rout, rev, mode, c, st.cfg, st.T, cur, nxt, dir, st.SA, st.WN, st.BW, st.nk, st.status,
                   epoch, st.tickets + range_slot, chain_max, tail_follows, pass_large);
     else
-        sx_launch(ctx, SX_KC_INDUCE_CHAIN, 0, induce_round_kernel<WT, 8>, dim3(cgrid), dim3(kBlock), srcP, srcW,
+        sx_launch(ctx, SX_KC_INDUCE_CHAIN, 0, induce_round_kernel<WT, 8>, dim3(cgrid), dim3(kBlock), srcP, seedW, arrW,
                   (const uint32_t *)rin, rout, rev, mode, c, st.cfg, st.T, cur, nxt, dir, st.SA, st.WN, st.BW, st.nk, st.status,
                   epoch, st.tickets + range_slot, chain_max, tail_follows, pass_large);
     st.par ^= 1;
@@ -146,18 +149,18 @@
 #define SX_TAIL_ITERS_UNATTENDED 1024u
 #endif
 constexpr uint32_t kTailIters = 64, kTailItersUnattended = SX_TAIL_ITERS_UNATTENDED;
-template <class WT>
-void launch_tail(induce_state<WT> &st, int range_slot, int out_slot, int rev, int mode, uint32_t c, int dir)
+template <class WT, class ST>
+void launch_tail(induce_state<WT, ST> &st, int range_slot, int out_slot, int rev, int mode, uint32_t c, int dir)
 {
     sx_ctx *ctx = st.ctx;
     const uint32_t *cur = st.cursor[st.par];
     uint32_t *nxt = st.cursor[st.par ^ 1];
     if (st.small_alphabet)
-        sx_launch(ctx, SX_KC_INDUCE_CHAIN, 0, induce_tail_small_kernel<WT>, dim3(1), dim3(kTailBlock), st.SA, st.WN, st.BW,
+        sx_launch(ctx, SX_KC_INDUCE_CHAIN, 0, induce_tail_small_kernel<WT, ST>, dim3(1), dim3(kTailBlock), st.SA, st.WN, st.BW,
                   (const uint32_t *)(st.ranges + 2 * range_slot), st.ranges + 2 * out_slot, rev, mode, c, st.cfg, st.T,
                   cur, nxt, dir, st.unattended ? kTailItersUnattended : kTailIters, st.unattended ? st.poison : (uint32_t *)nullptr,
                   st.host_poison);
-    else {
+    else if constexpr (!induce_state<WT, ST>::kNarrow) {
         tail_next nb = {-1, st.nk, nullptr, nullptr, nullptr, nullptr, nullptr, 0u, nullptr};
         if (st.hoist && st.unattended && st.next_c >= 0)
             nb = {st.next_c, st.nk, (const uint32_t *)st.d_begin, (const uint32_t *)st.hoist_E, (const uint32_t *)st.hoist_tot, st.ranges,
@@ -171,8 +174,8 @@
     st.par ^= 1;
 }
 
-template <class WT>
-void launch_batch(induce_state<WT> &st, int range_slot, int out_slot, uint32_t tiles_bound, int mode, uint32_t c)
+template <class WT, class ST>
+void launch_batch(induce_state<WT, ST> &st, int range_slot, int out_slot, uint32_t tiles_bound, int mode, uint32_t c)
 {
     sx_ctx *ctx = st.ctx;
     uint32_t grid = tiles_bound < 1 ? 1 : tiles_bound;
@@ -183,29 +186,29 @@
     uint32_t *nxt = st.cursor[st.par ^ 1];
     const uint32_t min_len = ctx->induce_batch_min >= 0 ? (uint32_t)ctx->induce_batch_min : kTailEntries;
     if (mode == MODE_L_FROM_L) {
-        sx_launch(ctx, SX_KC_INDUCE_GATHER, 0, induce_batch_count_kernel<WT, MODE_L_FROM_L>, dim3(grid), dim3(kBlock),
-                  (const uint32_t *)st.SA, (const WT *)st.WN, rin, c, st.cfg, st.T, st.bhist, st.stride, min_len);
+        sx_launch(ctx, SX_KC_INDUCE_GATHER, 0, induce_batch_count_kernel<WT, MODE_L_FROM_L, ST>, dim3(grid), dim3(kBlock),
+                  (const uint32_t *)st.SA, (const ST *)st.WN, rin, c, st.cfg, st.T, st.bhist, st.stride, min_len);
     } else {
-        sx_launch(ctx, SX_KC_INDUCE_GATHER, 0, induce_batch_count_kernel<WT, MODE_S_FROM_S>, dim3(grid), dim3(kBlock),
-                  (const uint32_t *)st.SA, (const WT *)st.WN, rin, c, st.cfg, st.T, st.bhist, st.stride, min_len);
+        sx_launch(ctx, SX_KC_INDUCE_GATHER, 0, induce_batch_count_kernel<WT, MODE_S_FROM_S, ST>, dim3(grid), dim3(kBlock),
+                  (const uint32_t *)st.SA, (const ST *)st.WN, rin, c, st.cfg, st.T, st.bhist, st.stride, min_len);
     }
     sx_launch(ctx, SX_KC_INDUCE_SCAN, (uint64_t)tiles_bound * st.nk * kBatchRounds * 8, induce_batch_offsets_kernel,
               dim3(kBatchRounds * st.nk), dim3(kRowThreads), st.bhist, st.stride, rin, st.btotals, st.nk, min_len);
     if (mode == MODE_L_FROM_L) {
-        sx_launch(ctx, SX_KC_INDUCE_SCATTER, 0, induce_batch_scatter_kernel<WT, MODE_L_FROM_L>, dim3(grid), dim3(kBlock),
-                  (const uint32_t *)st.SA, (const WT *)st.WN, rin, rout, c, st.cfg, st.T, (const uint32_t *)st.bhist, st.stride,
+        sx_launch(ctx, SX_KC_INDUCE_SCATTER, 0, induce_batch_scatter_kernel<WT, MODE_L_FROM_L, ST>, dim3(grid), dim3(kBlock),
+                  (const uint32_t *)st.SA, (const ST *)st.WN, rin, rout, c, st.cfg, st.T, (const uint32_t *)st.bhist, st.stride,
                   (const uint32_t *)st.btotals, cur, nxt, st.SA, st.WN, st.BW, st.nk, min_len);
     } else {
-        sx_launch(ctx, SX_KC_INDUCE_SCATTER, 0, induce_batch_scatter_kernel<WT, MODE_S_FROM_S>, dim3(grid), dim3(kBlock),
-                  (const uint32_t *)st.SA, (const WT *)st.WN, rin, rout, c, st.cfg, st.T, (const uint32_t *)st.bhist, st.stride,
+        sx_launch(ctx, SX_KC_INDUCE_SCATTER, 0, induce_batch_scatter_kernel<WT, MODE_S_FROM_S, ST>, dim3(grid), dim3(kBlock),
+                  (const uint32_t *)st.SA, (const ST *)st.WN, rin, rout, c, st.cfg, st.T, (const uint32_t *)st.bhist, st.stride,
                   (const uint32_t *)st.btotals, cur, nxt, st.SA, st.WN, st.BW, st.nk, min_len);
     }
     st.par ^= 1;
     ctx->stats.induce_rounds++;
 }
 
-template <class WT>
-int run_self_rounds(induce_state<WT> &st, uint32_t fixed_bound, uint32_t region_entries, int rev, int mode, uint32_t c,
+template <class WT, class ST>
+int run_self_rounds(induce_state<WT, ST> &st, uint32_t fixed_bound, uint32_t region_entries, int rev, int mode, uint32_t c,
                     int dir, int which, uint32_t *total_in_region, double share ,
                     const uint32_t *resume = nullptr )
 {
@@ -255,7 +258,7 @@
                     uint32_t tb = sx_div_up((uint64_t)(expect * 2.0 < (double)region_entries ? expect * 2.0 : (double)region_entries), kIndTile);
                     if (tb < 256) tb = bound_tiles < 256 ? bound_tiles : 256;
                     const bool sure = ctx->induce_batch_min >= 0 || expect > 4.0 * (double)st.chain_max;
-                    launch_round<WT>(st, st.SA, st.WN, slot, slot + 1, tb, tb, rev, mode, c, dir, 1, 0, sure ? 1 : 0);
+                    launch_round<WT>(st, st.SA, (const WT *)nullptr, st.WN, slot, slot + 1, tb, tb, rev, mode, c, dir, 1, 0, sure ? 1 : 0);
                     ++slot;
                 }
             }
@@ -263,7 +266,7 @@
             ++slot;
             if (!first) {
                 for (int k = 0; k < 3; ++k, ++slot)
-                    launch_round<WT>(st, st.SA, st.WN, slot, slot + 1, bound_tiles < 256 ? bound_tiles : 256, 0, rev, mode, c, dir, 1, 1);
+                    launch_round<WT>(st, st.SA, (const WT *)nullptr, st.WN, slot, slot + 1, bound_tiles < 256 ? bound_tiles : 256, 0, rev, mode, c, dir, 1, 1);
             }
             spec = slot;
         }
@@ -275,7 +278,7 @@
             for (int i = 0; i < k; ++i) expect *= share;
             const uint32_t likely = expect < (double)bound_tiles ? (uint32_t)expect : bound_tiles;
             const bool sure = first && k == 0 && (uint64_t)region_entries > 16ull * st.chain_max;
-            launch_round<WT>(st, st.SA, st.WN, k, k + 1, tb, first && k == 0 ? bound_tiles : likely, rev, mode, c, dir, 1, 0, sure ? 1 : 0);
+            launch_round<WT>(st, st.SA, (const WT *)nullptr, st.WN, k, k + 1, tb, first && k == 0 ? bound_tiles : likely, rev, mode, c, dir, 1, 0, sure ? 1 : 0);
         }
         launch_tail<WT>(st, spec, spec + 1, rev, mode, c, dir);
         if (st.unattended) {
@@ -304,7 +307,7 @@
                               dim3(far_chunks < kRunProbeGrid ? far_chunks : kRunProbeGrid, r[1] - r[0]), dim3(kBlock), st.T,
                               (const uint32_t *)st.SA, (const uint32_t *)st.ranges, c, kRunProbeChunk, (uint32_t)look, st.run_len);
                 }
-                sx_launch(ctx, SX_KC_INDUCE_CHAIN, 0, run_fill_kernel<WT>, dim3(4096), dim3(kBlock), st.T, st.SA, st.WN, st.BW,
+                sx_launch(ctx, SX_KC_INDUCE_CHAIN, 0, run_fill_kernel<WT, ST>, dim3(4096), dim3(kBlock), st.T, st.SA, st.WN, st.BW,
                           (const uint32_t *)st.ranges, (const uint32_t *)st.cursor[st.par], c, rev, dir, st.cfg,
                           (const uint32_t *)st.run_len);
                 sx_launch(ctx, SX_KC_INDUCE_CHAIN, 0, run_commit_kernel, dim3(1), dim3(1), st.ranges, st.cursor[st.par], c, dir,
@@ -315,21 +318,23 @@
     }
 }
 
-template <class WT>
+template <class WT, class ST = WT>
 int induce_typed(sx_ctx *ctx, const sx_text_info &ti, uint32_t sigma, const uint32_t *sorted_lms,
                  const void *seed_windows, bool seed_windows_u32, uint32_t *SA, uint8_t *bwt_out, sx_arena &arena, wnd_cfg cfg)
 {
     const uint64_t N = ti.N;
     const uint32_t nk = ti.maxc + 1 < sigma ? ti.maxc + 1 : sigma;
-    induce_state<WT> st;
+    induce_state<WT, ST> st;
     st.ctx = ctx;
     st.T = ti.T;
     st.SA = SA;
     st.nk = nk;
     st.small_alphabet = nk <= 8;
+    if (induce_state<WT, ST>::kNarrow && !st.small_alphabet)
+        return sx_fail_msg(ctx, SX_E_INTERNAL, "induce: 16-bit stored windows with more than 8 buckets");
     st.cfg = cfg;
     st.par = 0;
-    st.WN = arena.take<WT>(N);
+    st.WN = arena.take<ST>(N);
     st.BW = bwt_out ? bwt_out : arena.take<uint8_t>(N);
     st.N = N;
     st.m = ti.m;
@@ -379,7 +384,7 @@
     else if (!seed_windows)
         sx_launch(ctx, SX_KC_INDUCE_GATHER, ti.m * (4 + sizeof(WT) + 16), fill_windows_kernel<WT>,
                   dim3(sx_div_up(ti.m, kBlock)), dim3(kBlock), ti.T, sorted_lms, ti.m, cfg, seedW);
-    sx_launch(ctx, SX_KC_MISC, 0, set_entry_kernel<WT>, dim3(1), dim3(1), SA, st.WN, st.BW, (uint32_t)ti.n, ti.T, cfg);
+    sx_launch(ctx, SX_KC_MISC, 0, set_entry_kernel<WT, ST>, dim3(1), dim3(1), SA, st.WN, st.BW, (uint32_t)ti.n, ti.T, cfg);
 
     st.poison = arena.take<uint32_t>(4);
     if (!st.poison) return sx_fail_msg(ctx, SX_E_INTERNAL, "induce: arena too small");
@@ -429,6 +434,7 @@
                   hz_EL, hz_ES);
     }
     auto hoisted_rounds = [&](int pass) -> int {
+        if constexpr (!induce_state<WT, ST>::kNarrow) {
         const uint32_t *desc = hz_desc + pass * 768;
         const int rev = pass, mode = pass == 0 ? MODE_L_FROM_LMS : MODE_S_FROM_L, dir = pass == 0 ? +1 : -1;
         const uint32_t *srcP = pass == 0 ? sorted_lms : (const uint32_t *)SA;
@@ -447,6 +453,7 @@
                   mode, st.cfg, st.T, (const uint32_t *)hz_hist, (const uint32_t *)hz_dbase, dir, st.SA, st.WN, st.BW,
                   (uint32_t)(pass == 0 ? 1 : 0));
         ctx->stats.induce_rounds++;
+        }
         return 0;
     };
     auto pass_end = [&](int pass, bool with_stop, uint32_t (&rec)[4], uint32_t (&cur)[256], uint32_t (&tail)[3]) -> int {
@@ -499,7 +506,7 @@
             if (ti.h_lms[c] && !st.hoist) {
                 sx_launch(ctx, SX_KC_INDUCE_SCAN, 0, set_range_kernel, dim3(1), dim3(1), st.ranges, lms_off[c], lms_off[c + 1],
                           (const uint32_t *)st.cursor[st.par], (int)c, 0, st.tickets, 1u, (const uint32_t *)(st.unattended ? st.poison : nullptr));
-                launch_round<WT>(st, sorted_lms, seedW, 0, -1, sx_div_up(ti.h_lms[c], kIndTile), sx_div_up(ti.h_lms[c], kIndTile), 0,
+                launch_round<WT>(st, sorted_lms, seedW, (const ST *)nullptr, 0, -1, sx_div_up(ti.h_lms[c], kIndTile), sx_div_up(ti.h_lms[c], kIndTile), 0,
                                  MODE_L_FROM_LMS, c, +1, 0, 0, ti.h_lms[c] > st.chain_max ? 1 : 0);
             }
         }
@@ -529,7 +536,7 @@
                 sx_launch(ctx, SX_KC_INDUCE_SCAN, 0, set_range_kernel, dim3(1), dim3(1), st.ranges, begin[c],
                           begin[c] + ti.h_l[c], (const uint32_t *)st.cursor[st.par], (int)c, 0, st.tickets, 1u,
                           (const uint32_t *)(st.unattended ? st.poison : nullptr));
-                launch_round<WT>(st, SA, st.WN, 0, -1, sx_div_up(ti.h_l[c], kIndTile), sx_div_up(ti.h_l[c], kIndTile), 1,
+                launch_round<WT>(st, SA, (const WT *)nullptr, st.WN, 0, -1, sx_div_up(ti.h_l[c], kIndTile), sx_div_up(ti.h_l[c], kIndTile), 1,
                                  MODE_S_FROM_L, c, -1, 0, 0, ti.h_l[c] > st.chain_max ? 1 : 0);
             }
         }
@@ -571,7 +578,7 @@
         if (ctx->prof_only < 0 || ctx->prof_only == SX_KC_INDUCE_GATHER)
             ctx->kstat[SX_KC_INDUCE_GATHER].alg_bytes += (scanned - ti.m) + ti.m * sizeof(WT);
         if (ctx->prof_only < 0 || ctx->prof_only == SX_KC_INDUCE_SCATTER)
-            ctx->kstat[SX_KC_INDUCE_SCATTER].alg_bytes += (scanned + N) * (4 + sizeof(WT)) + N;
+            ctx->kstat[SX_KC_INDUCE_SCATTER].alg_bytes += (scanned + N) * (4 + sizeof(ST)) + ti.m * (sizeof(WT) - sizeof(ST)) + N;
     }
     return 0;
 }
@@ -593,6 +600,9 @@
     if (ti.N > 0xFFFFFFFFull) return sx_fail_msg(ctx, SX_E_ARG, "induce: n exceeds 32-bit positions");
     wnd_cfg cfg;
     const bool wide = sx_window_cfg(ti.maxc, cfg);
+    ctx->stats.window_bits = sx_window_stored_bits(cfg, wide, ctx->induce_window_bits);
+    if (ctx->stats.window_bits == 16u)
+        return induce_typed<uint32_t, uint16_t>(ctx, ti, sigma, sorted_lms, seed_windows, false, SA, bwt_out, arena, cfg);
     if (!wide) return induce_typed<uint32_t>(ctx, ti, sigma, sorted_lms, seed_windows, false, SA, bwt_out, arena, cfg);
     return induce_typed<uint64_t>(ctx, ti, sigma, sorted_lms, seed_windows, seed_windows_u32, SA, bwt_out, arena, cfg);
 }
diff --git a/stralg_amd/csrc/sx_induce_chain.hpp b/stralg_amd/csrc/sx_induce_chain.hpp
--- a/stralg_amd/csrc/sx_induce_chain.hpp
+++ b/stralg_amd/csrc/sx_induce_chain.hpp
@@ -3,12 +3,13 @@
 
 namespace sx {
 
-template <class WT, int BITS>
+template <class WT, int BITS, class ST = WT>
 __global__ __launch_bounds__(kBlock) void induce_round_kernel(
-    const uint32_t *__restrict__ srcP, const WT *__restrict__ srcW, const uint32_t *__restrict__ range_in,
+    const uint32_t *__restrict__ srcP, const WT *__restrict__ seedW , const ST *__restrict__ arrW ,
+    const uint32_t *__restrict__ range_in,
     uint32_t *__restrict__ range_out, int rev, int mode, uint32_t c, wnd_cfg cfg, const uint8_t *__restrict__ T,
     const uint32_t *__restrict__ cursor_cur, uint32_t *__restrict__ cursor_nxt, int dir, uint32_t *__restrict__ SA,
-    WT *__restrict__ WN, uint8_t *__restrict__ BW, uint32_t nkeys, uint64_t *__restrict__ status, uint32_t epoch,
+    ST *__restrict__ WN, uint8_t *__restrict__ BW, uint32_t nkeys, uint64_t *__restrict__ status, uint32_t epoch,
     uint32_t *__restrict__ ticket,
     uint32_t chain_max ,
     int tail_follows ,
@@ -50,7 +51,7 @@
             const uint32_t i = wave0 + (uint32_t)k * kWave + lane;
             const uint32_t idx = lo + (i < len ? (rev ? len - 1u - i : i) : 0u);
             val[k] = srcP[idx];
-            wnd[k] = srcW[idx];
+            wnd[k] = arrW ? (WT)arrW[idx] : seedW[idx];
         }
 #pragma unroll
         for (int k = 0; k < kIndItems; ++k) {
@@ -122,7 +123,7 @@
                 const uint32_t dst = dir > 0 ? gbase[d] + r : gbase[d] - 1u - r;
                 const WT nw = wnd[k];
                 SA[dst] = val[k];
-                WN[dst] = nw;
+                WN[dst] = wnd_store<ST, WT>(nw, cfg);
                 BW[dst] = wnd_symbol<WT>(nw, cfg);
             }
         }
@@ -421,8 +422,8 @@
     return L > most ? most : L;
 }
 
-template <class WT>
-__global__ __launch_bounds__(kBlock) void run_fill_kernel(const uint8_t *__restrict__ T, uint32_t *SA, WT *__restrict__ WN,
+template <class WT, class ST = WT>
+__global__ __launch_bounds__(kBlock) void run_fill_kernel(const uint8_t *__restrict__ T, uint32_t *SA, ST *__restrict__ WN,
                                                          uint8_t *__restrict__ BW, const uint32_t *__restrict__ range,
                                                          const uint32_t *__restrict__ cursor, uint32_t c, int rev, int dir,
                                                          wnd_cfg cfg, const uint32_t *__restrict__ run_len)
@@ -436,7 +437,7 @@
         const uint32_t dst = dir > 0 ? cur + (uint32_t)o : cur - 1u - (uint32_t)o;
         const WT nw = v ? wnd_fill<WT>(T, v, cfg) : (WT)0;
         SA[dst] = v;
-        WN[dst] = nw;
+        WN[dst] = wnd_store<ST, WT>(nw, cfg);
         BW[dst] = wnd_symbol<WT>(nw, cfg);
     }
 }
@@ -520,12 +521,12 @@
     }
 }
 
-template <class WT>
-__global__ void set_entry_kernel(uint32_t *SA, WT *WN, uint8_t *BW, uint32_t p, const uint8_t *T, wnd_cfg cfg)
+template <class WT, class ST = WT>
+__global__ void set_entry_kernel(uint32_t *SA, ST *WN, uint8_t *BW, uint32_t p, const uint8_t *T, wnd_cfg cfg)
 {
     const WT w = p ? wnd_fill<WT>(T, p, cfg) : (WT)0;
     SA[0] = p;
-    WN[0] = w;
+    WN[0] = wnd_store<ST, WT>(w, cfg);
     BW[0] = wnd_symbol<WT>(w, cfg);
 }
 
diff --git a/stralg_amd/csrc/sx_induce_common.hpp b/stralg_amd/csrc/sx_induce_common.hpp
--- a/stralg_amd/csrc/sx_induce_common.hpp
+++ b/stralg_amd/csrc/sx_induce_common.hpp
@@ -4,6 +4,7 @@
 #include "sx_scan.hpp"
 #include "sx_internal.hpp"
 #include "sx_window.hpp"
+#include <type_traits>
 
 namespace sx {
 
diff --git a/stralg_amd/csrc/sx_induce_small.hpp b/stralg_amd/csrc/sx_induce_small.hpp
--- a/stralg_amd/csrc/sx_induce_small.hpp
+++ b/stralg_amd/csrc/sx_induce_small.hpp
@@ -152,20 +152,25 @@
     }
 }
 
-template <class WT, int MODE>
+template <class WT, int MODE, class ST = WT>
 __global__ __launch_bounds__(kBlock) void induce_scatter_small_kernel(
-    const uint32_t *__restrict__ srcP, const WT *__restrict__ srcW, const uint32_t *__restrict__ range_in, uint32_t c,
+    const uint32_t *__restrict__ srcP, const WT *__restrict__ seedW , const ST *__restrict__ arrW ,
+    const uint32_t *__restrict__ range_in, uint32_t c,
     wnd_cfg cfg, const uint8_t *__restrict__ T, const uint32_t *__restrict__ offs, uint32_t stride,
-    const uint32_t *__restrict__ cursor_cur, uint32_t *__restrict__ SA, WT *__restrict__ WN, uint8_t *__restrict__ BW,
+    const uint32_t *__restrict__ cursor_cur, uint32_t *__restrict__ SA, ST *__restrict__ WN, uint8_t *__restrict__ BW,
     uint32_t nkeys, uint32_t chain_max)
 {
+    using SrcT = typename std::conditional<MODE == MODE_L_FROM_LMS, WT, ST>::type;
+    const SrcT *__restrict__ srcW;
+    if constexpr (MODE == MODE_L_FROM_LMS) srcW = seedW;
+    else srcW = arrW;
     constexpr bool kRev = MODE == MODE_S_FROM_S || MODE == MODE_S_FROM_L;
     constexpr uint64_t kField16 = 0x00FF00FF00FF00FFull;
     __shared__ uint64_t wsum[2][kWavesPerBlock];
     __shared__ uint64_t sbase[2];
     __shared__ uint32_t gadj[8];
     __shared__ uint32_t sP[kIndTile];
-    __shared__ WT sW[kIndTile];
+    __shared__ ST sW[kIndTile];
     __shared__ uint8_t sD[kIndTile];
     __shared__ uint16_t refill[kIndTile];
     __shared__ uint32_t nrefill;
@@ -183,13 +188,13 @@
         if (i0 + kIndItems <= len) {
             const uint32_t first = kRev ? lo + len - i0 - kIndItems : lo + i0;
             uint32_t Pm[kIndItems];
-            WT Wm[kIndItems];
+            SrcT Wm[kIndItems];
             __builtin_memcpy(Pm, srcP + first, sizeof(Pm));
             __builtin_memcpy(Wm, srcW + first, sizeof(Wm));
 #pragma unroll
             for (int k = 0; k < kIndItems; ++k) {
                 P[k] = Pm[kRev ? kIndItems - 1 - k : k];
-                W[k] = Wm[kRev ? kIndItems - 1 - k : k];
+                W[k] = (WT)Wm[kRev ? kIndItems - 1 - k : k];
             }
         } else {
 #pragma unroll
@@ -197,7 +202,7 @@
                 const uint32_t i = i0 + (uint32_t)k;
                 const uint32_t idx = i < len ? (kRev ? lo + len - 1u - i : lo + i) : lo;
                 P[k] = i < len ? srcP[idx] : 0u;
-                W[k] = i < len ? srcW[idx] : (WT)0;
+                W[k] = i < len ? (WT)srcW[idx] : (WT)0;
             }
         }
         uint32_t rnk[kIndItems], dig[kIndItems];
@@ -252,7 +257,7 @@
                 const uint32_t j = P[k] - 1u;
                 const WT nw = wnd_pop<WT>(W[k], cfg);
                 sP[slot] = j;
-                sW[slot] = nw;
+                sW[slot] = wnd_store<ST, WT>(nw, cfg);
                 sD[slot] = (uint8_t)d;
                 if (j != 0 && wnd_count<WT>(nw) == 0) refill[atomicAdd(&nrefill, 1u)] = (uint16_t)slot;
             }
@@ -262,7 +267,7 @@
         if (nre) {
             for (uint32_t r = (uint32_t)t; r < nre; r += kBlock) {
                 const uint32_t slot = refill[r];
-                sW[slot] = wnd_fill<WT>(T, sP[slot], cfg);
+                sW[slot] = wnd_store<ST, WT>(wnd_fill<WT>(T, sP[slot], cfg), cfg);
             }
             __syncthreads();
         }
@@ -272,10 +277,10 @@
             if (i < produced) {
                 const uint32_t g = gadj[sD[i]];
                 const uint32_t dst = kRev ? g - i : g + i;
-                const WT nw = sW[i];
+                const ST nw = sW[i];
                 SA[dst] = sP[i];
                 WN[dst] = nw;
-                BW[dst] = wnd_symbol<WT>(nw, cfg);
+                BW[dst] = wnd_symbol<WT>((WT)nw, cfg);
             }
         }
         __syncthreads();
@@ -289,8 +294,8 @@
 #endif
 constexpr uint32_t kClosedFrom = SX_TAIL_CLOSED_FROM;
 constexpr uint32_t kClosedEntries = 5120;
-template <class WT>
-__global__ __launch_bounds__(kTailBlock) void induce_tail_small_kernel(uint32_t *SA, WT *WN, uint8_t *BW,
+template <class WT, class ST = WT>
+__global__ __launch_bounds__(kTailBlock) void induce_tail_small_kernel(uint32_t *SA, ST *WN, uint8_t *BW,
                                                                        const uint32_t *__restrict__ range_in,
                                                                        uint32_t *__restrict__ range_out, int rev, int mode,
                                                                        uint32_t c, wnd_cfg cfg, const uint8_t *__restrict__ T,
@@ -356,7 +361,7 @@
                     const uint32_t dst = dir > 0 ? cur + o : cur - 1u - o;
                     const WT nw = v ? wnd_fill<WT>(T, v, cfg) : (WT)0;
                     SA[dst] = v;
-                    WN[dst] = nw;
+                    WN[dst] = wnd_store<ST, WT>(nw, cfg);
                     BW[dst] = wnd_symbol<WT>(nw, cfg);
                 }
                 __syncthreads();
@@ -530,7 +535,7 @@
                                 nw = (codes << kCntBits) | (WT)(have < cfg.CW ? have : cfg.CW);
                             }
                             SA[dst] = pos;
-                            WN[dst] = nw;
+                            WN[dst] = wnd_store<ST, WT>(nw, cfg);
                             BW[dst] = wnd_symbol<WT>(nw, cfg);
                         }
                         cc += (uint32_t)__popcll(bc);
@@ -547,7 +552,7 @@
                                     const uint32_t dst = dir > 0 ? curD[d] + o : curD[d] - 1u - o, pos = p - j;
                                     const WT nw = pos == 0 ? (WT)0 : wnd_pop<WT>(wend, cfg);
                                     SA[dst] = pos;
-                                    WN[dst] = nw;
+                                    WN[dst] = wnd_store<ST, WT>(nw, cfg);
                                     BW[dst] = wnd_symbol<WT>(nw, cfg);
                                 }
                                 cd[d] += (uint32_t)__popcll(bd);
@@ -586,7 +591,7 @@
                 if ((uint32_t)k < per && i < len) {
                     const uint32_t idx = lo + (rev ? len - 1u - i : i);
                     val[k] = SA[idx];
-                    wnd[k] = WN[idx];
+                    wnd[k] = (WT)WN[idx];
                     live |= 1u << k;
                 }
             }
@@ -709,7 +714,7 @@
                     WT nw = (((codes >> (j * B)) >> B) << kCntBits) | (WT)(wcnt - (uint32_t)(j + 1));
                     if (pos != 0 && wcnt == (uint32_t)(j + 1)) nw = wnd_fill<WT>(T, pos, cfg);
                     SA[dst] = pos;
-                    WN[dst] = nw;
+                    WN[dst] = wnd_store<ST, WT>(nw, cfg);
                     BW[dst] = wnd_symbol<WT>(nw, cfg);
                     if ((uint32_t)j == nr - 1u && ((alive_after >> k) & 1u)) {
                         live_next |= 1u << k;
@@ -791,20 +796,20 @@
     return pat;
 }
 
-template <class WT, bool kRev, bool kWantP>
-__device__ __forceinline__ void batch_load(const uint32_t *__restrict__ srcP, const WT *__restrict__ srcW, uint32_t lo, uint32_t len,
+template <class WT, bool kRev, bool kWantP, class ST>
+__device__ __forceinline__ void batch_load(const uint32_t *__restrict__ srcP, const ST *__restrict__ srcW, uint32_t lo, uint32_t len,
                                            uint32_t i0, uint32_t (&P)[kIndItems], WT (&W)[kIndItems])
 {
     if (i0 + kIndItems <= len) {
         const uint32_t first = kRev ? lo + len - i0 - kIndItems : lo + i0;
         uint32_t Pm[kIndItems];
-        WT Wm[kIndItems];
+        ST Wm[kIndItems];
         if (kWantP) __builtin_memcpy(Pm, srcP + first, sizeof(Pm));
         __builtin_memcpy(Wm, srcW + first, sizeof(Wm));
 #pragma unroll
         for (int k = 0; k < kIndItems; ++k) {
             P[k] = kWantP ? Pm[kRev ? kIndItems - 1 - k : k] : 0u;
-            W[k] = Wm[kRev ? kIndItems - 1 - k : k];
+            W[k] = (WT)Wm[kRev ? kIndItems - 1 - k : k];
         }
     } else {
 #pragma unroll
@@ -812,7 +817,7 @@
             const uint32_t i = i0 + (uint32_t)k;
             const uint32_t idx = i < len ? (kRev ? lo + len - 1u - i : lo + i) : lo;
             P[k] = (kWantP && i < len) ? srcP[idx] : 0u;
-            W[k] = i < len ? srcW[idx] : (WT)0;
+            W[k] = i < len ? (WT)srcW[idx] : (WT)0;
         }
     }
 }
@@ -828,8 +833,8 @@
     }
 }
 
-template <class WT, int MODE>
-__global__ __launch_bounds__(kBlock) void induce_batch_count_kernel(const uint32_t *__restrict__ srcP, const WT *__restrict__ srcW,
+template <class WT, int MODE, class ST = WT>
+__global__ __launch_bounds__(kBlock) void induce_batch_count_kernel(const uint32_t *__restrict__ srcP, const ST *__restrict__ srcW,
                                                                     const uint32_t *__restrict__ range_in, uint32_t c, wnd_cfg cfg,
                                                                     const uint8_t *__restrict__ T, uint32_t *__restrict__ hist ,
                                                                     uint32_t stride, uint32_t min_len)
@@ -846,7 +851,7 @@
         const uint32_t i0 = tile * (uint32_t)kIndTile + (uint32_t)t * kIndItems;
         uint32_t P[kIndItems];
         WT W[kIndItems];
-        batch_load<WT, kRev, false>(srcP, srcW, lo, len, i0, P, W);
+        batch_load<WT, kRev, false, ST>(srcP, srcW, lo, len, i0, P, W);
         uint64_t cnt[kBatchRounds];
 #pragma unroll
         for (int j = 0; j < kBatchRounds; ++j) cnt[j] = 0;
@@ -895,12 +900,12 @@
     if (threadIdx.x == 0) totals[row] = total;
 }
 
-template <class WT, int MODE>
+template <class WT, int MODE, class ST = WT>
 __global__ __launch_bounds__(kBlock, 2) void induce_batch_scatter_kernel(
-    const uint32_t *__restrict__ srcP, const WT *__restrict__ srcW, const uint32_t *__restrict__ range_in,
+    const uint32_t *__restrict__ srcP, const ST *__restrict__ srcW, const uint32_t *__restrict__ range_in,
     uint32_t *__restrict__ range_out, uint32_t c, wnd_cfg cfg, const uint8_t *__restrict__ T, const uint32_t *__restrict__ offs,
     uint32_t stride, const uint32_t *__restrict__ totals, const uint32_t *__restrict__ cursor_cur, uint32_t *__restrict__ cursor_nxt,
-    uint32_t *__restrict__ SA, WT *__restrict__ WN, uint8_t *__restrict__ BW, uint32_t nk, uint32_t min_len)
+    uint32_t *__restrict__ SA, ST *__restrict__ WN, uint8_t *__restrict__ BW, uint32_t nk, uint32_t min_len)
 {
     constexpr bool kRev = MODE == MODE_S_FROM_S;
     constexpr uint64_t kField16 = 0x00FF00FF00FF00FFull;
@@ -948,7 +953,7 @@
         const uint32_t i0 = tile * (uint32_t)kIndTile + (uint32_t)t * kIndItems;
         uint32_t P[kIndItems];
         WT W[kIndItems];
-        batch_load<WT, kRev, true>(srcP, srcW, lo, len, i0, P, W);
+        batch_load<WT, kRev, true, ST>(srcP, srcW, lo, len, i0, P, W);
         batch_plan<WT> pl[kIndItems];
         uint64_t cnt[kBatchRounds];
 #pragma unroll
@@ -990,7 +995,7 @@
                     const uint32_t pos = P[k] - (uint32_t)(j + 1);
                     const WT nw = batch_window<WT>(W[k], (uint32_t)j, pos, cfg, T);
                     SA[dst] = pos;
-                    WN[dst] = nw;
+                    WN[dst] = wnd_store<ST, WT>(nw, cfg);
                     BW[dst] = wnd_symbol<WT>(nw, cfg);
                     run[j] += 1ull << (8u * d);
                 }
diff --git a/stralg_amd/csrc/sx_window.hpp b/stralg_amd/csrc/sx_window.hpp
--- a/stralg_amd/csrc/sx_window.hpp
+++ b/stralg_amd/csrc/sx_window.hpp
@@ -62,6 +62,18 @@
     return (acc << kCntBits) | (WT)cnt;
 }
 
+constexpr uint32_t kNarrowCodeBits = 16 - kCntBits;
+template <class ST, class WT> __device__ __forceinline__ ST wnd_store(WT w, const wnd_cfg &c)
+{
+    if constexpr (sizeof(ST) == sizeof(WT)) {
+        return (ST)w;
+    } else {
+        static_assert(sizeof(ST) == 2 && sizeof(WT) == 4, "16-bit stored windows of 32-bit working windows");
+        const uint32_t cn = c.B >= 2 ? kNarrowCodeBits / 2u : kNarrowCodeBits, cnt = (uint32_t)w & 15u;
+        return (ST)(((uint32_t)w & 0xFFF0u) | (cnt < cn ? cnt : cn));
+    }
+}
+
 template <class WT>
 __device__ __forceinline__ WT wnd_fill(const uint8_t *__restrict__ T, uint32_t p, const wnd_cfg &c)
 {
@@ -92,3 +104,9 @@
     if (cfg.CW > 15) cfg.CW = 15;
     return wide;
 }
+
+static inline uint32_t sx_window_stored_bits(const sx::wnd_cfg &cfg, bool wide, int want)
+{
+    if (wide) return 64u;
+    return (cfg.B <= 2 && want == 16) ? 16u : 32u;
+}
```

New measurement: 54140 Msuffixes/s (median of 5 runs). 1.6% higher.
